# GaryGky/IDEAL-NeRF

Measured on AMD Instinct MI355X. Metric: ray-samples/sec (64+128 pts, 512x512), whole job, higher is better.
Workload: dtype f32

## Files before the change

ideal-nerf_amd/_lib.py:

```python
import ctypes as C
import os

HERE = os.path.dirname(os.path.abspath(__file__))
LIB_PATH = os.environ.get("IDN_LIB") or os.path.join(HERE, "libidealnerf.so")

IDN_PREC_F32, IDN_PREC_BF16X3, IDN_PREC_BF16, IDN_PREC_FP16X3, IDN_PREC_BF16X6 = 0, 1, 2, 3, 4
RAY_FLOATS = 11
MAX_MULTIRES, MAX_MULTIRES_VIEWS = 10, 4
SAMPLE_MAX_REGION = 4096
SCORE_TILE = 32
PROF_KINDS = ("mlp_fwd", "mlp_fwd_save", "delta_chain", "dw_gemm", "dw_gemm_x6", "mlp_fwd_save_x6", "delta_chain_x6")

fp = C.c_void_p


class FaceNerfParams(C.Structure):
    _fields_ = [("pts_w", fp * 8), ("pts_b", fp * 8), ("views_w", fp * 3), ("views_b", fp * 3),
                ("alpha_w", fp), ("alpha_b", fp), ("rgb_w", fp), ("rgb_b", fp),
                ("dim_aud", C.c_int), ("dim_expr", C.c_int), ("dim_latent", C.c_int),
                ("multires_plus1", C.c_int), ("multires_views_plus1", C.c_int)]


class FaceNerfGrads(C.Structure):
    _fields_ = [("pts_w", fp * 8), ("pts_b", fp * 8), ("views_w", fp * 3), ("views_b", fp * 3),
                ("alpha_w", fp), ("alpha_b", fp), ("rgb_w", fp), ("rgb_b", fp)]


class PassBwdExtra(C.Structure):
    _fields_ = [("d_expr", fp), ("d_rays", fp), ("d_views0_bias", fp)]


class CompositeOut(C.Structure):
    _fields_ = [(n, fp) for n in ("rgb_map", "disp_map", "acc_map", "depth_map", "weights", "rgb_fg", "last_weight")]


class RenderArgs(C.Structure):
    _fields_ = [("rays", fp), ("bc_rgb", fp), ("n_rays", C.c_int64), ("n_samples", C.c_int),
                ("n_importance", C.c_int), ("precision", C.c_int),
                ("packed_coarse", fp), ("folded_coarse", fp), ("packed_fine", fp), ("folded_fine", fp),
                ("t_vals", fp), ("t_rand", fp), ("u", fp), ("u_per_ray", C.c_int)] + \
               [(n, fp) for n in ("rgb_map", "disp_map", "acc_map", "depth_map", "last_weight", "rgb_fg",
                                  "rgb0", "disp0", "acc0", "z_std", "last_weight0", "rgb_fg0",
                                  "tap_z_coarse", "tap_raw_coarse", "tap_weights_coarse", "tap_cdf", "tap_inds",
                                  "tap_z_samples", "tap_z_fine", "tap_raw_fine", "tap_weights_fine")] + \
               [("workspace", fp), ("workspace_bytes", C.c_size_t), ("precision_fine_plus1", C.c_int),
                ("lindisp", C.c_int), ("white_bkgd", C.c_int), ("noise_coarse", fp), ("noise_fine", fp), ("fused_march", C.c_int),
                ("rng_mode", C.c_int), ("rng_seed", C.c_uint64), ("rng_ray0", C.c_int64)]


class AudioNetParams(C.Structure):
    _fields_ = [("conv_w", fp * 4), ("conv_b", fp * 4), ("fc_w", fp * 2), ("fc_b", fp * 2), ("dim_aud", C.c_int)]


class AudioNetGrads(C.Structure):
    _fields_ = [("conv_w", fp * 4), ("conv_b", fp * 4), ("fc_w", fp * 2), ("fc_b", fp * 2)]


class Frame(C.Structure):
    _fields_ = [("c2w", C.c_float * 12), ("H", C.c_int), ("W", C.c_int), ("focal", C.c_float), ("cx", C.c_float), ("cy", C.c_float),
                ("near_", C.c_float), ("far_", C.c_float), ("row0", C.c_int), ("nrows", C.c_int), ("rays_out", fp)]


class RenderOpts(C.Structure):
    _fields_ = [("colour_gate", C.c_int), ("gate_counters", fp)]


class CullGridStruct(C.Structure):
    _fields_ = [("bits", fp), ("G", C.c_int), ("lo", C.c_float * 3), ("cell", C.c_float)]


CULL_MAX_OUTPUTS = 12


class CullOutput(C.Structure):
    _fields_ = [("dense", fp), ("live", fp), ("channels", C.c_int), ("fill_background", C.c_int), ("value", C.c_float)]


DW_MAX_PRODUCTS, DW_MAX_TAKES, DW_MAX_COLSUM_TAKES = 16, 4, 2


class DwTake(C.Structure):
    _fields_ = [("row0", C.c_int), ("col0", C.c_int), ("rows", C.c_int), ("cols", C.c_int), ("out", fp), ("ldo", C.c_int)]


class DwColsumTake(C.Structure):
    _fields_ = [("col0", C.c_int), ("cols", C.c_int), ("out", fp)]


class DwProduct(C.Structure):
    _fields_ = [("delta", fp), ("ld_delta", C.c_int), ("N", C.c_int), ("acts", fp), ("ld_acts", C.c_int), ("K", C.c_int),
                ("acts2", fp), ("want_colsum", C.c_int), ("n_takes", C.c_int), ("takes", DwTake * DW_MAX_TAKES),
                ("n_colsum_takes", C.c_int), ("colsum_takes", DwColsumTake * DW_MAX_COLSUM_TAKES),
                ("splits", C.c_int), ("chunks_per_split", C.c_int)]


PATCH_MAX, PATCH_MIN_P, PATCH_MAX_P = 16, 11, 48


class PatchSet(C.Structure):
    _fields_ = [("n_patches", C.c_int), ("p", C.c_int), ("oy", C.c_int * PATCH_MAX), ("ox", C.c_int * PATCH_MAX)]


ABI_VERSION = 4

PROTOTYPES = {
    "idealnerf_version": (C.c_int, []),
    "idealnerf_last_error": (C.c_char_p, []),
    "idealnerf_packed_weight_floats": (C.c_size_t, [C.c_int]),
    "idealnerf_folded_bias_floats": (C.c_size_t, []),
    "idealnerf_pack_weights": (C.c_int, [C.POINTER(FaceNerfParams), C.c_int, fp, fp]),
    "idealnerf_fold_conditioning": (C.c_int, [C.POINTER(FaceNerfParams), fp, fp, fp, fp, fp]),
    "idealnerf_facenerf_fwd": (C.c_int, [fp, fp, C.c_int, fp, C.c_int64, fp, fp]),
    "idealnerf_facenerf_fwd_ch": (C.c_int, [fp, fp, C.c_int, fp, C.c_int, C.c_int, C.c_int64, fp, fp]),
    "idealnerf_params_pts_ch": (C.c_int, [C.POINTER(FaceNerfParams)]),
    "idealnerf_params_views_ch": (C.c_int, [C.POINTER(FaceNerfParams)]),
    "idealnerf_query_rays_fwd": (C.c_int, [fp, fp, C.c_int, fp, fp, C.c_int64, C.c_int, fp, fp]),
    "idealnerf_query_points_fwd": (C.c_int, [fp, fp, C.c_int, fp, fp, C.c_int64, C.c_int, fp, fp]),
    "idealnerf_frame_rays": (C.c_int, [C.POINTER(C.c_float), C.c_int, C.c_int, C.c_float, C.c_float, C.c_float,
                                       C.c_float, C.c_float, C.c_int, C.c_int, fp, fp]),
    "idealnerf_to8b": (C.c_int, [fp, C.c_int64, C.c_int, fp, fp, fp]),
    "idealnerf_compose_to8b": (C.c_int, [fp, fp, fp, C.c_int64, C.c_int, fp, fp, fp, fp]),
    "idealnerf_philox_uniform": (C.c_int, [C.c_uint64, C.c_int, C.c_int64, C.c_int64, C.c_int, fp, fp]),
    "idealnerf_sample_pixels_workspace_bytes": (C.c_size_t, []),
    "idealnerf_sample_pixels": (C.c_int, [fp, C.c_int, C.c_int, C.c_int, C.c_int, C.c_int, C.c_int, C.c_uint64, C.c_uint64,
                                          fp, C.c_size_t, fp, fp]),
    "idealnerf_gather_rays": (C.c_int, [fp, C.c_int64, C.POINTER(C.c_float), C.c_int, C.c_int, C.c_float, C.c_float, C.c_float,
                                        fp, fp, fp, fp, fp, fp, fp, fp]),
    "idealnerf_gather_ray_pairs": (C.c_int, [fp, C.c_int64, C.POINTER(C.c_float), C.POINTER(C.c_float), C.c_int, C.c_int, C.c_float,
                                             C.c_float, C.c_float, fp, fp, fp, fp, fp, fp, fp, fp, fp]),
    "idealnerf_frame_scores_workspace_bytes": (C.c_size_t, [C.c_int, C.c_int]),
    "idealnerf_frame_scores": (C.c_int, [fp, fp, fp, C.c_int, C.c_int, fp, fp, C.c_size_t, fp]),
    "idealnerf_patch_pixels": (C.c_int, [C.POINTER(PatchSet), C.c_int, fp, fp]),
    "idealnerf_ssim_patch_fwd": (C.c_int, [fp, fp, C.c_int, C.c_int, fp, fp]),
    "idealnerf_ssim_patch_bwd": (C.c_int, [fp, fp, C.c_int, C.c_int, C.c_float, fp, fp]),
    "idealnerf_coarse_depths": (C.c_int, [fp, fp, fp, C.c_int, C.c_int64, C.c_int, fp, fp]),
    "idealnerf_composite_fwd": (C.c_int, [fp, fp, fp, fp, fp, C.c_int, C.c_int64, C.c_int, C.POINTER(CompositeOut), fp]),
    "idealnerf_sample_pdf_fwd": (C.c_int, [fp, fp, fp, C.c_int, C.c_int64, C.c_int, C.c_int, fp, fp, fp, fp, fp, fp]),
    "idealnerf_march_fwd": (C.c_int, [fp, fp, fp, fp, fp, C.c_int, fp, C.c_int, C.c_int64, C.c_int, C.c_int,
                                      C.POINTER(CompositeOut), fp, fp, fp, fp, fp, fp]),
    "idealnerf_sample_pdf_bins_fwd": (C.c_int, [fp, fp, fp, C.c_int, C.c_int64, C.c_int, C.c_int, fp, fp, fp, fp]),
    "idealnerf_invert_cdf": (C.c_int, [fp, fp, fp, C.c_int, C.c_int64, C.c_int, C.c_int, fp, fp, fp]),
    "idealnerf_render_workspace_bytes": (C.c_size_t, [C.c_int64, C.c_int, C.c_int]),
    "idealnerf_render_rays_fwd": (C.c_int, [C.POINTER(RenderArgs), fp]),
    "idealnerf_render_frame_workspace_bytes": (C.c_size_t, [C.c_int64, C.c_int, C.c_int]),
    "idealnerf_render_frame_fwd": (C.c_int, [C.POINTER(RenderArgs), C.POINTER(Frame), fp]),
    "idealnerf_render_rays_fwd_opts": (C.c_int, [C.POINTER(RenderArgs), C.POINTER(RenderOpts), fp]),
    "idealnerf_render_frame_fwd_opts": (C.c_int, [C.POINTER(RenderArgs), C.POINTER(Frame), C.POINTER(RenderOpts), fp]),
    "idealnerf_colour_gate_max_dist": (C.c_float, []),
    "idealnerf_audio_net_saved_floats": (C.c_size_t, [C.c_int]),
    "idealnerf_audio_net_fwd": (C.c_int, [C.POINTER(AudioNetParams), fp, C.c_int, fp, fp, fp]),
    "idealnerf_audio_net_bwd": (C.c_int, [C.POINTER(AudioNetParams), C.POINTER(AudioNetGrads), fp, fp, fp, C.c_int, fp]),
    "idealnerf_train_acts_floats": (C.c_size_t, [C.c_int64]),
    "idealnerf_query_rays_train_fwd": (C.c_int, [fp, fp, C.c_int, fp, fp, C.c_int64, C.c_int, fp, fp, fp]),
    "idealnerf_query_rays_train_fwd_ch": (C.c_int, [fp, fp, C.c_int, fp, fp, C.c_int64, C.c_int, C.c_int, C.c_int, fp, fp, fp]),
    "idealnerf_pass_bwd_workspace_bytes": (C.c_size_t, [C.c_int64, C.c_int]),
    "idealnerf_pass_bwd": (C.c_int, [C.POINTER(FaceNerfParams), C.POINTER(FaceNerfGrads), fp, fp, fp, fp, fp, fp, fp,
                                     fp, C.c_int64, C.c_int, fp, fp, fp, fp, fp, fp, fp, C.c_size_t, fp]),
    "idealnerf_pass_bwd_rays": (C.c_int, [C.POINTER(FaceNerfParams), C.POINTER(FaceNerfGrads), fp, fp, fp, fp, fp, fp, fp,
                                          fp, C.c_int64, C.c_int, fp, fp, fp, fp, fp, fp, fp, fp, C.c_size_t, fp]),
    "idealnerf_pass_bwd_cond": (C.c_int, [C.POINTER(FaceNerfParams), fp, fp, fp, fp, fp, fp, fp, fp, C.c_int64, C.c_int, fp, fp, fp,
                                          fp, fp, fp, fp, C.c_size_t, fp]),
    "idealnerf_pass_bwd_ex": (C.c_int, [C.POINTER(FaceNerfParams), C.POINTER(FaceNerfGrads), fp, fp, fp, fp, fp, fp, fp,
                                        fp, C.c_int64, C.c_int, fp, fp, fp, fp, fp, fp, C.POINTER(PassBwdExtra), fp, C.c_size_t, fp]),
    "idealnerf_facenerf_train_fwd": (C.c_int, [fp, fp, C.c_int, fp, C.c_int64, fp, fp, fp]),
    "idealnerf_facenerf_train_fwd_ch": (C.c_int, [fp, fp, C.c_int, fp, C.c_int, C.c_int, C.c_int64, fp, fp, fp]),
    "idealnerf_facenerf_bwd_workspace_bytes": (C.c_size_t, [C.c_int64]),
    "idealnerf_facenerf_bwd": (C.c_int, [C.POINTER(FaceNerfParams), C.POINTER(FaceNerfGrads), fp, fp, fp, fp, C.c_int64, fp,
                                         fp, fp, fp, fp, fp, C.c_size_t, fp]),
    "idealnerf_dw_gemm_workspace_bytes": (C.c_size_t, []),
    "idealnerf_dw_gemm": (C.c_int, [fp, C.c_int, fp, C.c_int, C.c_int64, fp, fp, C.c_int, fp, C.c_size_t, fp]),
    "idealnerf_dw_products_workspace_bytes": (C.c_size_t, []),
    "idealnerf_dw_products": (C.c_int, [C.c_int64, C.c_int, C.c_int, C.POINTER(DwProduct), C.c_int, fp, C.c_size_t, fp]),
    "idealnerf_delta_chain_workspace_bytes": (C.c_size_t, []),
    "idealnerf_delta_chain": (C.c_int, [C.POINTER(FaceNerfParams), C.c_int, fp, C.c_int64, fp, fp, fp, fp, C.c_int,
                                        C.POINTER(C.c_int), fp, C.c_size_t, fp]),
    "idealnerf_composite_bwd": (C.c_int, [fp, fp, fp, fp, C.c_int64, C.c_int, fp, fp, fp, fp, fp, C.c_int, fp, C.c_int, fp, C.c_int, fp]),
    "idealnerf_input_grad": (C.c_int, [C.POINTER(FaceNerfParams), fp, fp, fp, C.c_int64, C.c_int64, fp, C.c_int, C.POINTER(C.c_int), fp]),
    "idealnerf_ray_grad": (C.c_int, [fp, C.c_int, C.c_int, fp, fp, C.c_int64, C.c_int, fp, fp]),
    "idealnerf_fold_bwd": (C.c_int, [C.POINTER(FaceNerfParams), fp, fp, fp, fp, fp, fp, fp, fp, fp, fp, fp, fp, fp]),
    "idealnerf_cond_colsums_workspace_bytes": (C.c_size_t, []),
    "idealnerf_cond_colsums": (C.c_int, [fp, fp, fp, C.c_int64, C.c_int64, fp, fp, fp, C.c_size_t, fp]),
    "idealnerf_cull_mark": (C.c_int, [fp, C.c_int64, C.c_float, fp, fp]),
    "idealnerf_cull_cells": (C.c_int, [fp, C.c_int, C.c_int, fp, fp]),
    "idealnerf_cull_classify_workspace_bytes": (C.c_size_t, [C.c_int64]),
    "idealnerf_cull_classify": (C.c_int, [C.POINTER(CullGridStruct), C.POINTER(Frame), C.c_float, C.c_int, fp, fp, fp, C.c_size_t, fp]),
    "idealnerf_cull_gather": (C.c_int, [fp, C.c_int64, C.POINTER(Frame), fp, fp, fp, fp]),
    "idealnerf_cull_scatter": (C.c_int, [fp, C.c_int64, C.c_int64, fp, C.POINTER(CullOutput), C.c_int, fp]),
    "idealnerf_cull_sample_classify": (C.c_int, [C.POINTER(CullGridStruct), fp, fp, C.c_int64, C.c_int, fp, fp, fp, C.c_size_t, fp]),
    "idealnerf_cull_sample_gather": (C.c_int, [fp, C.c_int64, fp, fp, C.c_int64, C.c_int, fp, fp, fp]),
    "idealnerf_cull_sample_scatter": (C.c_int, [fp, C.c_int64, fp, C.c_int64, fp, fp]),
    "idealnerf_profile_begin": (None, []),
    "idealnerf_profile_end": (C.c_int, [C.POINTER(C.c_double), C.POINTER(C.c_int64), C.POINTER(C.c_int64)]),
    "idealnerf_profile_end_kinds": (C.c_int, [C.POINTER(C.c_double), C.POINTER(C.c_int64), C.POINTER(C.c_int64)]),
}

_lib = None


class IdealNerfError(RuntimeError):
    pass


def load():
    global _lib
    if _lib is not None:
        return _lib
    if not os.path.exists(LIB_PATH):
        raise IdealNerfError(
            f"{LIB_PATH} is missing: build the HIP extension first "
            "(python ideal-nerf_amd/build.py, or __graft_entry__.build()). There is no fallback path.")
    lib = C.CDLL(LIB_PATH)
    for name, (res, args) in PROTOTYPES.items():
        fn = getattr(lib, name)
        fn.restype = res
        fn.argtypes = args
    if lib.idealnerf_version() != ABI_VERSION:
        raise IdealNerfError(f"{LIB_PATH} has ABI version {lib.idealnerf_version()}, this package binds version {ABI_VERSION}: rebuild it")
    _lib = lib
    return lib


def check(rc):
    if rc != 0:
        msg = load().idealnerf_last_error()
        raise IdealNerfError(f"libidealnerf error {rc}: {msg.decode() if msg else '?'}")
```

ideal-nerf_amd/csrc/dw_gemm.h:

```cpp
#pragma once
#include "mlp_common.h"

namespace idn {

__device__ __forceinline__ f32x16 mfma32(float a, float b, f32x16 c) { return __builtin_amdgcn_mfma_f32_32x32x2f32(a, b, c, 0, 0, 0); }
__device__ __forceinline__ int d_row(int r, int hh) { return (r & 3) + 8 * (r >> 2) + 4 * hh; }

struct TNArgs {
    const float* A; int lda;
    const float* B; int ldb;
    float* part;
    int N, K;
    long P;
    int chunks_per_split;
    float* cpart;
    int b_split, b_off0, b_off1;
};
constexpr int kMaxTnBatch = 12;
struct TNBatch {
    TNArgs it[kMaxTnBatch];
    int n, splits;
};
constexpr int kMaxReduceItems = 32;
struct ReduceItem {
    const float* part;
    float* out;
    int splits, N, K, ldo, rows, cols;
    int block_end;
};
struct ReduceBatch {
    ReduceItem it[kMaxReduceItems];
    int n;
};

inline size_t al256(size_t x) { return (x + 255) & ~(size_t)255; }
enum { kPipeX6 = IDN_DW_PIPE_BF16X6, kPipeF32 = IDN_DW_PIPE_F32 };

struct DwPassProduct { int N, K; bool colsum; int pipes; };
constexpr int kOnX6 = 1 << kPipeX6, kOnF32 = 1 << kPipeF32, kOnBoth = kOnX6 | kOnF32;
constexpr DwPassProduct kTrunk = {256, 256, true, kOnBoth};
constexpr DwPassProduct kPassProducts[] = {
    {64, 128, true, kOnBoth},
    {256, 256, true, kOnX6}, {128, 128, true, kOnF32}, {128, 128, true, kOnF32},
    kTrunk, {128, 64, false, kOnBoth},
    kTrunk, kTrunk, kTrunk, {256, 64, false, kOnBoth}, kTrunk, kTrunk, kTrunk, kTrunk,
    {256, 64, true, kOnBoth},
};
constexpr size_t pass_sum(int pipe, int what) {
    size_t n = 0;
    for (const DwPassProduct& t : kPassProducts)
        if (t.pipes >> pipe & 1) n += what == 0 ? (t.N == 256 && t.K == 256) : what == 1 ? (size_t)t.N * t.K : t.colsum ? t.N : 0;
    return n;
}
constexpr int kX6ItemsPerPass = (int)pass_sum(kPipeX6, 0);
static_assert(kX6ItemsPerPass == 9 && kX6ItemsPerPass <= kMaxTnBatch, "one x6 batch per pass");

constexpr int kMaxSplits = 256;
constexpr int kColsumBlocks = 256;
constexpr int kGemmsPerPass = 16;
constexpr size_t kPartFloatsPerSplit = 9 * 65536 + 6 * 16384 + 4 * 8192;
constexpr size_t kPartPoolFloats = (size_t)kMaxSplits * kPartFloatsPerSplit, kCpartPoolFloats = (size_t)kColsumBlocks * 256 * kGemmsPerPass;
static_assert(pass_sum(kPipeX6, 1) <= kPartFloatsPerSplit && pass_sum(kPipeF32, 1) <= kPartFloatsPerSplit, "a pass's partial blocks fit");
static_assert(kMaxSplits * pass_sum(kPipeX6, 2) <= kCpartPoolFloats && kMaxSplits * pass_sum(kPipeF32, 2) <= kCpartPoolFloats, "a pass's column sums fit");

struct DwProduct { const float *part, *cpart; int splits, N, K, chunks_per_split; };

struct DwPass {
    DwPass(float* part, size_t part_floats, float* cpart, size_t cpart_floats, int64_t P, int pipe, int x6_items, hipStream_t s)
        : part_next(part), part_left(part_floats), cpart_next(cpart), cpart_left(cpart_floats), P(P), pipe(pipe), x6_items(x6_items), s(s) {}
    int product(const float* A, int lda, int N, const float* B, int ldb, int K, bool want_colsum, DwProduct* h, const float* B2 = nullptr);
    int take(const DwProduct& h, int row0, int col0, int rows, int cols, float* out, int ldo);
    int take_colsum(const DwProduct& h, int col0, int cols, float* out);
    int finish();

private:
    float* part_next; size_t part_left;
    float* cpart_next; size_t cpart_left;
    int64_t P;
    int pipe, x6_items;
    hipStream_t s;
    TNBatch x6{{}, 0, 0};
    ReduceBatch red{{}, 0};
    int red_blocks = 0;
};

}
```

ideal-nerf_amd/csrc/dw_gemm.hip:

```cpp
#include "dw_gemm.h"
#include "mlp_x6.h"

namespace idn {

template <int N>
struct LdsVec;
template <>
struct LdsVec<4> {
    f32x4 v;
    template <int OFF>
    __device__ __forceinline__ void issue(uint32_t addr) { asm volatile("ds_read_b128 %0, %1 offset:%2" : "=v"(v) : "v"(addr), "n"(OFF) : "memory"); }
    __device__ __forceinline__ float get(int j) const { return v[j]; }
};
template <>
struct LdsVec<2> {
    typedef float f32x2 __attribute__((ext_vector_type(2)));
    f32x2 v;
    template <int OFF>
    __device__ __forceinline__ void issue(uint32_t addr) { asm volatile("ds_read_b64 %0, %1 offset:%2" : "=v"(v) : "v"(addr), "n"(OFF) : "memory"); }
    __device__ __forceinline__ float get(int j) const { return v[j]; }
};
template <>
struct LdsVec<1> {
    float v;
    template <int OFF>
    __device__ __forceinline__ void issue(uint32_t addr) { asm volatile("ds_read_b32 %0, %1 offset:%2" : "=v"(v) : "v"(addr), "n"(OFF) : "memory"); }
    __device__ __forceinline__ float get(int) const { return v; }
};
template <int OFF>
__device__ __forceinline__ void lds_read_f32(float& dst, uint32_t addr) {
    asm volatile("ds_read_b32 %0, %1 offset:%2" : "=v"(dst) : "v"(addr), "n"(OFF) : "memory");
}
__device__ __forceinline__ float landed(float& v) {
    asm volatile("" : "+v"(v));
    return v;
}
template <int NEWER, class VA, class VB>
__device__ __forceinline__ void lds_retire(VA& a, VB& b) {
    if constexpr (NEWER == 0) asm volatile("s_waitcnt lgkmcnt(0)" : "+v"(a.v), "+v"(b.v)::"memory");
    else asm volatile("s_waitcnt lgkmcnt(2)" : "+v"(a.v), "+v"(b.v)::"memory");
}

constexpr int kTnRows = 16, kTnBufs = 3;
constexpr int kTnNarrowBufs = 3;
constexpr int kTnRows4x1 = 32, kTnRowsThin = 64;
constexpr int kTnNarrowSplits = 256;

template <int NTW, int KTW, int NB = kTnBufs, int R = kTnRows>
__global__ __launch_bounds__(256) void gemm_tn_kernel(TNArgs g) {
    static_assert(R % 16 == 0, "chunks are multiples of 16 points");
    constexpr int NPA = NTW * R / 16, NPB = KTW * R / 16;
    static_assert(NB >= 3 && (NB - 2) * (NPA + NPB) <= 63, "vmcnt is a 6-bit field");
    constexpr int BN = 64 * NTW, BK = 64 * KTW;
    constexpr int kTileFloats = R * (BN + BK);
    constexpr int kSteps = R / 2;
    constexpr int NP = NPA + NPB;
    static_assert(NP <= kSteps, "at most one piece per step");
    extern __shared__ __attribute__((aligned(16))) float tn_smem[];
    const int tid = threadIdx.x, lane = tid & 63;
    const int w = __builtin_amdgcn_readfirstlane(tid >> 6);
    const int i = lane & 31, hh = lane >> 5;
    const int wr = w >> 1, wc = w & 1;
    const int n0 = blockIdx.x * BN, k0 = blockIdx.y * BK;
    const int split = blockIdx.z;
    f32x16 acc[NTW][KTW];
#pragma unroll
    for (int a = 0; a < NTW; ++a)
#pragma unroll
        for (int b = 0; b < KTW; ++b)
            for (int r = 0; r < 16; ++r) acc[a][b][r] = 0.f;

    const long c_begin = (long)split * g.chunks_per_split;
    long c_end = c_begin + g.chunks_per_split;
    const long c_total = g.P / R;
    if (c_end > c_total) c_end = c_total;
    const bool colsum_block = g.cpart != nullptr && blockIdx.y == 0;
    const bool do_colsum = colsum_block && tid < BN;
    const int ccol = tid < BN ? tid : 0;
    float csum = 0.0f;

    constexpr int kRowsPerPieceA = 256 / BN > 0 ? 256 / BN : 1, kRowsPerPieceB = 256 / BK > 0 ? 256 / BK : 1;
    const __amdgpu_buffer_rsrc_t rsrcA = __builtin_amdgcn_make_buffer_rsrc(const_cast<float*>(g.A + n0 + c_begin * R * (long)g.lda), 0, 0xfffffffc, 0x00020000);
    const __amdgpu_buffer_rsrc_t rsrcB = __builtin_amdgcn_make_buffer_rsrc(const_cast<float*>(g.B + k0 + c_begin * R * (long)g.ldb), 0, 0xfffffffc, 0x00020000);
    const uint32_t voffA = ((lane / (BN / 4)) * g.lda + (lane % (BN / 4)) * 4) * 4;
    const uint32_t voffB = ((lane / (BK / 4)) * g.ldb + (lane % (BK / 4)) * 4) * 4;
    const uint32_t rowA = g.lda * 4, rowB = g.ldb * 4;
    auto piece_a = [&](long c, int buf, int ja) {
        const int pc = NPA * w + ja;
        __builtin_amdgcn_raw_ptr_buffer_load_lds(rsrcA, (__attribute__((address_space(3))) void*)(tn_smem + buf * kTileFloats + pc * 256), 16, voffA,
                                                 (uint32_t)(((c - c_begin) * R + pc * kRowsPerPieceA) * rowA), 0, 0);
    };
    auto piece_b = [&](long c, int buf, int jb) {
        const int pc = NPB * w + jb;
        __builtin_amdgcn_raw_ptr_buffer_load_lds(rsrcB, (__attribute__((address_space(3))) void*)(tn_smem + buf * kTileFloats + R * BN + pc * 256), 16, voffB,
                                                 (uint32_t)(((c - c_begin) * R + pc * kRowsPerPieceB) * rowB), 0, 0);
    };
    auto piece = [&](long c, int buf, int j) {
        if (j < NPA) piece_a(c, buf, j);
        else if (j < NP) piece_b(c, buf, j - NPA);
    };
    const uint32_t smem0 = (uint32_t)(uintptr_t)(__attribute__((address_space(3))) float*)tn_smem;
    const uint32_t a_addr0 = smem0 + (hh * BN + NTW * (32 * wr + i)) * 4;
    const uint32_t b_addr0 = smem0 + (R * BN + hh * BK + KTW * (32 * wc + i)) * 4;
    for (int ahead = 0; ahead < NB - 1; ++ahead)
        for (int j = 0; j < NP; ++j) piece(c_begin + ahead < c_end ? c_begin + ahead : c_end - 1, ahead, j);
    int buf = 0;
    for (long c = c_begin; c < c_end; ++c) {
        asm volatile("s_waitcnt vmcnt(%0)" ::"n"((NB - 2) * NP) : "memory");
        __builtin_amdgcn_s_barrier();
        asm volatile("" ::: "memory");
        const int buf2 = buf >= 1 ? buf - 1 : NB - 1;
        const long cnext = c + NB - 1 < c_end ? c + NB - 1 : c_end - 1;
        float cs[16];
        auto cs_issue = [&](int batch) {
            const uint32_t caddr = smem0 + buf * (kTileFloats * 4) + ccol * 4 + batch * (16 * BN * 4);
            static_for<16>([&](auto Row) {
                lds_read_f32<decltype(Row)::value * BN * 4>(cs[decltype(Row)::value], caddr);
            });
        };
        static_assert(R / 16 <= kSteps / 4, "one batch of column reads per iteration of the first half loop");
        if (colsum_block) cs_issue(0);
        LdsVec<NTW> a0v, a1v;
        LdsVec<KTW> b0v, b1v;
        constexpr int kStepA = 2 * BN * 4, kStepB = 2 * BK * 4;
        uint32_t pa = a_addr0 + buf * (kTileFloats * 4), pb = b_addr0 + buf * (kTileFloats * 4);
        a0v.template issue<0>(pa);
        b0v.template issue<0>(pb);
        static_assert(NPA <= kSteps / 2 && NPB <= kSteps / 2, "pieces of one matrix fit one half of a chunk");
        constexpr int M = NTW * KTW;
        if constexpr (M >= 4) {
            auto step = [&](LdsVec<NTW>& ca, LdsVec<KTW>& cb, auto&& side0, auto&& side1, auto&& side2) {
                lds_retire<0>(ca, cb);
                static_for<M>([&](auto M_) {
                    constexpr int m = decltype(M_)::value, x = m / KTW, y = m % KTW;
                    acc[x][y] = mfma32(ca.get(x), cb.get(y), acc[x][y]);
                    if constexpr (m < 3) {
                        __builtin_amdgcn_sched_barrier(0);
                        if constexpr (m == 0) side0();
                        if constexpr (m == 1) side1();
                        if constexpr (m == 2) side2();
                        __builtin_amdgcn_sched_barrier(0);
                    }
                });
            };
#pragma unroll 1
            for (int it = 0; it < kSteps / 4; ++it) {
                step(a0v, b0v,
                     [&]() { a1v.template issue<kStepA>(pa); b1v.template issue<kStepB>(pb); },
                     [&]() { if (2 * it < NPA) piece_a(cnext, buf2, 2 * it); },
                     [&]() {
                         if (colsum_block && it < R / 16) {
                             static_for<16>([&](auto Row) { csum += landed(cs[decltype(Row)::value]); });
                         }
                         pa += 2 * kStepA;
                         pb += 2 * kStepB;
                     });
                step(a1v, b1v,
                     [&]() { a0v.template issue<0>(pa); b0v.template issue<0>(pb); },
                     [&]() { if (2 * it + 1 < NPA) piece_a(cnext, buf2, 2 * it + 1); },
                     [&]() { if (colsum_block && it + 1 < R / 16) cs_issue(it + 1); });
            }
#pragma unroll 1
            for (int it = 0; it < kSteps / 4; ++it) {
                const bool last = it == kSteps / 4 - 1;
                step(a0v, b0v,
                     [&]() { a1v.template issue<kStepA>(pa); b1v.template issue<kStepB>(pb); },
                     [&]() { if (2 * it < NPB) piece_b(cnext, buf2, 2 * it); },
                     [&]() {
                         pa = last ? pa : pa + 2 * kStepA;
                         pb = last ? pb : pb + 2 * kStepB;
                     });
                step(a1v, b1v,
                     [&]() { a0v.template issue<0>(pa); b0v.template issue<0>(pb); },
                     [&]() { if (2 * it + 1 < NPB) piece_b(cnext, buf2, 2 * it + 1); },
                     [&]() {});
            }
        } else {
            static_assert(M == 2 && kSteps % 8 == 0, "the two-pair schedule");
            LdsVec<NTW> a2v, a3v;
            LdsVec<KTW> b2v, b3v;
            a1v.template issue<kStepA>(pa);
            b1v.template issue<kStepB>(pb);
            auto quad = [&](LdsVec<NTW>& c0a, LdsVec<KTW>& c0b, LdsVec<NTW>& c1a, LdsVec<KTW>& c1b, LdsVec<NTW>& n0a, LdsVec<KTW>& n0b,
                            LdsVec<NTW>& n1a, LdsVec<KTW>& n1b, bool last, auto&& side_c, auto&& side_d) {
                lds_retire<0>(c0a, c0b);
                lds_retire<0>(c1a, c1b);
                const uint32_t na = last ? pa : pa + 2 * kStepA, nb = last ? pb : pb + 2 * kStepB;
                auto mf = [&](LdsVec<NTW>& ca, LdsVec<KTW>& cb, auto M_) {
                    constexpr int m = decltype(M_)::value, x = m / KTW, y = m % KTW;
                    acc[x][y] = mfma32(ca.get(x), cb.get(y), acc[x][y]);
                    __builtin_amdgcn_sched_barrier(0);
                };
                mf(c0a, c0b, ic<0>{});
                n0a.template issue<0>(na);
                n0b.template issue<0>(nb);
                __builtin_amdgcn_sched_barrier(0);
                mf(c0a, c0b, ic<1>{});
                n1a.template issue<kStepA>(na);
                n1b.template issue<kStepB>(nb);
                __builtin_amdgcn_sched_barrier(0);
                mf(c1a, c1b, ic<0>{});
                side_c();
                __builtin_amdgcn_sched_barrier(0);
                mf(c1a, c1b, ic<1>{});
                side_d();
                pa = na;
                pb = nb;
                __builtin_amdgcn_sched_barrier(0);
            };
#pragma unroll 1
            for (int it = 0; it < kSteps / 8; ++it) {
                quad(a0v, b0v, a1v, b1v, a2v, b2v, a3v, b3v, false,
                     [&]() { if (2 * it < NPA) piece_a(cnext, buf2, 2 * it); },
                     [&]() {
                         if (colsum_block && it < R / 16) {
                             static_for<16>([&](auto Row) { csum += landed(cs[decltype(Row)::value]); });
                         }
                     });
                quad(a2v, b2v, a3v, b3v, a0v, b0v, a1v, b1v, false,
                     [&]() { if (2 * it + 1 < NPA) piece_a(cnext, buf2, 2 * it + 1); },
                     [&]() { if (colsum_block && it + 1 < R / 16) cs_issue(it + 1); });
            }
#pragma unroll 1
            for (int it = 0; it < kSteps / 8; ++it) {
                quad(a0v, b0v, a1v, b1v, a2v, b2v, a3v, b3v, false,
                     [&]() { if (2 * it < NPB) piece_b(cnext, buf2, 2 * it); }, [&]() {});
                quad(a2v, b2v, a3v, b3v, a0v, b0v, a1v, b1v, it == kSteps / 8 - 1,
                     [&]() { if (2 * it + 1 < NPB) piece_b(cnext, buf2, 2 * it + 1); }, [&]() {});
            }
            lds_retire<0>(a1v, b1v);
        }
        lds_retire<0>(a0v, b0v);
        buf = buf + 1 == NB ? 0 : buf + 1;
    }
    asm volatile("s_waitcnt vmcnt(0)" ::: "memory");
    if (do_colsum) g.cpart[(long)split * g.N + n0 + tid] = csum;
    float* out = g.part + (long)split * g.N * g.K;
#pragma unroll
    for (int x = 0; x < NTW; ++x)
#pragma unroll
        for (int r = 0; r < 16; ++r) {
            const int n = n0 + NTW * (32 * wr + d_row(r, hh)) + x;
            float* dst = out + (long)n * g.K + k0 + KTW * (32 * wc + i);
            if constexpr (KTW == 4) {
                *reinterpret_cast<f32x4*>(dst) = f32x4{acc[x][0][r], acc[x][1][r], acc[x][2][r], acc[x][3][r]};
            } else {
#pragma unroll
                for (int y = 0; y < KTW; ++y) dst[y] = acc[x][y][r];
            }
        }
}

typedef unsigned tn_u32x4 __attribute__((ext_vector_type(4)));
typedef int tn_i32x4 __attribute__((ext_vector_type(4)));
__device__ __forceinline__ void split3(float x0, float x1, unsigned& p1, unsigned& p2, unsigned& p3) {
    float w1, w2, w3;
    x6::split3(x0, x1, w1, w2, w3);
    p1 = __float_as_uint(w1), p2 = __float_as_uint(w2), p3 = __float_as_uint(w3);
}
constexpr int kX6BufBytes = 2 * 8 * 3 * kFragBytes;
constexpr int kX6Lds = 2 * kX6BufBytes;

struct X6Frag {
    f32x4 v;
    template <int OFF>
    __device__ __forceinline__ void issue(uint32_t addr) { asm volatile("ds_read_b128 %0, %1 offset:%2" : "=v"(v) : "v"(addr), "n"(OFF) : "memory"); }
};
template <int N>
__device__ __forceinline__ void x6_retire(X6Frag (&f)[3]) {
    static_assert(N <= 15, "lgkmcnt is a 4-bit field");
    asm volatile("s_waitcnt lgkmcnt(%3)" : "+v"(f[0].v), "+v"(f[1].v), "+v"(f[2].v) : "n"(N) : "memory");
}

__device__ __forceinline__ void gemm_tn_x6_item(const TNArgs& g, const int split, char* x6_smem) {
    const int tid = threadIdx.x, lane = tid & 63;
    const int w = __builtin_amdgcn_readfirstlane(tid >> 6);
    const int i = lane & 31, hh = lane >> 5;
    const int wr = w >> 1, wc = w & 1;
    f32x16 acc[4][4];
#pragma unroll
    for (int a = 0; a < 4; ++a)
#pragma unroll
        for (int b = 0; b < 4; ++b)
            for (int r = 0; r < 16; ++r) acc[a][b][r] = 0.f;

    const long c_begin = (long)split * g.chunks_per_split;
    long c_end = c_begin + g.chunks_per_split;
    const long c_total = g.P / kTnRows;
    if (c_end > c_total) c_end = c_total;
    const int n_chunks = (int)(c_end - c_begin);
    auto make_rsrc = [](const float* ptr) {
        const uint64_t a64 = (uint64_t)(uintptr_t)ptr;
        return tn_i32x4{(int)(uint32_t)a64, (int)((uint32_t)(a64 >> 32) & 0xffffu), (int)0xfffffffcu, 0x00020000};
    };
    const tn_i32x4 rsrcA = make_rsrc(g.A + c_begin * kTnRows * (long)g.lda);
    const tn_i32x4 rsrcB = make_rsrc(g.B + c_begin * kTnRows * (long)g.ldb);
    const int voff = tid * 4;
    const int voffB = g.b_split ? (tid < 128 ? g.b_off0 : g.b_off1) + (tid & 127) * 4 : voff;
    const int rowA = g.lda * 4, rowB = g.ldb * 4;
    float ra[kTnRows], rb[kTnRows];
#pragma unroll
    for (int p = 0; p < kTnRows; ++p) ra[p] = rb[p] = 0.f;
    auto load_row_at = [&](float& dst, const tn_i32x4& rsrc, int soff, int vo) {
        asm volatile("buffer_load_dword %0, %1, %2, %3 offen" : "+v"(dst) : "v"(vo), "s"(rsrc), "s"(soff) : "memory");
    };
    auto load_row = [&](float& dst, const tn_i32x4& rsrc, int soff) { load_row_at(dst, rsrc, soff, voff); };
    auto load_chunk = [&](int rc) {
        const int base = (rc < n_chunks ? rc : n_chunks - 1) * kTnRows;
#pragma unroll
        for (int p = 0; p < kTnRows; ++p) load_row(ra[p], rsrcA, (base + p) * rowA);
#pragma unroll
        for (int p = 0; p < kTnRows; ++p) load_row_at(rb[p], rsrcB, (base + p) * rowB, voffB);
    };
    char* const my_slot = x6_smem + (tid >> 5) * (3 * kFragBytes) + (tid & 31) * 16;
    auto split_store = [&](int buf, int X, const float (&r)[kTnRows]) {
        unsigned pw[3][8];
#pragma unroll
        for (int j = 0; j < 8; ++j) split3(r[2 * j], r[2 * j + 1], pw[0][j], pw[1][j], pw[2][j]);
        char* dst = my_slot + buf * kX6BufBytes + X * (8 * 3 * kFragBytes);
#pragma unroll
        for (int q = 0; q < 3; ++q)
#pragma unroll
            for (int h2 = 0; h2 < 2; ++h2)
                *reinterpret_cast<tn_u32x4*>(dst + q * kFragBytes + h2 * 512) =
                    tn_u32x4{pw[q][4 * h2], pw[q][4 * h2 + 1], pw[q][4 * h2 + 2], pw[q][4 * h2 + 3]};
    };
    const bool do_colsum = g.cpart != nullptr;
    float csum = 0.0f, csum1 = 0.0f;
    auto colsum = [&]() {
        float s0 = (ra[0] + ra[1]) + (ra[2] + ra[3]), s1 = (ra[4] + ra[5]) + (ra[6] + ra[7]);
        float s2 = (ra[8] + ra[9]) + (ra[10] + ra[11]), s3 = (ra[12] + ra[13]) + (ra[14] + ra[15]);
        csum += (s0 + s1) + (s2 + s3);
    };
    const uint32_t smem0 = (uint32_t)(uintptr_t)(__attribute__((address_space(3))) char*)x6_smem;
    const uint32_t a_base = smem0 + (4 * wr) * (3 * kFragBytes) + lane * 16;
    const uint32_t b_base = smem0 + (8 + 4 * wc) * (3 * kFragBytes) + lane * 16;

    load_chunk(0);
#pragma unroll
    for (int p = 0; p < kTnRows; ++p) asm volatile("s_waitcnt vmcnt(0)" : "+v"(ra[p]), "+v"(rb[p])::"memory");
    colsum();
    split_store(0, 0, ra);
    split_store(0, 1, rb);
    load_chunk(1);
    asm volatile("s_waitcnt lgkmcnt(0)" ::: "memory");
    __builtin_amdgcn_s_barrier();
    asm volatile("" ::: "memory");

    X6Frag fa[4][3], fb[4][3];
    auto issue_first_row = [&](uint32_t pa, uint32_t pb) {
        static_for<3>([&](auto Q) { fa[0][decltype(Q)::value].template issue<decltype(Q)::value * kFragBytes>(pa); });
        static_for<2>([&](auto Y) {
            static_for<3>([&](auto Q) {
                fb[decltype(Y)::value][decltype(Q)::value].template issue<(decltype(Y)::value * 3 + decltype(Q)::value) * kFragBytes>(pb);
            });
        });
    };
    issue_first_row(a_base, b_base);
#pragma unroll 1
    for (int rc = 0; rc < n_chunks; ++rc) {
        const int buf = rc & 1;
        const uint32_t pa = a_base + buf * kX6BufBytes, pb = b_base + buf * kX6BufBytes;
        static_for<2>([&](auto Y) {
            static_for<3>([&](auto Q) {
                fb[decltype(Y)::value + 2][decltype(Q)::value].template issue<((decltype(Y)::value + 2) * 3 + decltype(Q)::value) * kFragBytes>(pb);
            });
        });
        static_for<3>([&](auto X) {
            static_for<3>([&](auto Q) {
                fa[decltype(X)::value + 1][decltype(Q)::value].template issue<((decltype(X)::value + 1) * 3 + decltype(Q)::value) * kFragBytes>(pa);
            });
        });
        auto mm2 = [&](int x, int y0, int y1) {
#define X6_TERM(QA, QB)                                                   \
    acc[x][y0] = x6::mfma_bf(fa[x][QA].v, fb[y0][QB].v, acc[x][y0]);        \
    acc[x][y1] = x6::mfma_bf(fa[x][QA].v, fb[y1][QB].v, acc[x][y1]);
            X6_TERM(0, 0) X6_TERM(0, 1) X6_TERM(1, 0) X6_TERM(1, 1) X6_TERM(0, 2) X6_TERM(2, 0)
#undef X6_TERM
        };
        x6_retire<15>(fa[0]);
        x6_retire<15>(fb[0]);
        x6_retire<15>(fb[1]);
        mm2(0, 0, 1);
        x6_retire<9>(fb[2]);
        x6_retire<9>(fb[3]);
        mm2(0, 2, 3);
        x6_retire<0>(fa[1]);
        x6_retire<0>(fa[2]);
        x6_retire<0>(fa[3]);
        const unsigned live_mask = rc + 1 < n_chunks ? 0xffffffffu : 0u;
        const int nbase = (rc + 2 < n_chunks ? rc + 2 : n_chunks - 1) * kTnRows;
        char* const dst = my_slot + (buf ^ 1) * kX6BufBytes;
        unsigned pw[2][3][8];
        float t0 = 0.f, t1 = 0.f;
        auto slice = [&](auto X_, auto S_) {
            constexpr int X = decltype(X_)::value, sl = decltype(S_)::value;
            float (&r)[kTnRows] = *(X ? &rb : &ra);
            auto store = [&](auto Q_, auto H_) {
                constexpr int q = decltype(Q_)::value, h2 = decltype(H_)::value;
                *reinterpret_cast<tn_u32x4*>(dst + X * (8 * 3 * kFragBytes) + q * kFragBytes + h2 * 512) =
                    tn_u32x4{pw[X][q][4 * h2], pw[X][q][4 * h2 + 1], pw[X][q][4 * h2 + 2], pw[X][q][4 * h2 + 3]};
            };
            if constexpr (sl < 24) {
                constexpr int j = sl / 3, ph = sl % 3;
                if constexpr (ph == 0) {
                    asm volatile("s_waitcnt vmcnt(30)" : "+v"(r[2 * j]), "+v"(r[2 * j + 1])::"memory");
                    const unsigned p1 = x6::cvt_pk_bf16(r[2 * j], r[2 * j + 1]);
                    pw[X][0][j] = p1;
                    t0 = r[2 * j] - __uint_as_float(p1 << 16);
                    t1 = r[2 * j + 1] - __uint_as_float(p1 & 0xffff0000u);
                    if constexpr (X == 0) {
                        csum += __uint_as_float(__float_as_uint(r[2 * j]) & live_mask);
                        csum1 += __uint_as_float(__float_as_uint(r[2 * j + 1]) & live_mask);
                        asm volatile("" : "+v"(csum), "+v"(csum1));
                    }
                } else if constexpr (ph == 1) {
                    const unsigned p2 = x6::cvt_pk_bf16(t0, t1);
                    pw[X][1][j] = p2;
                    t0 = t0 - __uint_as_float(p2 << 16);
                    t1 = t1 - __uint_as_float(p2 & 0xffff0000u);
                    pw[X][2][j] = x6::cvt_pk_bf16(t0, t1);
                } else {
                    load_row_at(r[2 * j], X ? rsrcB : rsrcA, (nbase + 2 * j) * (X ? rowB : rowA), X ? voffB : voff);
                    load_row_at(r[2 * j + 1], X ? rsrcB : rsrcA, (nbase + 2 * j + 1) * (X ? rowB : rowA), X ? voffB : voff);
                    if constexpr (j >= 3 && j < 6) store(ic<j - 3>{}, ic<0>{});
                    if constexpr (j == 7) store(ic<0>{}, ic<1>{});
                }
            } else if constexpr (sl == 24) {
                store(ic<1>{}, ic<1>{});
            } else if constexpr (sl == 25) {
                store(ic<2>{}, ic<1>{});
            }
        };
        __builtin_amdgcn_sched_barrier(0);
        static_for<72>([&](auto K_) {
            constexpr int k = decltype(K_)::value;
            constexpr int x = 1 + k / 24, kk = k % 24, y = 2 * (kk / 12) + (kk % 2), t = (kk % 12) / 2;
            constexpr int qa = t == 2 || t == 3 ? 1 : (t == 5 ? 2 : 0);
            constexpr int qb = t == 1 || t == 3 ? 1 : (t == 4 ? 2 : 0);
            acc[x][y] = x6::mfma_bf(fa[x][qa].v, fb[y][qb].v, acc[x][y]);
            constexpr int kX1 = 26;
            if constexpr (k < kX1) slice(ic<0>{}, ic<k>{});
            else slice(ic<1>{}, ic<k - kX1>{});
            if constexpr (k == 59) {
                asm volatile("s_waitcnt lgkmcnt(0)" ::: "memory");
                __builtin_amdgcn_s_barrier();
                asm volatile("" ::: "memory");
                issue_first_row(a_base + (buf ^ 1) * kX6BufBytes, b_base + (buf ^ 1) * kX6BufBytes);
            }
            __builtin_amdgcn_sched_barrier(0);
        });
    }
    x6_retire<0>(fa[0]);
    x6_retire<0>(fb[0]);
    x6_retire<0>(fb[1]);
#pragma unroll
    for (int p = 0; p < kTnRows; ++p) asm volatile("s_waitcnt vmcnt(0)" : "+v"(ra[p]), "+v"(rb[p])::"memory");
    if (do_colsum) g.cpart[(long)split * g.N + tid] = csum + csum1;
    float* out = g.part + (long)split * g.N * g.K;
#pragma unroll
    for (int x = 0; x < 4; ++x)
#pragma unroll
        for (int y = 0; y < 4; ++y)
#pragma unroll
            for (int r = 0; r < 16; ++r)
                out[(long)(32 * (4 * wr + x) + d_row(r, hh)) * g.K + 32 * (4 * wc + y) + i] = acc[x][y][r];
}
__global__ __launch_bounds__(256) void gemm_tn_x6_kernel(TNBatch b) {
    extern __shared__ __attribute__((aligned(16))) char x6_smem[];
    const int item = __builtin_amdgcn_readfirstlane((int)blockIdx.z / b.splits);
    const int split = __builtin_amdgcn_readfirstlane((int)blockIdx.z - item * b.splits);
    gemm_tn_x6_item(b.it[item], split, x6_smem);
}

__global__ __launch_bounds__(256) void reduce_batch_kernel(ReduceBatch b) {
    __shared__ double red[4][64];
    int i = 0;
    while (i + 1 < b.n && (int)blockIdx.x >= b.it[i].block_end) ++i;
    const ReduceItem& t = b.it[i];
    const int block0 = i ? b.it[i - 1].block_end : 0;
    const int o = threadIdx.x & 63, q = threadIdx.x >> 6;
    const int idx = ((int)blockIdx.x - block0) * 64 + o;
    const bool live = idx < t.rows * t.cols;
    const int n = live ? idx / t.cols : 0, k = live ? idx % t.cols : 0;
    double s = 0.0;
    if (live) {
        const float* src = t.part + (long)n * t.K + k;
        const long stride = (long)t.N * t.K;
#pragma unroll 8
        for (int sp = q; sp < t.splits; sp += 4) s += (double)src[sp * stride];
    }
    red[q][o] = s;
    __syncthreads();
    if (q == 0 && live) t.out[(long)n * t.ldo + k] = (float)(((red[0][o] + red[1][o]) + red[2][o]) + red[3][o]);
}

template <int NTW, int KTW, int NB, int R = kTnRows>
static int launch_tn(const TNArgs& g, int splits, hipStream_t s) {
    constexpr size_t lds = (size_t)NB * R * (size_t)(64 * NTW + 64 * KTW) * 4;
    static_assert(lds <= 160 * 1024, "the chunk ring must fit a CU's LDS");
    static LaunchSetup setup;
    int num_cu = 0;
    if (int e = setup.get([]() -> int {
            IDN_HIP_CHECK(hipFuncSetAttribute(reinterpret_cast<const void*>(&gemm_tn_kernel<NTW, KTW, NB, R>),
                                              hipFuncAttributeMaxDynamicSharedMemorySize, (int)lds));
            return IDN_OK;
        }, &num_cu))
        return e;
    hipLaunchKernelGGL((gemm_tn_kernel<NTW, KTW, NB, R>), dim3(g.N / (64 * NTW), g.K / (64 * KTW), splits), dim3(256), lds, s, g);
    IDN_HIP_CHECK(hipGetLastError());
    return IDN_OK;
}
struct DwShape { int N, K, rows_per_chunk, max_splits; int (*launch)(const TNArgs&, int, hipStream_t); };
constexpr DwShape kX6Shape = {256, 256, kTnRows, kMaxSplits, nullptr};
constexpr DwShape kF32Shapes[] = {
    {256, 256, kTnRows, kMaxSplits, &launch_tn<4, 4, kTnBufs>},
    {256, 64, kTnRows4x1, kTnNarrowSplits, &launch_tn<4, 1, kTnNarrowBufs, kTnRows4x1>},
    {128, 256, kTnRows, kMaxSplits, &launch_tn<2, 4, kTnBufs>},
    {128, 64, kTnRowsThin, kTnNarrowSplits, &launch_tn<2, 1, kTnNarrowBufs, kTnRowsThin>},
    {128, 128, kTnRows, kMaxSplits, &launch_tn<2, 2, kTnBufs>},
    {64, 128, kTnRowsThin, kTnNarrowSplits, &launch_tn<1, 2, kTnNarrowBufs, kTnRowsThin>},
};
static_assert(kTnNarrowSplits <= kMaxSplits, "the pools hold kMaxSplits splits of every product of a pass (dw_gemm.h)");

static int x6_setup(int* cus) {
    static LaunchSetup st;
    return st.get([]() -> int {
        IDN_HIP_CHECK(hipFuncSetAttribute(reinterpret_cast<const void*>(&gemm_tn_x6_kernel), hipFuncAttributeMaxDynamicSharedMemorySize, kX6Lds));
        return IDN_OK;
    }, cus);
}

int DwPass::product(const float* A, int lda, int N, const float* B, int ldb, int K, bool want_colsum, DwProduct* h, const float* B2) {
    const DwShape* sh = nullptr;
    if (N == 256 && K == 256 && pipe == kPipeX6) sh = &kX6Shape;
    else
        for (const DwShape& t : kF32Shapes)
            if (t.N == N && t.K == K) sh = &t;
    if (!sh) return fail(IDN_EUNSUPPORTED, "gemm_tn: no instantiation for %d x %d", N, K);
    const bool queued = sh->launch == nullptr;
    if (B2 && !queued) return fail(IDN_EINVAL, "gemm_tn: a split B needs the 256 x 256 bf16-piece kernel");
    if (P % sh->rows_per_chunk) return fail(IDN_EINVAL, "gemm_tn: %lld rows are not a multiple of the %d-row chunk", (long long)P, sh->rows_per_chunk);
    const long chunks = P / sh->rows_per_chunk;
    int splits = sh->max_splits;
    if (queued) {
        if (x6.n >= x6_items || x6.n >= kMaxTnBatch) return fail(IDN_EINVAL, "gemm_tn: more 256 x 256 products than the pass declared (%d)", x6_items);
        int cus = 0;
        if (int e = x6_setup(&cus)) return e;
        splits = 2 * cus / x6_items;
        if (splits > kMaxSplits) splits = kMaxSplits;
    }
    if (splits > chunks) splits = (int)chunks;
    if (splits < 1) splits = 1;
    const int cps = (int)((chunks + splits - 1) / splits);
    splits = (int)((chunks + cps - 1) / cps);
    const size_t part_floats = (size_t)splits * N * K, cpart_floats = want_colsum ? (size_t)splits * N : 0;
    if (part_floats > part_left || cpart_floats > cpart_left)
        return fail(IDN_EWORKSPACE, "gemm_tn: the partial blocks of %d x %d in %d splits do not fit the pool", N, K, splits);
    TNArgs g{A, lda, B, ldb, part_next, N, K, (long)P, cps, want_colsum ? cpart_next : nullptr, 0, 0, 0};
    if (B2) {
        const float* base = B < B2 ? B : B2;
        const int64_t o0 = (int64_t)(B - base) * 4, o1 = (int64_t)(B2 - base) * 4;
        if (o0 >= (int64_t)1 << 31 || o1 >= (int64_t)1 << 31) return fail(IDN_EUNSUPPORTED, "gemm_tn: split B matrices more than 2 GiB apart");
        g.B = base, g.b_split = 1;
        g.b_off0 = (int)o0, g.b_off1 = (int)o1;
    }
    if (queued) {
        x6.splits = splits;
        x6.it[x6.n++] = g;
    } else {
        ProfScope prof(s, P, IDN_PROF_DW_GEMM);
        if (int e = sh->launch(g, splits, s)) return e;
    }
    *h = DwProduct{g.part, g.cpart, splits, N, K, cps};
    part_next += part_floats, part_left -= part_floats;
    cpart_next += cpart_floats, cpart_left -= cpart_floats;
    return IDN_OK;
}

int DwPass::take(const DwProduct& h, int row0, int col0, int rows, int cols, float* out, int ldo) {
    if (red.n >= kMaxReduceItems) return fail(IDN_EUNSUPPORTED, "reduce queue full");
    red_blocks += (rows * cols + 63) / 64;
    red.it[red.n++] = ReduceItem{h.part + (size_t)row0 * h.K + col0, out, h.splits, h.N, h.K, ldo, rows, cols, red_blocks};
    return IDN_OK;
}
int DwPass::take_colsum(const DwProduct& h, int col0, int cols, float* out) {
    if (!h.cpart) return fail(IDN_EINVAL, "gemm_tn: the product kept no column sums");
    return take(DwProduct{h.cpart, nullptr, h.splits, 1, h.N, h.chunks_per_split}, 0, col0, 1, cols, out, cols);
}

int DwPass::finish() {
    if (x6.n) {
        ProfScope prof(s, P * x6.n, IDN_PROF_DW_GEMM_X6);
        hipLaunchKernelGGL(gemm_tn_x6_kernel, dim3(1, 1, x6.splits * x6.n), dim3(256), kX6Lds, s, x6);
    }
    IDN_HIP_CHECK(hipGetLastError());
    if (red.n) hipLaunchKernelGGL(reduce_batch_kernel, dim3(red_blocks), dim3(256), 0, s, red);
    IDN_HIP_CHECK(hipGetLastError());
    return IDN_OK;
}

size_t dw_gemm_workspace_bytes() { return al256((size_t)kMaxSplits * 65536 * 4) + al256((size_t)kColsumBlocks * 256 * 4); }
int launch_dw_gemm(const float* delta, int ld_delta, const float* acts, int ld_acts, int64_t rows, float* dW, float* db, int pipe,
                   void* ws, size_t ws_bytes, hipStream_t s) {
    if (rows <= 0 || rows % 128) return fail(IDN_EINVAL, "dw_gemm: rows %lld is not a positive multiple of 128", (long long)rows);
    if (ld_delta < 256 || ld_acts < 256) return fail(IDN_EINVAL, "dw_gemm: row pitch < 256");
    const int x6_items = pipe == IDN_DW_PIPE_BF16X6_PASS ? kX6ItemsPerPass : 1;
    if (pipe == IDN_DW_PIPE_BF16X6_PASS) pipe = IDN_DW_PIPE_BF16X6;
    if (pipe != IDN_DW_PIPE_BF16X6 && pipe != IDN_DW_PIPE_F32) return fail(IDN_EINVAL, "dw_gemm: pipe %d", pipe);
    if (!ws || ws_bytes < dw_gemm_workspace_bytes()) return fail(IDN_EWORKSPACE, "dw_gemm workspace %zu < %zu", ws_bytes, dw_gemm_workspace_bytes());
    float* part = reinterpret_cast<float*>(ws);
    float* cpart = reinterpret_cast<float*>(reinterpret_cast<char*>(ws) + al256((size_t)kMaxSplits * 65536 * 4));
    DwPass q(part, (size_t)kMaxSplits * 65536, cpart, (size_t)kColsumBlocks * 256, rows, pipe, x6_items, s);
    DwProduct h;
    if (int e = q.product(delta, ld_delta, 256, acts, ld_acts, 256, db != nullptr, &h)) return e;
    int e = db ? q.take_colsum(h, 0, 256, db) : IDN_OK;
    if (!e) e = q.take(h, 0, 0, 256, 256, dW, 256);
    return e ? e : q.finish();
}

size_t dw_products_workspace_bytes() { return al256(kPartPoolFloats * 4) + al256(kCpartPoolFloats * 4); }
int launch_dw_products(int64_t rows, int pipe, int x6_items, idn_dw_product* pr, int n, void* ws, size_t ws_bytes, hipStream_t s) {
    if (!pr) return fail(IDN_EINVAL, "dw_products: NULL pointer");
    if (n < 1 || n > IDN_DW_MAX_PRODUCTS) return fail(IDN_EINVAL, "dw_products: %d products outside [1, %d]", n, IDN_DW_MAX_PRODUCTS);
    if (pipe != kPipeX6 && pipe != kPipeF32) return fail(IDN_EINVAL, "dw_products: pipe %d", pipe);
    if (rows <= 0 || rows % 128) return fail(IDN_EINVAL, "dw_products: rows %lld is not a positive multiple of 128", (long long)rows);
    if (rows > (int64_t)1 << 24) return fail(IDN_EUNSUPPORTED, "dw_products: rows %lld exceed 2^24", (long long)rows);
    if (pipe == kPipeX6 && (x6_items < 1 || x6_items > kMaxTnBatch))
        return fail(IDN_EINVAL, "dw_products: x6_items %d outside [1, %d]", x6_items, kMaxTnBatch);
    int n_x6 = 0, n_red = 0;
    size_t part_per_split = 0, cpart_per_split = 0;
    for (int i = 0; i < n; ++i) {
        const idn_dw_product& t = pr[i];
        if (!t.delta || !t.acts) return fail(IDN_EINVAL, "dw_products: product %d: NULL pointer", i);
        const bool x6 = t.N == 256 && t.K == 256 && pipe == kPipeX6;
        bool known = x6;
        for (const DwShape& sh : kF32Shapes) known = known || (sh.N == t.N && sh.K == t.K);
        if (!known) return fail(IDN_EUNSUPPORTED, "dw_products: product %d: no instantiation for %d x %d", i, t.N, t.K);
        const int b_cols = t.acts2 ? 128 : t.K;
        if (t.ld_delta < t.N || t.ld_acts < b_cols) return fail(IDN_EINVAL, "dw_products: product %d: row pitch %d / %d < %d / %d", i, t.ld_delta, t.ld_acts, t.N, b_cols);
        if (t.ld_delta % 4 || t.ld_acts % 4 || ((uintptr_t)t.delta | (uintptr_t)t.acts | (uintptr_t)t.acts2) % 16)
            return fail(IDN_EINVAL, "dw_products: product %d: operands are not 16-byte aligned row by row", i);
        if (t.acts2 && !x6) return fail(IDN_EINVAL, "dw_products: product %d: a split B needs the 256 x 256 bf16-piece kernel", i);
        if (t.acts2) {
            const uintptr_t lo = (uintptr_t)(t.acts < t.acts2 ? t.acts : t.acts2), hi = (uintptr_t)(t.acts < t.acts2 ? t.acts2 : t.acts);
            if (hi - lo >= (uintptr_t)1 << 31) return fail(IDN_EUNSUPPORTED, "dw_products: product %d: split B matrices more than 2 GiB apart", i);
        }
        if (x6 && ++n_x6 > x6_items) return fail(IDN_EINVAL, "dw_products: more 256 x 256 products than x6_items (%d)", x6_items);
        if (t.n_takes < 0 || t.n_takes > IDN_DW_MAX_TAKES || t.n_colsum_takes < 0 || t.n_colsum_takes > IDN_DW_MAX_COLSUM_TAKES)
            return fail(IDN_EINVAL, "dw_products: product %d: %d takes / %d column-sum takes", i, t.n_takes, t.n_colsum_takes);
        if (t.n_colsum_takes && !t.want_colsum) return fail(IDN_EINVAL, "dw_products: product %d kept no column sums", i);
        if ((n_red += t.n_takes + t.n_colsum_takes) > kMaxReduceItems)
            return fail(IDN_EINVAL, "dw_products: more than %d takes in one pass", kMaxReduceItems);
        for (int j = 0; j < t.n_takes; ++j) {
            const idn_dw_take& k = t.takes[j];
            if (!k.out) return fail(IDN_EINVAL, "dw_products: product %d take %d: NULL pointer", i, j);
            if (k.row0 < 0 || k.col0 < 0 || k.rows < 1 || k.cols < 1 || k.row0 + k.rows > t.N || k.col0 + k.cols > t.K || k.ldo < k.cols)
                return fail(IDN_EINVAL, "dw_products: product %d take %d leaves the %d x %d block (or its pitch is short)", i, j, t.N, t.K);
        }
        for (int j = 0; j < t.n_colsum_takes; ++j) {
            const idn_dw_colsum_take& k = t.colsum_takes[j];
            if (!k.out) return fail(IDN_EINVAL, "dw_products: product %d column-sum take %d: NULL pointer", i, j);
            if (k.col0 < 0 || k.cols < 1 || k.col0 + k.cols > t.N)
                return fail(IDN_EINVAL, "dw_products: product %d column-sum take %d leaves the %d columns", i, j, t.N);
        }
        part_per_split += (size_t)t.N * t.K;
        cpart_per_split += t.want_colsum ? t.N : 0;
    }
    if (part_per_split > kPartFloatsPerSplit || cpart_per_split * kMaxSplits > kCpartPoolFloats)
        return fail(IDN_EWORKSPACE, "dw_products: the list's partial blocks do not fit the pools of a pass");
    if (!ws || ws_bytes < dw_products_workspace_bytes())
        return fail(IDN_EWORKSPACE, "dw_products workspace %zu < %zu", ws_bytes, dw_products_workspace_bytes());
    float* part = reinterpret_cast<float*>(ws);
    float* cpart = reinterpret_cast<float*>(reinterpret_cast<char*>(ws) + al256(kPartPoolFloats * 4));
    DwPass q(part, kPartPoolFloats, cpart, kCpartPoolFloats, rows, pipe, x6_items, s);
    for (int i = 0; i < n; ++i) {
        idn_dw_product& t = pr[i];
        DwProduct h;
        if (int e = q.product(t.delta, t.ld_delta, t.N, t.acts, t.ld_acts, t.K, t.want_colsum != 0, &h, t.acts2)) return e;
        for (int j = 0; j < t.n_colsum_takes; ++j)
            if (int e = q.take_colsum(h, t.colsum_takes[j].col0, t.colsum_takes[j].cols, t.colsum_takes[j].out)) return e;
        for (int j = 0; j < t.n_takes; ++j) {
            const idn_dw_take& k = t.takes[j];
            if (int e = q.take(h, k.row0, k.col0, k.rows, k.cols, k.out, k.ldo)) return e;
        }
        t.splits = h.splits, t.chunks_per_split = h.chunks_per_split;
    }
    return q.finish();
}

}
```

ideal-nerf_amd/csrc/train.hip:

```cpp
#include "dw_gemm.h"
#include "march.h"
#include <cstdlib>

namespace idn {

__device__ __forceinline__ double shfl_up_dd(double v, int delta) {
    int lo = __double2loint(v), hi = __double2hiint(v);
    lo = __shfl_up(lo, delta, 64);
    hi = __shfl_up(hi, delta, 64);
    return __hiloint2double(hi, lo);
}
__device__ __forceinline__ double shfl_down_dd(double v, int delta) {
    int lo = __double2loint(v), hi = __double2hiint(v);
    lo = __shfl_down(lo, delta, 64);
    hi = __shfl_down(hi, delta, 64);
    return __hiloint2double(hi, lo);
}
__device__ __forceinline__ double shfl_xor_dd(double v, int mask) {
    int lo = __double2loint(v), hi = __double2hiint(v);
    lo = __shfl_xor(lo, mask, 64);
    hi = __shfl_xor(hi, mask, 64);
    return __hiloint2double(hi, lo);
}

template <int SPL, bool kNorm = false>
__global__ __launch_bounds__(256) void composite_bwd_kernel(CompBwdArgs a) {
    const int lane = threadIdx.x & 63;
    const long ray = (long)blockIdx.x * 4 + (threadIdx.x >> 6);
    if (ray >= a.n_rays) return;
    const int S = a.S;
    const float* rr = a.rays + ray * IDN_RAY_FLOATS;
    const float dn = sqrtf((rr[3] * rr[3] + rr[4] * rr[4]) + rr[5] * rr[5]);
    const float4* rawr = a.raw + ray * S;
    const float* zr = a.z + ray * S;
    float gr = 0, gg = 0, gb = 0, fr = 0, fg = 0, fb = 0, glw = 0, gacc = 0;
    if (a.g_rgb) { gr = a.g_rgb[ray * 3]; gg = a.g_rgb[ray * 3 + 1]; gb = a.g_rgb[ray * 3 + 2]; }
    if (a.g_fg) { fr = a.g_fg[ray * 3]; fg = a.g_fg[ray * 3 + 1]; fb = a.g_fg[ray * 3 + 2]; }
    if (a.g_lw) glw = a.g_lw[ray];
    if (a.g_acc) gacc = a.g_acc[ray];

    float zs[SPL + 1];
    float4 rw[SPL];
#pragma unroll
    for (int i = 0; i < SPL; ++i) {
        const int s = lane * SPL + i;
        zs[i] = s < S ? zr[s] : 0.f;
        rw[i] = s < S ? rawr[s] : make_float4(0.f, 0.f, 0.f, 0.f);
    }
    zs[SPL] = __shfl_down(zs[0], 1, 64);
    float alpha[SPL], tf[SPL], ex[SPL], dist[SPL];
    double local = 1.0;
#pragma unroll
    for (int i = 0; i < SPL; ++i) {
        const int s = lane * SPL + i;
        float d = (s >= S - 1) ? 1e10f : (zs[i + 1] - zs[i]);
        d = d * dn;
        const float e = expf(-(fmaxf(rw[i].w, 0.0f) + 1e-6f) * d);
        dist[i] = d;
        ex[i] = e;
        alpha[i] = (s < S) ? 1.0f - e : 0.0f;
        tf[i] = (s < S) ? (1.0f - (1.0f - e)) + 1e-10f : 1.0f;
        local *= (double)tf[i];
    }
    double incl = local;
#pragma unroll
    for (int d = 1; d < 64; d <<= 1) {
        const double o = shfl_up_dd(incl, d);
        if (lane >= d) incl *= o;
    }
    double run = shfl_up_dd(incl, 1);
    if (lane == 0) run = 1.0;
    float T[SPL], w[SPL], dw[SPL], cr[SPL], cg[SPL], cb[SPL];
    double lsum = 0.0;
#pragma unroll
    for (int i = 0; i < SPL; ++i) {
        const int s = lane * SPL + i;
        T[i] = (float)run;
        w[i] = alpha[i] * T[i];
        run *= (double)tf[i];
        dw[i] = 0.f;
        cr[i] = cg[i] = cb[i] = 0.f;
        if (s < S) {
            if (s == S - 1) {
                cr[i] = a.bc[ray * 3]; cg[i] = a.bc[ray * 3 + 1]; cb[i] = a.bc[ray * 3 + 2];
                dw[i] = (gr * cr[i] + gg * cg[i] + gb * cb[i]) + glw + gacc;
            } else {
                cr[i] = 1.0f / (1.0f + expf(-rw[i].x));
                cg[i] = 1.0f / (1.0f + expf(-rw[i].y));
                cb[i] = 1.0f / (1.0f + expf(-rw[i].z));
                dw[i] = ((gr + fr) * cr[i] + (gg + fg) * cg[i] + (gb + fb) * cb[i]) + gacc;
            }
            lsum += (double)dw[i] * (double)w[i];
        }
    }
    double lsfx = lsum;
#pragma unroll
    for (int d = 1; d < 64; d <<= 1) {
        const double o = shfl_down_dd(lsfx, d);
        if (lane + d < 64) lsfx += o;
    }
    double after = shfl_down_dd(lsfx, 1);
    if (lane == 63) after = 0.0;
    double sfx[SPL];
#pragma unroll
    for (int i = SPL - 1; i >= 0; --i) {
        sfx[i] = after;
        after += (double)dw[i] * (double)w[i];
    }
    double nsum = 0.0;
#pragma unroll
    for (int i = 0; i < SPL; ++i) {
        const int s = lane * SPL + i;
        if (s < S) {
            const float dalpha = dw[i] * T[i] - (float)(sfx[i] / (double)tf[i]);
            const float dsig = (rw[i].w > 0.f) ? dalpha * ex[i] * dist[i] : 0.f;
            if constexpr (kNorm) {
                if (s < S - 1)
                    nsum += (double)dalpha * (double)ex[i] * (double)(fmaxf(rw[i].w, 0.0f) + 1e-6f) * (double)(zs[i + 1] - zs[i]);
            }
            const long p = ray * S + s;
            a.d_sig[p * a.ld_sig] = dsig;
            float d0 = 0.f, d1 = 0.f, d2 = 0.f;
            if (s < S - 1) {
                d0 = w[i] * (gr + fr) * cr[i] * (1.0f - cr[i]);
                d1 = w[i] * (gg + fg) * cg[i] * (1.0f - cg[i]);
                d2 = w[i] * (gb + fb) * cb[i] * (1.0f - cb[i]);
            }
            a.d_rgb[p * a.ld_rgb + 0] = d0;
            a.d_rgb[p * a.ld_rgb + 1] = d1;
            a.d_rgb[p * a.ld_rgb + 2] = d2;
        }
    }
    if constexpr (kNorm) {
#pragma unroll
        for (int m = 32; m >= 1; m >>= 1) nsum += shfl_xor_dd(nsum, m);
        if (lane == 0) a.d_norm[ray * a.ld_norm] = (float)nsum;
    }
}

__device__ __forceinline__ float cond_val(const FoldBwdArgs& d, int c) {
    if (c < d.p.dim_aud) return d.aud[c];
    c -= d.p.dim_aud;
    if (c < d.p.dim_expr) return d.expr[c] * 1.0f / 3.0f;
    c -= d.p.dim_expr;
    return d.latent[c];
}
template <bool kCondOnly>
__global__ void fold_bwd_kernel(FoldBwdArgs d) {
    const int C = d.p.dim_aud + d.p.dim_expr + d.p.dim_latent;
    const int PC = pts_ch_of(d.p), VC = views_ch_of(d.p);
    const int ld0 = PC + C, ld5 = PC + C + IDN_W, ldv = IDN_W + VC + d.p.dim_expr;
    const int idx = blockIdx.x * blockDim.x + threadIdx.x + (kCondOnly ? IDN_W * C + (IDN_W / 2) * d.p.dim_expr : 0);
    const int n_outer = IDN_W * C;
    if (!kCondOnly && idx < n_outer) {
        const int n = idx / C, c = idx % C;
        const float cv = cond_val(d, c);
        d.gW0[(long)n * ld0 + PC + c] = d.db0[n] * cv;
        d.gW5[(long)n * ld5 + PC + c] = d.db5[n] * cv;
    } else if (!kCondOnly && idx < n_outer + (IDN_W / 2) * d.p.dim_expr) {
        const int k = idx - n_outer, n = k / d.p.dim_expr, e = k % d.p.dim_expr;
        d.gWv0[(long)n * ldv + IDN_W + VC + e] = d.dbv[n] * (d.expr[e] * 1.0f / 3.0f);
    } else {
        const int rel = idx - n_outer - (IDN_W / 2) * d.p.dim_expr;
        const int c = rel >> 6, lane = rel & 63;
        if (c >= C) return;
        double s = 0.0;
        for (int n = lane; n < IDN_W; n += 64)
            s += (double)d.p.pts_w[0][(long)n * ld0 + PC + c] * (double)d.db0[n] +
                 (double)d.p.pts_w[5][(long)n * ld5 + PC + c] * (double)d.db5[n];
#pragma unroll
        for (int m = 32; m >= 1; m >>= 1) s += shfl_xor_dd(s, m);
        const int e = c - d.p.dim_aud;
        const bool want_expr = d.d_expr != nullptr && e >= 0 && e < d.p.dim_expr;
        double sv = 0.0;
        if (want_expr) {
            for (int n = lane; n < IDN_W / 2; n += 64)
                sv += (double)d.p.views_w[0][(long)n * ldv + IDN_W + VC + e] * (double)d.dbv[n];
#pragma unroll
            for (int m = 32; m >= 1; m >>= 1) sv += shfl_xor_dd(sv, m);
        }
        if (lane != 0) return;
        if (c < d.p.dim_aud) {
            if (d.d_aud) d.d_aud[c] += (float)s;
        } else if (c >= d.p.dim_aud + d.p.dim_expr) {
            if (d.d_latent) d.d_latent[c - d.p.dim_aud - d.p.dim_expr] += (float)s;
        } else if (want_expr) {
            d.d_expr[e] += (float)((s + sv) / 3.0);
        }
    }
}

__global__ __launch_bounds__(256) void colsum_rows_kernel(const float* m0, const float* m1, long rows, long rows_per_block, double* part) {
    const float* m = blockIdx.y ? m1 : m0;
    const long r0 = (long)blockIdx.x * rows_per_block;
    const long r1 = r0 + rows_per_block < rows ? r0 + rows_per_block : rows;
    const float* col = m + threadIdx.x;
    double acc = 0.0;
    long r = r0;
    for (; r + 8 <= r1; r += 8) {
        float v[8];
#pragma unroll
        for (int i = 0; i < 8; ++i) v[i] = col[(r + i) * 256];
#pragma unroll
        for (int i = 0; i < 8; ++i) acc += (double)v[i];
    }
    for (; r < r1; ++r) acc += (double)col[r * 256];
    part[((long)blockIdx.x * 2 + blockIdx.y) * 256 + threadIdx.x] = acc;
}
__global__ __launch_bounds__(256) void colsum_finish_kernel(const double* part, int blocks, float* out) {
    double acc = 0.0;
    for (int b = 0; b < blocks; ++b) acc += part[((long)b * 2 + blockIdx.x) * 256 + threadIdx.x];
    out[blockIdx.x * 256 + threadIdx.x] = (float)acc;
}
constexpr int kCondColsumBlocks = 512;
static_assert(512 + (size_t)kCondColsumBlocks * 512 * 2 <= kCpartPoolFloats, "the conditioning-only column sums fit the cpart pool");
size_t cond_colsums_workspace_bytes() { return (size_t)kCondColsumBlocks * 512 * sizeof(double); }

int launch_cond_colsums(const float* dA0, const float* dA5, const float* dV0, int64_t P, int64_t Pp, float* db, float* dbv,
                        double* part, hipStream_t s) {
    const int64_t chunks = Pp / 128;
    const int64_t rows_per_block = (chunks + kCondColsumBlocks - 1) / kCondColsumBlocks * 128;
    if (dA0) {
        const int blocks = (int)((Pp + rows_per_block - 1) / rows_per_block);
        hipLaunchKernelGGL(colsum_rows_kernel, dim3(blocks, 2), dim3(256), 0, s, dA0, dA5, (long)Pp, (long)rows_per_block, part);
        IDN_HIP_CHECK(hipGetLastError());
        hipLaunchKernelGGL(colsum_finish_kernel, dim3(2), dim3(256), 0, s, (const double*)part, blocks, db);
        IDN_HIP_CHECK(hipGetLastError());
    }
    if (dV0) {
        const int blocks = (int)((P + rows_per_block - 1) / rows_per_block);
        hipLaunchKernelGGL(colsum_rows_kernel, dim3(blocks, 1), dim3(128), 0, s, dV0, dV0, (long)P, (long)rows_per_block, part);
        IDN_HIP_CHECK(hipGetLastError());
        hipLaunchKernelGGL(colsum_finish_kernel, dim3(1), dim3(128), 0, s, (const double*)part, blocks, dbv);
        IDN_HIP_CHECK(hipGetLastError());
    }
    return IDN_OK;
}

int launch_fold_bwd(const FoldBwdArgs& f, bool cond_only, hipStream_t s) {
    const int C = f.p.dim_aud + f.p.dim_expr + f.p.dim_latent;
    if (cond_only) {
        if (C == 0) return IDN_OK;
        hipLaunchKernelGGL(fold_bwd_kernel<true>, dim3((C * 64 + 255) / 256), dim3(256), 0, s, f);
    } else {
        const int total = IDN_W * C + (IDN_W / 2) * f.p.dim_expr + C * 64;
        if (total == 0) return IDN_OK;
        hipLaunchKernelGGL(fold_bwd_kernel<false>, dim3((total + 255) / 256), dim3(256), 0, s, f);
    }
    IDN_HIP_CHECK(hipGetLastError());
    return IDN_OK;
}

struct BwdWs {
    float *dA[8], *dV[2], *dV0, *dRGB, *part, *cpart, *wbwd;
    size_t bytes;
};
static BwdWs carve_bwd(char* base, int64_t p_pad) {
    BwdWs w;
    size_t off = 0;
    auto take = [&](size_t floats) {
        float* p = reinterpret_cast<float*>(base + off);
        off += al256(floats * 4);
        return p;
    };
    for (int l = 0; l < 8; ++l) w.dA[l] = take((size_t)p_pad * 256);
    w.dV[0] = take((size_t)p_pad * 256);
    w.dV[1] = w.dV[0] + 128;
    w.dV0 = take((size_t)p_pad * 256);
    w.dRGB = take((size_t)p_pad * 64);
    w.part = take(kPartPoolFloats);
    w.cpart = take(kCpartPoolFloats);
    w.wbwd = take(bwd_stream_floats_x6());
    w.bytes = off;
    return w;
}

size_t bwd_workspace_bytes(int64_t n_points) {
    const int64_t p_pad = (n_points + 127) / 128 * 128;
    return carve_bwd(nullptr, p_pad).bytes;
}

static int backward_pipe() {
    static const int v = [] {
        const char* e = getenv("IDN_BACKWARD_PIPE");
        return (e && e[0] == 'f' && e[1] == '3' && e[2] == '2' && e[3] == 0) ? kPipeF32 : kPipeX6;
    }();
    return v;
}

static int bwd_tail(const idn_facenerf_params& p, const idn_facenerf_grads* grads, const BwdCond& cond, const float* acts, int64_t P,
                    int64_t Pp, const BwdWs& w, hipStream_t s) {
    const int C = p.dim_aud + p.dim_expr + p.dim_latent;
    const int PC = pts_ch_of(p), VC = views_ch_of(p);
    const int ld0 = PC + C, ld5 = PC + C + IDN_W, ldv = IDN_W + VC + p.dim_expr;
    auto act = [&](int i) { return acts + (size_t)act_off(i) * Pp; };
    auto a_l = [&](int l) { return act(kActA1 + l - 1); };
    auto v_l = [&](int l) { return act(kActV1 + l - 1); };
#define TRY(x) do { if (int e_ = (x)) return e_; } while (0)
    const int pipe = backward_pipe();
    if (pipe == kPipeX6) {
        TRY(launch_pack_bf16x6_bwd(p, w.wbwd, s));
        TRY(launch_delta_chain_x6(w.wbwd, acts, Pp, w.dRGB, w.dV0, w.dV[0], w.dV[1], w.dA, s));
    } else {
        TRY(launch_pack_f32_bwd(p, w.wbwd, s));
        TRY(launch_delta_chain(w.wbwd, acts, Pp, w.dRGB, w.dV0, w.dV[0], w.dV[1], w.dA, s));
    }
    if (!grads) {
        const bool want_dbv = cond.d_expr != nullptr || cond.d_vb != nullptr;
        if (C == 0 && !want_dbv) return IDN_OK;
        float* db = w.cpart;
        double* part = reinterpret_cast<double*>(w.cpart + 512);
        float* dbv = cond.d_vb ? cond.d_vb : w.part;
        TRY(launch_cond_colsums(C > 0 ? w.dA[0] : nullptr, w.dA[5], want_dbv ? w.dV0 : nullptr, P, Pp, db, dbv, part, s));
        const FoldBwdArgs f{p, cond.aud, cond.expr, cond.latent, db, db + 256, dbv, nullptr, nullptr, nullptr, cond.d_aud, cond.d_latent, cond.d_expr};
        return launch_fold_bwd(f, true, s);
    }
    const idn_facenerf_grads& gr = *grads;
    DwPass q(w.part, kPartPoolFloats, w.cpart, kCpartPoolFloats, Pp, pipe, kX6ItemsPerPass, s);
    DwProduct h;
    TRY(q.product(w.dRGB, 64, 64, v_l(3), 128, 128, true, &h));
    TRY(q.take_colsum(h, 0, 3, gr.rgb_b));
    TRY(q.take(h, 0, 0, 3, 128, gr.rgb_w, 128));
    if (pipe == kPipeX6) {
        TRY(q.product(w.dV[0], 256, 256, v_l(2), 128, 256, true, &h, v_l(1)));
        TRY(q.take_colsum(h, 0, 128, gr.views_b[2]));
        TRY(q.take_colsum(h, 128, 128, gr.views_b[1]));
        TRY(q.take(h, 0, 0, 128, 128, gr.views_w[2], 128));
        TRY(q.take(h, 128, 128, 128, 128, gr.views_w[1], 128));
    } else {
        for (int l = 2; l >= 1; --l) {
            TRY(q.product(w.dV[2 - l], 256, 128, v_l(l), 128, 128, true, &h));
            TRY(q.take_colsum(h, 0, 128, gr.views_b[l]));
            TRY(q.take(h, 0, 0, 128, 128, gr.views_w[l], 128));
        }
    }
    TRY(q.product(w.dV0, 256, 256, a_l(8), 256, 256, true, &h));
    TRY(q.take_colsum(h, 0, 128, gr.views_b[0]));
    TRY(q.take_colsum(h, kSigmaChannel, 1, gr.alpha_b));
    TRY(q.take(h, 0, 0, 128, 256, gr.views_w[0], ldv));
    TRY(q.take(h, kSigmaChannel, 0, 1, 256, gr.alpha_w, 256));
    TRY(q.product(w.dV0, 256, 128, act(kActDir), 64, 64, false, &h));
    TRY(q.take(h, 0, 0, 128, VC, gr.views_w[0] + IDN_W, ldv));
    for (int l = 7; l >= 1; --l) {
        TRY(q.product(w.dA[l], 256, 256, a_l(l), 256, 256, true, &h));
        TRY(q.take_colsum(h, 0, 256, gr.pts_b[l]));
        TRY(q.take(h, 0, 0, 256, 256, l == 5 ? gr.pts_w[5] + PC + C : gr.pts_w[l], l == 5 ? ld5 : 256));
        if (l == 5) {
            TRY(q.product(w.dA[5], 256, 256, act(kActX0), 64, 64, false, &h));
            TRY(q.take(h, 0, 0, 256, PC, gr.pts_w[5], ld5));
        }
    }
    TRY(q.product(w.dA[0], 256, 256, act(kActX0), 64, 64, true, &h));
    TRY(q.take_colsum(h, 0, 256, gr.pts_b[0]));
    TRY(q.take(h, 0, 0, 256, PC, gr.pts_w[0], ld0));
    TRY(q.finish());
    const FoldBwdArgs f{p, cond.aud, cond.expr, cond.latent, gr.pts_b[0], gr.pts_b[5], gr.views_b[0], gr.pts_w[0], gr.pts_w[5],
                        gr.views_w[0], cond.d_aud, cond.d_latent, cond.d_expr};
    TRY(launch_fold_bwd(f, false, s));
#undef TRY
    return IDN_OK;
}


template <bool kNorm>
static void launch_composite_bwd_spl(const CompBwdArgs& a, hipStream_t s) {
    const dim3 grid((unsigned)((a.n_rays + 3) / 4)), block(256);
    switch ((a.S + 63) / 64) {
        case 1: hipLaunchKernelGGL((composite_bwd_kernel<1, kNorm>), grid, block, 0, s, a); break;
        case 2: hipLaunchKernelGGL((composite_bwd_kernel<2, kNorm>), grid, block, 0, s, a); break;
        case 3: hipLaunchKernelGGL((composite_bwd_kernel<3, kNorm>), grid, block, 0, s, a); break;
        case 4: hipLaunchKernelGGL((composite_bwd_kernel<4, kNorm>), grid, block, 0, s, a); break;
        case 5: hipLaunchKernelGGL((composite_bwd_kernel<5, kNorm>), grid, block, 0, s, a); break;
        case 6: hipLaunchKernelGGL((composite_bwd_kernel<6, kNorm>), grid, block, 0, s, a); break;
        case 7: hipLaunchKernelGGL((composite_bwd_kernel<7, kNorm>), grid, block, 0, s, a); break;
        default: hipLaunchKernelGGL((composite_bwd_kernel<8, kNorm>), grid, block, 0, s, a); break;
    }
}

int launch_composite_bwd(const CompBwdArgs& a, hipStream_t s) {
    if (a.S < 2 || a.S > 64 * kMaxSpl) return fail(IDN_EUNSUPPORTED, "composite_bwd: n_samples %d outside [2, %d]", a.S, 64 * kMaxSpl);
    if (a.d_norm) launch_composite_bwd_spl<true>(a, s);
    else launch_composite_bwd_spl<false>(a, s);
    IDN_HIP_CHECK(hipGetLastError());
    return IDN_OK;
}

int launch_pass_bwd(const PassBwd& b, hipStream_t s) {
    const idn_facenerf_params& p = *b.p;
    const int64_t n_rays = b.n_rays; const int S = b.S;
    float* const d_rays = b.d_rays;
    const int64_t P = n_rays * S;
    const int64_t Pp = (P + 127) / 128 * 128;
    if (S < 2 || S > 64 * kMaxSpl) return fail(IDN_EUNSUPPORTED, "pass_bwd: n_samples %d outside [2, %d]", S, 64 * kMaxSpl);
    const BwdWs w = carve_bwd(reinterpret_cast<char*>(b.ws), Pp);
    if (!b.ws || b.ws_bytes < w.bytes) return fail(IDN_EWORKSPACE, "backward workspace %zu < %zu", b.ws_bytes, w.bytes);

    IDN_HIP_CHECK(hipMemsetAsync(w.dRGB, 0, (size_t)Pp * 64 * 4, s));
    if (Pp > P) IDN_HIP_CHECK(hipMemsetAsync(w.dV0 + (size_t)P * 256, 0, (size_t)(Pp - P) * 256 * 4, s));
    {
        CompBwdArgs a{reinterpret_cast<const float4*>(b.raw), b.z, b.rays, b.bc, b.g_rgb, b.g_fg, b.g_lw, b.g_acc,
                      w.dRGB, 64, w.dV0 + kSigmaChannel, 256, (long)n_rays, S, d_rays ? d_rays + 6 : nullptr, IDN_RAY_FLOATS};
        if (int e = launch_composite_bwd(a, s)) return e;
    }
    if (int e = bwd_tail(p, b.grads, b.cond, b.acts, P, Pp, w, s)) return e;
    if (d_rays) {
        float* d_x = w.dA[1];
        static_assert(IDN_PTS_CH + IDN_VIEWS_CH <= 256, "the input-row gradient fits a delta matrix");
        if (int e = launch_dx(p, w.dA[0], w.dA[5], w.dV0, P, Pp, d_x, 0, nullptr, s)) return e;
        return launch_ray_grad(d_x, pts_ch_of(p), views_ch_of(p), b.rays, b.z, n_rays, S, d_rays, s);
    }
    return IDN_OK;
}

__global__ __launch_bounds__(256) void head_seed_kernel(const float* g_out, long n, long p_pad, float* d_rgb, float* dv0) {
    const long idx = (long)blockIdx.x * 256 + threadIdx.x;
    const long p = idx >> 4;
    const int q = (int)(idx & 15);
    if (p >= p_pad) return;
    f32x4 v = {0.f, 0.f, 0.f, 0.f};
    if (q == 0 && p < n) v = f32x4{g_out[p * 4 + 0], g_out[p * 4 + 1], g_out[p * 4 + 2], 0.f};
    *reinterpret_cast<f32x4*>(d_rgb + p * 64 + 4 * q) = v;
    if (q == 0) dv0[p * 256 + kSigmaChannel] = p < n ? g_out[p * 4 + 3] : 0.f;
}

constexpr int kDxFrags = 2 * 64 + 16;
constexpr int kDxLds = kDxFrags * kFragBytes;
constexpr int kDxWaves = 16;
static_assert(kDxLds <= 160 * 1024, "the fragments must fit a CU's LDS");
struct DxArgs {
    const float* w0; int ld0;
    const float* w5; int ld5;
    const float* wv; int ldv;
    const float* dA0; const float* dA5; const float* dV0;
    long n, p_pad;
    float* d_x;
    int pts_ch, views_ch;
};
__global__ __launch_bounds__(64 * kDxWaves, 1) void dx_kernel(DxArgs a) {
    extern __shared__ __attribute__((aligned(16))) f32x4 dx_frag[];
    const int tid = threadIdx.x, lane = tid & 63;
    const int wave = __builtin_amdgcn_readfirstlane(tid >> 6);
    const int j = lane & 31, hh = lane >> 5;
    for (int e = tid; e < kDxFrags * 64; e += 64 * kDxWaves) {
        const int f = e >> 6, i = e & 31, h = (e >> 5) & 1;
        float v[4];
        for (int t = 0; t < 4; ++t) {
            if (f < 128) {
                const int g = f >> 1, col = 32 * (f & 1) + i, k = 8 * g + 4 * h + t;
                const float* row = k < IDN_W ? a.w0 + (long)k * a.ld0 : a.w5 + (long)(k - IDN_W) * a.ld5;
                v[t] = col < a.pts_ch ? row[col] : 0.f;
            } else {
                const int k = 8 * (f - 128) + 4 * h + t;
                v[t] = i < a.views_ch ? a.wv[(long)k * a.ldv + IDN_W + i] : 0.f;
            }
        }
        dx_frag[e] = f32x4{v[0], v[1], v[2], v[3]};
    }
    __syncthreads();
    const long ntiles = a.p_pad / 32;
    for (long tile = (long)blockIdx.x * kDxWaves + wave; tile < ntiles; tile += (long)gridDim.x * kDxWaves) {
        const long p = tile * 32 + j;
        f32x16 acc0, acc1, accv;
        for (int r = 0; r < 16; ++r) acc0[r] = acc1[r] = accv[r] = 0.f;
        const float* r0 = a.dA0 + p * 256 + 4 * hh;
        const float* r5 = a.dA5 + p * 256 + 4 * hh;
        const float* rv = a.dV0 + p * 256 + 4 * hh;
#pragma unroll 4
        for (int g = 0; g < 32; ++g) {
            const f32x4 d = *reinterpret_cast<const f32x4*>(r0 + 8 * g);
            const f32x4 w0 = dx_frag[(2 * g) * 64 + lane], w1 = dx_frag[(2 * g + 1) * 64 + lane];
#pragma unroll
            for (int t = 0; t < 4; ++t) {
                acc0 = mfma32(w0[t], d[t], acc0);
                acc1 = mfma32(w1[t], d[t], acc1);
            }
        }
#pragma unroll 4
        for (int g = 0; g < 32; ++g) {
            const f32x4 d = *reinterpret_cast<const f32x4*>(r5 + 8 * g);
            const f32x4 w0 = dx_frag[(64 + 2 * g) * 64 + lane], w1 = dx_frag[(64 + 2 * g + 1) * 64 + lane];
#pragma unroll
            for (int t = 0; t < 4; ++t) {
                acc0 = mfma32(w0[t], d[t], acc0);
                acc1 = mfma32(w1[t], d[t], acc1);
            }
        }
#pragma unroll 4
        for (int g = 0; g < 16; ++g) {
            const f32x4 d = *reinterpret_cast<const f32x4*>(rv + 8 * g);
            const f32x4 w = dx_frag[(128 + g) * 64 + lane];
#pragma unroll
            for (int t = 0; t < 4; ++t) accv = mfma32(w[t], d[t], accv);
        }
        if (p < a.n) {
            float* o = a.d_x + p * (a.pts_ch + a.views_ch);
#pragma unroll
            for (int r = 0; r < 16; ++r) {
                const int col = d_row(r, hh);
                if (col < a.pts_ch) o[col] = acc0[r];
                if (col < a.pts_ch - 32) o[32 + col] = acc1[r];
                if (col < a.views_ch) o[a.pts_ch + col] = accv[r];
            }
        }
    }
}

int launch_dx(const idn_facenerf_params& p, const float* dA0, const float* dA5, const float* dV0, int64_t n, int64_t Pp, float* d_x,
              int max_blocks, int* blocks_out, hipStream_t s) {
    static LaunchSetup setup;
    int num_cu = 0;
    if (int e = setup.get([]() -> int {
            IDN_HIP_CHECK(hipFuncSetAttribute(reinterpret_cast<const void*>(&dx_kernel), hipFuncAttributeMaxDynamicSharedMemorySize, kDxLds));
            return IDN_OK;
        }, &num_cu))
        return e;
    const int C = p.dim_aud + p.dim_expr + p.dim_latent;
    const int PC = pts_ch_of(p), VC = views_ch_of(p);
    const DxArgs da{p.pts_w[0], PC + C, p.pts_w[5], PC + C + IDN_W, p.views_w[0], IDN_W + VC + p.dim_expr,
                    dA0, dA5, dV0, (long)n, (long)Pp, d_x, PC, VC};
    const int64_t groups = (Pp / 32 + kDxWaves - 1) / kDxWaves;
    int grid = (int)(groups < num_cu ? groups : num_cu);
    if (max_blocks > 0 && grid > max_blocks) grid = max_blocks;
    hipLaunchKernelGGL(dx_kernel, dim3(grid), dim3(64 * kDxWaves), kDxLds, s, da);
    IDN_HIP_CHECK(hipGetLastError());
    if (blocks_out) *blocks_out = grid;
    return IDN_OK;
}

int launch_facenerf_bwd(const idn_facenerf_params& p, const idn_facenerf_grads& gr, const BwdCond& cond, const float* acts,
                        int64_t n, const float* g_out, float* d_x, void* ws_, size_t ws_bytes, hipStream_t s) {
    const int64_t Pp = (n + 127) / 128 * 128;
    const BwdWs w = carve_bwd(reinterpret_cast<char*>(ws_), Pp);
    if (!ws_ || ws_bytes < w.bytes) return fail(IDN_EWORKSPACE, "backward workspace %zu < %zu", ws_bytes, w.bytes);
    {
        const long threads = (long)Pp * 16;
        hipLaunchKernelGGL(head_seed_kernel, dim3((unsigned)((threads + 255) / 256)), dim3(256), 0, s, g_out, (long)n, (long)Pp,
                           w.dRGB, w.dV0);
        IDN_HIP_CHECK(hipGetLastError());
    }
    if (int e = bwd_tail(p, &gr, cond, acts, n, Pp, w, s)) return e;
    if (d_x) return launch_dx(p, w.dA[0], w.dA[5], w.dV0, n, Pp, d_x, 0, nullptr, s);
    return IDN_OK;
}

}
```

ideal-nerf_amd/ops.py:

```python
import contextlib
import ctypes as C
import os
from typing import Dict, Optional

import torch

from . import _lib
from ._lib import IDN_PREC_F32, RAY_FLOATS, IdealNerfError, check

PTS_CH, VIEWS_CH, W_HID = 63, 27, 256


def embed_channels(multires: int, views: bool = False) -> int:
    limit = _lib.MAX_MULTIRES_VIEWS if views else _lib.MAX_MULTIRES
    name = "multires_views" if views else "multires"
    if not 0 <= int(multires) <= limit:
        raise NotImplementedError(f"{name}={multires}: libidealnerf is compiled for {name} in 0..{limit} "
                                  f"({3 + 6 * limit} input channels at the most)")
    return 3 + 6 * int(multires)


def check_input_channels(input_ch: int, input_ch_views: int):
    for ch, name, flag, limit in ((input_ch, "input_ch", "multires", _lib.MAX_MULTIRES),
                                  (input_ch_views, "input_ch_views", "multires_views", _lib.MAX_MULTIRES_VIEWS)):
# ... 164 lines not shown


def facenerf_bwd(p, grads, aud, expr, latent, acts, g_out, d_x=None, d_aud=None, d_expr=None, d_latent=None):
    lib = _lib.load()
    _shape(g_out, "g_out", None, 4)
    n = g_out.shape[0]
    _shape(acts, "acts", lib.idealnerf_train_acts_floats(n))
    _shape(d_x, "d_x", n, sum(widths(p)))
    for t, name, dim in ((aud, "aud", p.dim_aud), (expr, "expr", p.dim_expr), (latent, "latent", p.dim_latent),
                         (d_aud, "d_aud", p.dim_aud), (d_expr, "d_expr", p.dim_expr), (d_latent, "d_latent", p.dim_latent)):
        _shape(t, name, dim)
    for k, t in grads.items():
        _ptr(t, f"grad {k}")
    with _Launch(aud, expr, latent, acts, g_out, d_x, d_aud, d_expr, d_latent, *grads.values()) as L:
        ptrs = [_ptr(t, name) for t, name in ((aud, "aud"), (expr, "expr"), (latent, "latent"), (acts, "acts"))]
        ptrs += [n, _ptr(g_out, "g_out")]
        ptrs += [_ptr(t, name) for t, name in ((d_x, "d_x"), (d_aud, "d_aud"), (d_expr, "d_expr"), (d_latent, "d_latent"))]
        ws = _workspace(lib.idealnerf_facenerf_bwd_workspace_bytes(n), g_out.device, L.stream)
        check(lib.idealnerf_facenerf_bwd(C.byref(p), C.byref(grads_struct(grads)), *ptrs, ws.data_ptr(), ws.numel(), L.stream))
    return grads


def query_rays_train_fwd(packed, folded, rays, z, precision=_lib.IDN_PREC_BF16X6, pts_ch=PTS_CH, views_ch=VIEWS_CH):
    lib = _lib.load()
    check_input_channels(pts_ch, views_ch)
    _shape(z, "z", None, None)
    n, S = z.shape
    _shape(rays, "rays", n, RAY_FLOATS)
    with _Launch(packed, folded, rays, z) as L:
        raw = torch.empty((n, S, 4), dtype=torch.float32, device=z.device)
        acts = torch.empty(lib.idealnerf_train_acts_floats(n * S), dtype=torch.float32, device=z.device)
        check(lib.idealnerf_query_rays_train_fwd_ch(_ptr(packed, "packed"), _ptr(folded, "folded"), precision, _ptr(rays, "rays"),
                                                    _ptr(z, "z"), n, S, pts_ch, views_ch, raw.data_ptr(), acts.data_ptr(), L.stream))
    return raw, acts


def _pass_bwd(p, grads, aud, expr, latent, acts, raw, z, rays, bc, g_rgb, g_fg, g_lw, g_acc, d_aud, d_latent, d_views0_bias=None,
              d_rays=None, with_rays=False, d_expr=None, ex=False):
    lib = _lib.load()
    if grads is None:
        grads = {}
    n, S = z.shape
    for t, name, shape in ((raw, "raw", (n, S, 4)), (rays, "rays", (n, RAY_FLOATS)), (bc, "bc_rgb", (n, 3)),
                           (g_rgb, "g_rgb_map", (n, 3)), (g_fg, "g_rgb_fg", (n, 3)), (g_lw, "g_last_weight", (n,)),
                           (g_acc, "g_acc", (n,)), (d_rays, "d_rays", (n, RAY_FLOATS)), (d_expr, "d_expr", (p.dim_expr,))):
        _shape(t, name, *shape)
    tensors = (aud, expr, latent, acts, raw, z, rays, bc, g_rgb, g_fg, g_lw, g_acc, d_aud, d_latent)
    with _Launch(*tensors, d_rays, d_expr, d_views0_bias if ex else None, *grads.values()) as L:
        ws = _workspace(lib.idealnerf_pass_bwd_workspace_bytes(n, S), z.device, L.stream)
        ptrs = [_ptr(t) for t in tensors]
        if ex:
            _shape(d_views0_bias, "d_views0_bias", W_HID // 2)
            extra = _lib.PassBwdExtra(_ptr(d_expr, "d_expr"), _ptr(d_rays, "d_rays"), _ptr(d_views0_bias, "d_views0_bias"))
            check(lib.idealnerf_pass_bwd_ex(C.byref(p), C.byref(grads_struct(grads)) if grads else None, *ptrs[:8], n, S, *ptrs[8:],
                                            C.byref(extra), ws.data_ptr(), ws.numel(), L.stream))
        elif with_rays:
            check(lib.idealnerf_pass_bwd_rays(C.byref(p), C.byref(grads_struct(grads)), *ptrs[:8], n, S, *ptrs[8:], _ptr(d_rays, "d_rays"),
                                              ws.data_ptr(), ws.numel(), L.stream))
        elif grads:
            check(lib.idealnerf_pass_bwd(C.byref(p), C.byref(grads_struct(grads)), *ptrs[:8], n, S, *ptrs[8:], ws.data_ptr(), ws.numel(), L.stream))
        else:
            check(lib.idealnerf_pass_bwd_cond(C.byref(p), *ptrs[:8], n, S, *ptrs[8:], ws.data_ptr(), ws.numel(), L.stream))
    return grads


def pass_bwd(p, grads, aud, expr, latent, acts, raw, z, rays, bc, g_rgb, g_fg, g_lw, g_acc, d_aud, d_latent):
    return _pass_bwd(p, grads, aud, expr, latent, acts, raw, z, rays, bc, g_rgb, g_fg, g_lw, g_acc, d_aud, d_latent)


def pass_bwd_rays(p, grads, aud, expr, latent, acts, raw, z, rays, bc, g_rgb, g_fg, g_lw, g_acc, d_aud, d_latent, d_rays):
    return _pass_bwd(p, grads, aud, expr, latent, acts, raw, z, rays, bc, g_rgb, g_fg, g_lw, g_acc, d_aud, d_latent,
                     d_rays=d_rays, with_rays=True)


def pass_bwd_cond(p, aud, expr, latent, acts, raw, z, rays, bc, g_rgb, g_fg, g_lw, g_acc, d_aud, d_latent, d_views0_bias=None):
    if d_views0_bias is not None and d_aud is None and d_latent is None:
        raise IdealNerfError("pass_bwd_cond: d_views0_bias needs d_aud or d_latent (with neither the pass is not run)")
    _pass_bwd(p, None, aud, expr, latent, acts, raw, z, rays, bc, g_rgb, g_fg, g_lw, g_acc, d_aud, d_latent, d_views0_bias,
              ex=d_views0_bias is not None)


def pass_bwd_ex(p, grads, aud, expr, latent, acts, raw, z, rays, bc, g_rgb, g_fg, g_lw, g_acc, d_aud, d_latent, d_expr=None,
                d_rays=None, d_views0_bias=None):
    return _pass_bwd(p, grads, aud, expr, latent, acts, raw, z, rays, bc, g_rgb, g_fg, g_lw, g_acc, d_aud, d_latent,
                     d_views0_bias=d_views0_bias, d_rays=d_rays, d_expr=d_expr, ex=True)


def query_rays_fwd(packed, folded, rays, z, precision=IDN_PREC_F32) -> torch.Tensor:
    lib = _lib.load()
    _shape(z, "z", None, None)
    n, S = z.shape
    _shape(rays, "rays", n, RAY_FLOATS)
    _net_buffers(lib, packed, folded, precision)
    with _Launch(packed, folded, rays, z) as L:
        raw = torch.empty((n, S, 4), dtype=torch.float32, device=z.device)
        check(lib.idealnerf_query_rays_fwd(_ptr(packed, "packed"), _ptr(folded, "folded"), precision, _ptr(rays, "rays"),
                                           _ptr(z, "z"), n, S, raw.data_ptr(), L.stream))
    return raw


def query_points_fwd(packed, folded, pts, viewdirs, precision=IDN_PREC_F32) -> torch.Tensor:
    lib = _lib.load()
    _shape(pts, "pts", None, None, 3)
    n, S, _ = pts.shape
    _shape(viewdirs, "viewdirs", n, 3)
    _net_buffers(lib, packed, folded, precision)
    with _Launch(packed, folded, pts, viewdirs) as L:
        raw = torch.empty((n, S, 4), dtype=torch.float32, device=pts.device)
        check(lib.idealnerf_query_points_fwd(_ptr(packed, "packed"), _ptr(folded, "folded"), precision, _ptr(pts, "pts"),
                                             _ptr(viewdirs, "viewdirs"), n, S, raw.data_ptr(), L.stream))
    return raw


def frame_rays(c2w, H, W, focal, near, far, row0=0, nrows=None, cx=None, cy=None, device="cuda") -> torch.Tensor:
    lib = _lib.load()
    nrows = H - row0 if nrows is None else nrows
    if not (0 <= row0 and 0 <= nrows and row0 + nrows <= H and W > 0):
        raise IdealNerfError(f"rows [{row0}, {row0 + nrows}) are outside a {H}x{W} frame")
    if tuple(c2w.shape[-2:]) not in ((3, 4), (4, 4)) or c2w.dim() != 2:
        raise IdealNerfError(f"c2w must be [3, 4] or [4, 4], got {list(c2w.shape)}")
    m = (C.c_float * 12)(*[float(v) for v in c2w[:3, :4].reshape(-1).tolist()])
    with _Launch(device=device) as L:
        out = torch.empty((nrows * W, RAY_FLOATS), dtype=torch.float32, device=L.device)
        check(lib.idealnerf_frame_rays(m, H, W, float(focal), -1.0 if cx is None else float(cx),
                                       -1.0 if cy is None else float(cy), float(near), float(far), row0, nrows,
                                       out.data_ptr(), L.stream))
    return out


def to8b(rgb, swap_rb=False, nonfinite_flag=None) -> torch.Tensor:
    lib = _lib.load()
    if rgb.shape[-1] != 3:
        raise IdealNerfError(f"to8b expects [..., 3], got {tuple(rgb.shape)}")
    if nonfinite_flag is not None and (nonfinite_flag.dtype != torch.int32 or not nonfinite_flag.is_cuda
                                       or nonfinite_flag.numel() < 1):
        raise IdealNerfError("nonfinite_flag must be an int32 device tensor")
    with _Launch(rgb, nonfinite_flag) as L:
        out = torch.empty(rgb.shape, dtype=torch.uint8, device=rgb.device)
        check(lib.idealnerf_to8b(_ptr(rgb, "rgb"), rgb.numel() // 3, int(bool(swap_rb)), out.data_ptr(),
                                 nonfinite_flag.data_ptr() if nonfinite_flag is not None else None, L.stream))
    return out


def compose_to8b(rgb_head, last_weight, rgb_fg, swap_rb=False, nonfinite_flag=None, want_fg=False):
    lib = _lib.load()
    if rgb_head.shape[-1] != 3:
        raise IdealNerfError(f"compose_to8b expects rgb_head [..., 3], got {tuple(rgb_head.shape)}")
    _shape(rgb_fg, "rgb_fg", *rgb_head.shape)
    _shape(last_weight, "last_weight", *rgb_head.shape[:-1])
    if nonfinite_flag is not None and (nonfinite_flag.dtype != torch.int32 or not nonfinite_flag.is_cuda
                                       or nonfinite_flag.numel() < 1):
        raise IdealNerfError("nonfinite_flag must be an int32 device tensor")
    with _Launch(rgb_head, last_weight, rgb_fg, nonfinite_flag) as L:
        ptrs = (_ptr(rgb_head, "rgb_head"), _ptr(last_weight, "last_weight"), _ptr(rgb_fg, "rgb_fg"))
        out = torch.empty(rgb_head.shape, dtype=torch.uint8, device=rgb_head.device)
        fg_out = torch.empty_like(out) if want_fg else None
        check(lib.idealnerf_compose_to8b(*ptrs, rgb_head.numel() // 3, int(bool(swap_rb)), out.data_ptr(),
                                         fg_out.data_ptr() if want_fg else None,
                                         nonfinite_flag.data_ptr() if nonfinite_flag is not None else None, L.stream))
    return (out, fg_out) if want_fg else out


def coarse_depths(rays, t_vals, t_rand=None, lindisp=False) -> torch.Tensor:
    lib = _lib.load()
    _shape(rays, "rays", None, RAY_FLOATS)
    _shape(t_vals, "t_vals", None)
    n, S = rays.shape[0], t_vals.shape[0]
    _shape(t_rand, "t_rand", n, S)
    with _Launch(rays, t_vals, t_rand) as L:
        z = torch.empty((n, S), dtype=torch.float32, device=rays.device)
        check(lib.idealnerf_coarse_depths(_ptr(rays, "rays"), _ptr(t_vals, "t_vals"), _ptr(t_rand, "t_rand"),
                                          int(bool(lindisp)), n, S, z.data_ptr(), L.stream))
    return z


def composite_fwd(raw, z, rays, bc_rgb, with_fg=False, with_weights=True, sigma_noise=None,
                  white_bkgd=False) -> Dict[str, torch.Tensor]:
    lib = _lib.load()
    _shape(z, "z", None, None)
    n, S = z.shape
    _shape(raw, "raw", n, S, 4)
    _shape(rays, "rays", n, RAY_FLOATS)
    _shape(bc_rgb, "bc_rgb", n, 3)
    _shape(sigma_noise, "sigma_noise", n, S)
    dev = z.device
    with _Launch(raw, z, rays, bc_rgb, sigma_noise) as L:
        new = lambda *s: torch.empty(s, dtype=torch.float32, device=dev)
        o = dict(rgb_map=new(n, 3), disp_map=new(n), acc_map=new(n), depth_map=new(n), last_weight=new(n))
        if with_weights:
            o["weights"] = new(n, S)
        if with_fg:
            o["rgb_fg"] = new(n, 3)
        co = _lib.CompositeOut(**{k: v.data_ptr() for k, v in o.items()})
        check(lib.idealnerf_composite_fwd(_ptr(raw, "raw"), _ptr(z, "z"), _ptr(rays, "rays"), _ptr(bc_rgb, "bc_rgb"),
                                          _ptr(sigma_noise, "sigma_noise"), int(bool(white_bkgd)), n, S, C.byref(co), L.stream))
    return o


def _u_shape(u, n, n_importance=None):
    if u.dim() == 2:
        _shape(u, "u", n, n_importance)
        return 1
    _shape(u, "u", n_importance)
    return 0


def sample_pdf_fwd(z, weights, u, n_importance) -> Dict[str, torch.Tensor]:
    lib = _lib.load()
    _shape(z, "z", None, None)
    n, S = z.shape
    _shape(weights, "weights", n, S)
    per_ray = _u_shape(u, n, n_importance)
    dev = z.device
    with _Launch(z, weights, u) as L:
        o = dict(z_samples=torch.empty((n, n_importance), dtype=torch.float32, device=dev),
                 inds=torch.empty((n, n_importance), dtype=torch.int64, device=dev),
                 cdf=torch.empty((n, S - 1), dtype=torch.float32, device=dev),
                 z_fine=torch.empty((n, S + n_importance), dtype=torch.float32, device=dev),
                 z_std=torch.empty((n,), dtype=torch.float32, device=dev))
        check(lib.idealnerf_sample_pdf_fwd(_ptr(z, "z"), _ptr(weights, "weights"), _ptr(u, "u"), per_ray, n, S,
                                           n_importance, o["z_samples"].data_ptr(), o["inds"].data_ptr(),
                                           o["cdf"].data_ptr(), o["z_fine"].data_ptr(), o["z_std"].data_ptr(), L.stream))
    return o


def march_fwd(raw, z, rays, bc_rgb, u, n_importance, with_fg=False, with_weights=False, sigma_noise=None,
              white_bkgd=False) -> Dict[str, torch.Tensor]:
    lib = _lib.load()
    _shape(z, "z", None, None)
    n, S = z.shape
    _shape(raw, "raw", n, S, 4)
    _shape(rays, "rays", n, RAY_FLOATS)
    _shape(bc_rgb, "bc_rgb", n, 3)
    _shape(sigma_noise, "sigma_noise", n, S)
    per_ray = _u_shape(u, n, n_importance)
    dev = z.device
    with _Launch(raw, z, rays, bc_rgb, u, sigma_noise) as L:
        new = lambda *s: torch.empty(s, dtype=torch.float32, device=dev)
        o = dict(rgb_map=new(n, 3), disp_map=new(n), acc_map=new(n), depth_map=new(n), last_weight=new(n))
        if with_weights:
            o["weights"] = new(n, S)
        if with_fg:
            o["rgb_fg"] = new(n, 3)
        co = _lib.CompositeOut(**{k: v.data_ptr() for k, v in o.items()})
        o.update(z_samples=new(n, n_importance), inds=torch.empty((n, n_importance), dtype=torch.int64, device=dev),
                 cdf=new(n, S - 1), z_fine=new(n, S + n_importance), z_std=new(n))
        check(lib.idealnerf_march_fwd(_ptr(raw, "raw"), _ptr(z, "z"), _ptr(rays, "rays"), _ptr(bc_rgb, "bc_rgb"),
                                      _ptr(sigma_noise, "sigma_noise"), int(bool(white_bkgd)), _ptr(u, "u"), per_ray, n, S,
                                      n_importance, C.byref(co), o["z_samples"].data_ptr(), o["inds"].data_ptr(),
                                      o["cdf"].data_ptr(), o["z_fine"].data_ptr(), o["z_std"].data_ptr(), L.stream))
    return o


def sample_pdf_bins_fwd(bins, weights, u) -> Dict[str, torch.Tensor]:
    lib = _lib.load()
    _shape(bins, "bins", None, None)
    n, nb = bins.shape
    _shape(weights, "weights", n, nb - 1)
    per_ray = _u_shape(u, n)
    ni = u.shape[-1]
    dev = bins.device
    with _Launch(bins, weights, u) as L:
        o = dict(z_samples=torch.empty((n, ni), dtype=torch.float32, device=dev),
                 inds=torch.empty((n, ni), dtype=torch.int64, device=dev),
                 cdf=torch.empty((n, nb), dtype=torch.float32, device=dev))
        check(lib.idealnerf_sample_pdf_bins_fwd(_ptr(bins, "bins"), _ptr(weights, "weights"), _ptr(u, "u"), per_ray, n,
                                                nb, ni, o["z_samples"].data_ptr(), o["inds"].data_ptr(),
                                                o["cdf"].data_ptr(), L.stream))
    return o


def invert_cdf(cdf, bins, u):
    lib = _lib.load()
    _shape(cdf, "cdf", None, None)
    n, nb = cdf.shape
    _shape(bins, "bins", n, nb)
    per_ray = _u_shape(u, n)
    ni = u.shape[-1]
    with _Launch(cdf, bins, u) as L:
        zs = torch.empty((n, ni), dtype=torch.float32, device=cdf.device)
        inds = torch.empty((n, ni), dtype=torch.int64, device=cdf.device)
        check(lib.idealnerf_invert_cdf(_ptr(cdf, "cdf"), _ptr(bins, "bins"), _ptr(u, "u"), per_ray, n, nb, ni,
                                       zs.data_ptr(), inds.data_ptr(), L.stream))
    return zs, inds


def dw_gemm(delta, acts, pipe=0, with_bias=True):
    lib = _lib.load()
    _shape(delta, "delta", None, None)
    rows = delta.shape[0]
    _shape(acts, "acts", rows, None)
    with _Launch(delta, acts) as L:
        dW = torch.empty((256, 256), dtype=torch.float32, device=delta.device)
        db = torch.empty(256, dtype=torch.float32, device=delta.device) if with_bias else None
        nbytes = lib.idealnerf_dw_gemm_workspace_bytes()
        ws = _workspace(nbytes, delta.device, L.stream)
        check(lib.idealnerf_dw_gemm(_ptr(delta, "delta"), delta.shape[1], _ptr(acts, "acts"), acts.shape[1], rows, dW.data_ptr(),
                                    None if db is None else db.data_ptr(), int(pipe), ws.data_ptr(), ws.numel(), L.stream))
    return dW, db


DW_SHAPES = ((256, 256), (256, 64), (128, 256), (128, 64), (128, 128), (64, 128))
DW_MAX_X6_ITEMS, DW_MAX_REDUCE_ITEMS = 12, 32


_dw_products_ws = {}


def dw_products(rows, products, pipe=0, x6_items=1):
    lib = _lib.load()
    E = IdealNerfError
    if not 1 <= len(products) <= _lib.DW_MAX_PRODUCTS:
        raise E(f"dw_products: {len(products)} products outside [1, {_lib.DW_MAX_PRODUCTS}]")
    if pipe not in (0, 1):
        raise E(f"dw_products: pipe {pipe}")
    if rows <= 0 or rows % 128:
        raise E(f"dw_products: rows {rows} is not a positive multiple of 128")
    if pipe == 0 and not 1 <= x6_items <= DW_MAX_X6_ITEMS:
        raise E(f"dw_products: x6_items {x6_items} outside [1, {DW_MAX_X6_ITEMS}]")
    n_x6 = n_red = 0
    tensors = []
    for i, t in enumerate(products):
        N, K = int(t["N"]), int(t["K"])
        if (N, K) not in DW_SHAPES:
            raise E(f"dw_products: product {i}: no instantiation for {N} x {K}")
        _shape(t["delta"], f"product {i}: delta", rows, None)
        _shape(t["acts"], f"product {i}: acts", rows, None)
        b_cols = K if t.get("acts2") is None else 128
        if t["delta"].shape[1] < N or t["acts"].shape[1] < b_cols:
            raise E(f"dw_products: product {i}: row pitch {t['delta'].shape[1]} / {t['acts'].shape[1]} < {N} / {b_cols}")
        d0 = int(t.get("delta_col0", 0))
        if d0 < 0 or d0 % 4 or d0 + N > t["delta"].shape[1]:
            raise E(f"dw_products: product {i}: delta columns {d0} .. {d0 + N} of {t['delta'].shape[1]}")
        x6 = pipe == 0 and (N, K) == (256, 256)
        if t.get("acts2") is not None:
            if not x6:
                raise E(f"dw_products: product {i}: a split B needs the 256 x 256 bf16-piece kernel")
            _shape(t["acts2"], f"product {i}: acts2", rows, t["acts"].shape[1])
        n_x6 += x6
        if n_x6 > x6_items:
            raise E(f"dw_products: more 256 x 256 products than x6_items ({x6_items})")
        takes, ctakes = t.get("takes", ()), t.get("colsum_takes", ())
        if len(takes) > _lib.DW_MAX_TAKES or len(ctakes) > _lib.DW_MAX_COLSUM_TAKES:
            raise E(f"dw_products: product {i}: {len(takes)} takes / {len(ctakes)} column-sum takes")
        if ctakes and not t.get("colsum"):
            raise E(f"dw_products: product {i} kept no column sums")
        n_red += len(takes) + len(ctakes)
        if n_red > DW_MAX_REDUCE_ITEMS:
            raise E(f"dw_products: more than {DW_MAX_REDUCE_ITEMS} takes in one pass")
        for j, (row0, col0, nr, nc, out, o_r, o_c) in enumerate(takes):
            if min(row0, col0) < 0 or min(nr, nc) < 1 or row0 + nr > N or col0 + nc > K:
                raise E(f"dw_products: product {i} take {j} leaves the {N} x {K} block")
            _shape(out, f"product {i} take {j}: out", None, None)
            if min(o_r, o_c) < 0 or o_r + nr > out.shape[0] or o_c + nc > out.shape[1]:
                raise E(f"dw_products: product {i} take {j} does not fit out {list(out.shape)}")
            tensors.append(out)
        for j, (col0, nc, out, o0) in enumerate(ctakes):
            if col0 < 0 or nc < 1 or col0 + nc > N:
                raise E(f"dw_products: product {i} column-sum take {j} leaves the {N} columns")
            _shape(out, f"product {i} column-sum take {j}: out", None)
            if o0 < 0 or o0 + nc > out.shape[0]:
                raise E(f"dw_products: product {i} column-sum take {j} does not fit out {list(out.shape)}")
            tensors.append(out)
        tensors += [t["delta"], t["acts"], t.get("acts2")]
    with _Launch(*tensors) as L:
        recs = (_lib.DwProduct * len(products))()
        for r, t in zip(recs, products):
            r.delta, r.ld_delta, r.N = _ptr(t["delta"], "delta") + 4 * int(t.get("delta_col0", 0)), t["delta"].shape[1], int(t["N"])
            r.acts, r.ld_acts, r.K = _ptr(t["acts"], "acts"), t["acts"].shape[1], int(t["K"])
            r.acts2, r.want_colsum = _ptr(t.get("acts2"), "acts2"), int(bool(t.get("colsum")))
            takes, ctakes = t.get("takes", ()), t.get("colsum_takes", ())
            r.n_takes, r.n_colsum_takes = len(takes), len(ctakes)
            for k, (row0, col0, nr, nc, out, o_r, o_c) in zip(r.takes, takes):
                k.row0, k.col0, k.rows, k.cols, k.ldo = row0, col0, nr, nc, out.shape[1]
                k.out = _ptr(out, "out") + 4 * (o_r * out.shape[1] + o_c)
            for k, (col0, nc, out, o0) in zip(r.colsum_takes, ctakes):
                k.col0, k.cols, k.out = col0, nc, _ptr(out, "out") + 4 * o0
        nbytes = lib.idealnerf_dw_products_workspace_bytes()
        key = (str(L.device), int(L.stream))
        ws = _dw_products_ws.get(key)
        if ws is None:
            ws = _dw_products_ws[key] = torch.zeros(nbytes, dtype=torch.uint8, device=L.device)
        check(lib.idealnerf_dw_products(rows, int(pipe), int(x6_items), recs, len(products), ws.data_ptr(), ws.numel(), L.stream))
        return [(r.splits, r.chunks_per_split) for r in recs]


_delta_chain_ws = {}


def delta_chain(p, pipe, acts, d_rgb, dv0, max_blocks=0, dv21=None, da=None):
    lib = _lib.load()
    E = IdealNerfError
    if not isinstance(p, _lib.FaceNerfParams):
        raise E("delta_chain: p must be a params_struct")
    if pipe not in (0, 1):
        raise E(f"delta_chain: pipe {pipe}")
    if isinstance(max_blocks, bool) or not isinstance(max_blocks, int) or max_blocks < 0:
        raise E(f"delta_chain: max_blocks {max_blocks} < 0")
    _shape(dv0, "dv0", None, 256)
    p_pad = dv0.shape[0]
    if p_pad <= 0 or p_pad % 128 or p_pad > 1 << 24:
        raise E(f"delta_chain: p_pad {p_pad} is not a positive multiple of 128 up to 2^24")
    _shape(acts, "acts", lib.idealnerf_train_acts_floats(p_pad))
    _shape(d_rgb, "d_rgb", p_pad, 64)
    _shape(dv21, "dv21", p_pad, 256)
    _shape(da, "da", 8, p_pad, 256)
    for t, name in ((acts, "acts"), (d_rgb, "d_rgb"), (dv0, "dv0"), (dv21, "dv21"), (da, "da")):
        if t is not None and t.dtype != torch.float32:
            raise E(f"{name} must be {torch.float32} (got {t.dtype})")
    with _Launch(acts, d_rgb, dv0, dv21, da) as L:
        ptrs = [_ptr(t, name) for t, name in ((acts, "acts"), (d_rgb, "d_rgb"), (dv0, "dv0"))]
        if dv21 is None:
            dv21 = torch.empty((p_pad, 256), dtype=torch.float32, device=L.device)
        if da is None:
            da = torch.empty((8, p_pad, 256), dtype=torch.float32, device=L.device)
        ptrs += [_ptr(dv21, "dv21"), _ptr(da, "da")]
        if any(q % 16 for q in ptrs):
            raise E("delta_chain: operands are not 16-byte aligned")
        key = str(L.device)
        ws = _delta_chain_ws.get(key)
        if ws is None:
            ws = _delta_chain_ws[key] = torch.zeros(lib.idealnerf_delta_chain_workspace_bytes(), dtype=torch.uint8, device=L.device)
        blocks = C.c_int(0)
        check(lib.idealnerf_delta_chain(C.byref(p), int(pipe), ptrs[0], p_pad, ptrs[1], ptrs[2], ptrs[3], ptrs[4], int(max_blocks),
                                        C.byref(blocks), ws.data_ptr(), ws.numel(), L.stream))
    return dv21, da, blocks.value


def composite_bwd(raw, z, rays, bc, g_rgb=None, g_fg=None, g_lw=None, g_acc=None, d_rgb=None, d_sig=None, sig_col=0, d_norm=None,
                  norm_col=0):
    lib = _lib.load()
    E = IdealNerfError
    if z is None:
        raise E("composite_bwd: z is None")
    _shape(z, "z", None, None)
    n, S = z.shape
    for t, name, shape in ((raw, "raw", (n, S, 4)), (rays, "rays", (n, RAY_FLOATS)), (bc, "bc_rgb", (n, 3)), (g_rgb, "g_rgb_map", (n, 3)),
                           (g_fg, "g_rgb_fg", (n, 3)), (g_lw, "g_last_weight", (n,)), (g_acc, "g_acc", (n,)), (d_rgb, "d_rgb", (None, None)),
                           (d_sig, "d_sig", (None, None)), (d_norm, "d_norm", (n, None))):
        if t is None and name in ("raw", "rays", "bc_rgb"):
            raise E(f"composite_bwd: {name} is None")
        _shape(t, name, *shape)
    if not 2 <= S <= 512:
        raise E(f"composite_bwd: n_samples {S} outside [2, 512]")
    if (d_rgb is None) != (d_sig is None):
        raise E("composite_bwd: d_rgb and d_sig come together")
    for t, name, col in ((d_sig, "sig_col", sig_col), (d_norm, "norm_col", norm_col)):
        if isinstance(col, bool) or not isinstance(col, int) or col < 0 or (t is None and col != 0) or (t is not None and col >= t.shape[1]):
            raise E(f"composite_bwd: {name} {col} is not a column of its matrix")
    if d_rgb is not None and (d_rgb.shape[0] < n * S or d_sig.shape[0] < n * S or d_rgb.shape[1] < 3):
        raise E(f"composite_bwd: d_rgb {list(d_rgb.shape)} / d_sig {list(d_sig.shape)} hold fewer than {n * S} rows or d_rgb fewer than 3 columns")
    with _Launch(raw, z, rays, bc, g_rgb, g_fg, g_lw, g_acc, d_rgb, d_sig, d_norm) as L:
        ptrs = [_ptr(t, name) for t, name in ((raw, "raw"), (z, "z"), (rays, "rays"), (bc, "bc_rgb"))]
        grad_ptrs = [_ptr(t, name) for t, name in ((g_rgb, "g_rgb_map"), (g_fg, "g_rgb_fg"), (g_lw, "g_last_weight"), (g_acc, "g_acc"))]
        if d_rgb is None:
            d_rgb = d_sig = torch.empty((n, S, 4), dtype=torch.float32, device=L.device)
            out = (d_rgb.data_ptr(), 4, d_rgb.data_ptr() + 12, 4)
        else:
            out = (_ptr(d_rgb, "d_rgb"), d_rgb.shape[1], _ptr(d_sig, "d_sig") + 4 * sig_col, d_sig.shape[1])
        norm = (None, 0) if d_norm is None else (_ptr(d_norm, "d_norm") + 4 * norm_col, d_norm.shape[1])
        check(lib.idealnerf_composite_bwd(*ptrs, n, S, *grad_ptrs, *out, *norm, L.stream))
    return d_rgb, d_sig, d_norm


def _all_f32(*named):
    for t, name in named:
        if t is not None and t.dtype != torch.float32:
            raise IdealNerfError(f"{name} must be {torch.float32} (got {t.dtype})")


def input_grad(p, dA0, dA5, dV0, n, d_x=None, max_blocks=0):
    lib = _lib.load()
    E = IdealNerfError
    if not isinstance(p, _lib.FaceNerfParams):
        raise E("input_grad: p must be a params_struct")
    if isinstance(max_blocks, bool) or not isinstance(max_blocks, int) or max_blocks < 0:
        raise E(f"input_grad: max_blocks {max_blocks} < 0")
    _shape(dA0, "dA0", None, 256)
    p_pad = dA0.shape[0]
    if p_pad <= 0 or p_pad % 128 or p_pad > 1 << 24:
        raise E(f"input_grad: p_pad {p_pad} is not a positive multiple of 128 up to 2^24")
    if isinstance(n, bool) or not isinstance(n, int) or not 1 <= n <= p_pad:
        raise E(f"input_grad: n {n} outside [1, p_pad = {p_pad}]")
    _shape(dA5, "dA5", p_pad, 256)
    _shape(dV0, "dV0", p_pad, 256)
    _shape(d_x, "d_x", n, sum(widths(p)))
    _all_f32((dA0, "dA0"), (dA5, "dA5"), (dV0, "dV0"), (d_x, "d_x"))
    with _Launch(dA0, dA5, dV0, d_x) as L:
        ptrs = [_ptr(t, name) for t, name in ((dA0, "dA0"), (dA5, "dA5"), (dV0, "dV0"))]
        if any(q % 16 for q in ptrs):
            raise E("input_grad: the delta matrices are not 16-byte aligned")
        if d_x is None:
            d_x = torch.empty((n, sum(widths(p))), dtype=torch.float32, device=L.device)
        blocks = C.c_int(0)
        check(lib.idealnerf_input_grad(C.byref(p), *ptrs, n, p_pad, _ptr(d_x, "d_x"), int(max_blocks), C.byref(blocks), L.stream))
    return d_x, blocks.value


def ray_grad(d_x, pts_ch, views_ch, rays, z, d_rays):
    lib = _lib.load()
    E = IdealNerfError
    for ch, name, limit in ((pts_ch, "pts_ch", PTS_CH), (views_ch, "views_ch", VIEWS_CH)):
        if isinstance(ch, bool) or not isinstance(ch, int) or ch < 3 or ch > limit or ch % 6 != 3:
            raise E(f"ray_grad: {name} {ch} is not 3 + 6 L up to {limit}")
    if z is None or d_rays is None:
        raise E("ray_grad: z / d_rays is None")
    _shape(z, "z", None, None)
    n, S = z.shape
    if not 2 <= S <= 512:
        raise E(f"ray_grad: n_samples {S} outside [2, 512]")
    for t, name, shape in ((d_x, "d_x", (n * S, pts_ch + views_ch)), (rays, "rays", (n, RAY_FLOATS)), (d_rays, "d_rays", (n, RAY_FLOATS))):
        if t is None:
            raise E(f"ray_grad: {name} is None")
        _shape(t, name, *shape)
    _all_f32((d_x, "d_x"), (rays, "rays"), (z, "z"), (d_rays, "d_rays"))
    with _Launch(d_x, rays, z, d_rays) as L:
        ptrs = [_ptr(t, name) for t, name in ((d_x, "d_x"), (rays, "rays"), (z, "z"), (d_rays, "d_rays"))]
        check(lib.idealnerf_ray_grad(ptrs[0], pts_ch, views_ch, ptrs[1], ptrs[2], n, S, ptrs[3], L.stream))
    return d_rays


def fold_bwd(p, aud, expr, latent, db0, db5, dbv, gW0=None, gW5=None, gWv0=None, d_aud=None, d_expr=None, d_latent=None):
    lib = _lib.load()
    E = IdealNerfError
    if not isinstance(p, _lib.FaceNerfParams):
        raise E("fold_bwd: p must be a params_struct")
    given = sum(t is not None for t in (gW0, gW5, gWv0))
    if given not in (0, 3):
        raise E(f"fold_bwd: {given} of the three gradient tensors (all three, or none)")
    pc, vc = widths(p)
    Cc = p.dim_aud + p.dim_expr + p.dim_latent
    for t, name, dim in ((aud, "aud", p.dim_aud), (expr, "expr", p.dim_expr), (latent, "latent", p.dim_latent)):
        if (t is None) != (dim == 0):
            raise E(f"fold_bwd: {name} is {'None' if t is None else 'given'} but the network's width is {dim}")
        _shape(t, name, dim)
    for t, name, dim in ((d_aud, "d_aud", p.dim_aud), (d_expr, "d_expr", p.dim_expr), (d_latent, "d_latent", p.dim_latent)):
        if t is not None and dim == 0:
            raise E(f"fold_bwd: {name} for a width of 0")
        _shape(t, name, dim)
    if db0 is None or db5 is None or (dbv is None and p.dim_expr > 0 and (given or d_expr is not None)):
        raise E("fold_bwd: db0 / db5 / dbv is None")
    for t, name, shape in ((db0, "db0", (W_HID,)), (db5, "db5", (W_HID,)), (dbv, "dbv", (W_HID // 2,)), (gW0, "gW0", (W_HID, pc + Cc)),
                           (gW5, "gW5", (W_HID, pc + Cc + W_HID)), (gWv0, "gWv0", (W_HID // 2, W_HID + vc + p.dim_expr))):
        _shape(t, name, *shape)
    named = ((aud, "aud"), (expr, "expr"), (latent, "latent"), (db0, "db0"), (db5, "db5"), (dbv, "dbv"), (gW0, "gW0"), (gW5, "gW5"),
             (gWv0, "gWv0"), (d_aud, "d_aud"), (d_expr, "d_expr"), (d_latent, "d_latent"))
    _all_f32(*named)
    with _Launch(*(t for t, _ in named)) as L:
        check(lib.idealnerf_fold_bwd(C.byref(p), *(_ptr(t, name) for t, name in named), L.stream))


_cond_colsums_ws = {}


def cond_colsums(dA0, dA5, dV0, P, db=None, dbv=None):
    lib = _lib.load()
    E = IdealNerfError
    if (dA0 is None) != (dA5 is None):
        raise E("cond_colsums: dA0 and dA5 come together")
    first = dA0 if dA0 is not None else dV0
    if first is None:
        raise E("cond_colsums: no matrix")
    _shape(first, "dA0" if dA0 is not None else "dV0", None, 256)
    p_pad = first.shape[0]
    if p_pad <= 0 or p_pad % 128 or p_pad > 1 << 24:
        raise E(f"cond_colsums: p_pad {p_pad} is not a positive multiple of 128 up to 2^24")
    if isinstance(P, bool) or not isinstance(P, int) or not 1 <= P <= p_pad:
        raise E(f"cond_colsums: P {P} outside [1, p_pad = {p_pad}]")
    if (db is not None and dA0 is None) or (dbv is not None and dV0 is None):
        raise E("cond_colsums: an output without its matrices")
    for t, name, shape in ((dA5, "dA5", (p_pad, 256)), (dV0, "dV0", (p_pad, 256)), (db, "db", (2, 256)), (dbv, "dbv", (128,))):
        _shape(t, name, *shape)
    named = ((dA0, "dA0"), (dA5, "dA5"), (dV0, "dV0"), (db, "db"), (dbv, "dbv"))
    _all_f32(*named)
    with _Launch(*(t for t, _ in named)) as L:
        ptrs = [_ptr(t, name) for t, name in named[:3]]
        if db is None and dA0 is not None:
            db = torch.empty((2, 256), dtype=torch.float32, device=L.device)
        if dbv is None and dV0 is not None:
            dbv = torch.empty((128,), dtype=torch.float32, device=L.device)
        key = (str(L.device), int(L.stream))
        ws = _cond_colsums_ws.get(key)
        if ws is None:
            ws = _cond_colsums_ws[key] = torch.zeros(lib.idealnerf_cond_colsums_workspace_bytes(), dtype=torch.uint8, device=L.device)
        check(lib.idealnerf_cond_colsums(*ptrs, P, p_pad, _ptr(db, "db"), _ptr(dbv, "dbv"), ws.data_ptr(), ws.numel(), L.stream))
    return db, dbv


AUDIO_NET_MAX_BWD_WINDOWS = 8


def _audio_params_struct(params, dim_aud):
    shapes = [(32, 29, 3), (32,), (32, 32, 3), (32,), (64, 32, 3), (64,), (64, 64, 3), (64,), (64, 64), (64,), (dim_aud, 64), (dim_aud,)]
    if len(params) != 12:
        raise IdealNerfError(f"AudioNet has 12 parameter tensors, got {len(params)}")
    for i, (t, shp) in enumerate(zip(params, shapes)):
        _shape(t, f"AudioNet parameter {i}", *shp)
    p = _lib.AudioNetParams()
    for i in range(4):
        p.conv_w[i], p.conv_b[i] = _ptr(params[2 * i], "conv weight"), _ptr(params[2 * i + 1], "conv bias")
    for i in range(2):
        p.fc_w[i], p.fc_b[i] = _ptr(params[8 + 2 * i], "fc weight"), _ptr(params[9 + 2 * i], "fc bias")
    p.dim_aud = int(dim_aud)
    return p


def audio_net_fwd(params, windows, dim_aud, save=False):
    lib = _lib.load()
    _shape(windows, "windows", None, 16, 29)
    n = windows.shape[0]
    with _Launch(windows, *params) as L:
        p = _audio_params_struct(params, dim_aud)
        out = torch.empty((n, dim_aud), dtype=torch.float32, device=windows.device)
        saved = torch.empty(lib.idealnerf_audio_net_saved_floats(n), dtype=torch.float32, device=windows.device) if save else None
        check(lib.idealnerf_audio_net_fwd(C.byref(p), _ptr(windows, "windows"), n, out.data_ptr(),
                                          None if saved is None else saved.data_ptr(), L.stream))
    return out, saved


def audio_net_bwd(params, windows, saved, d_out, dim_aud):
    lib = _lib.load()
    n = windows.shape[0]
    _shape(windows, "windows", None, 16, 29)
    _shape(d_out, "d_out", n, dim_aud)
    _shape(saved, "saved", lib.idealnerf_audio_net_saved_floats(n))
    with _Launch(windows, saved, d_out, *params) as L:
        p = _audio_params_struct(params, dim_aud)
        grads = [torch.empty_like(t) for t in params]
        g = _lib.AudioNetGrads()
        for i in range(4):
            g.conv_w[i], g.conv_b[i] = grads[2 * i].data_ptr(), grads[2 * i + 1].data_ptr()
        for i in range(2):
            g.fc_w[i], g.fc_b[i] = grads[8 + 2 * i].data_ptr(), grads[9 + 2 * i].data_ptr()
        check(lib.idealnerf_audio_net_bwd(C.byref(p), C.byref(g), _ptr(windows, "windows"), _ptr(saved, "saved"), _ptr(d_out, "d_out"),
                                          n, L.stream))
    return grads


SCORE_GROUPS = ("frame", "rect", "outside", "mouth", "torso")
SCORE_COLUMNS = ("n_pixels", "sse", "n_windows", "ssim_sum")
SCORE_TILE = _lib.SCORE_TILE


def frame_scores_workspace_doubles(H, W) -> int:
    return _lib.load().idealnerf_frame_scores_workspace_bytes(int(H), int(W)) // 8


def frame_scores(pred, truth_u8, regions=None, out=None, workspace=None) -> torch.Tensor:
    lib = _lib.load()
    if pred.dim() != 3 or pred.shape[-1] != 3:
        raise IdealNerfError(f"pred must be [H, W, 3], got {list(pred.shape)}")
    H, W = int(pred.shape[0]), int(pred.shape[1])
    _shape(truth_u8, "truth_u8", H, W, 3)
    _shape(regions, "regions", H, W)
    _shape(out, "out", 5, 4)
    with _Launch(pred, truth_u8, regions, out, workspace) as L:
        ptrs = (_ptr(pred, "pred"), _ptr(truth_u8, "truth_u8", torch.uint8), _ptr(regions, "regions", torch.uint8))
        need = lib.idealnerf_frame_scores_workspace_bytes(H, W)
        if out is None:
            out = torch.empty((5, 4), dtype=torch.float64, device=pred.device)
        if workspace is None:
            workspace = torch.empty(need // 8, dtype=torch.float64, device=pred.device)
        if workspace.numel() * 8 < need:
            raise IdealNerfError(f"workspace must hold {need // 8} float64 for a {H} x {W} frame, got {workspace.numel()}")
        check(lib.idealnerf_frame_scores(*ptrs, H, W, _ptr(out, "out", torch.float64), _ptr(workspace, "workspace", torch.float64),
                                         workspace.numel() * 8, L.stream))
    return out


def summarise_scores(table):
    import numpy as np
    t = np.asarray(table.detach().cpu() if isinstance(table, torch.Tensor) else table, dtype=np.float64)
    if t.ndim < 2 or t.shape[-2:] != (5, 4):
# ... 528 lines not shown
```

include/idealnerf.h:

```cpp
#ifndef IDEALNERF_H
#define IDEALNERF_H

#include <stddef.h>
#include <stdint.h>

#ifdef __cplusplus
extern "C" {
#endif

#define IDN_OK 0
#define IDN_EINVAL (-1)
#define IDN_EUNSUPPORTED (-2)
#define IDN_EHIP (-3)
#define IDN_EWORKSPACE (-4)

#define IDN_W 256
#define IDN_D 8
#define IDN_PTS_CH 63
#define IDN_VIEWS_CH 27
#define IDN_MAX_MULTIRES 10
#define IDN_MAX_MULTIRES_VIEWS 4
#define IDN_RAY_FLOATS 11

#define IDN_PREC_F32 0
#define IDN_PREC_BF16X3 1
#define IDN_PREC_BF16 2
#define IDN_PREC_FP16X3 3
#define IDN_PREC_BF16X6 4

int idealnerf_version(void);
const char* idealnerf_last_error(void);

size_t idealnerf_packed_weight_floats(int precision);
size_t idealnerf_folded_bias_floats(void);

typedef struct idn_facenerf_params {
    const float* pts_w[8];
    const float* pts_b[8];
    const float* views_w[3];
    const float* views_b[3];
    const float* alpha_w;
    const float* alpha_b;
    const float* rgb_w;
    const float* rgb_b;
    int dim_aud, dim_expr, dim_latent;
    int multires_plus1, multires_views_plus1;
} idn_facenerf_params;

int idealnerf_params_pts_ch(const idn_facenerf_params* p);
int idealnerf_params_views_ch(const idn_facenerf_params* p);

int idealnerf_pack_weights(const idn_facenerf_params* p, int precision, float* packed, void* stream);

int idealnerf_fold_conditioning(const idn_facenerf_params* p, const float* aud, const float* expr,
                                const float* latent, float* folded, void* stream);

int idealnerf_facenerf_fwd(const float* packed, const float* folded, int precision, const float* x,
                           int64_t n, float* out, void* stream);
int idealnerf_facenerf_fwd_ch(const float* packed, const float* folded, int precision, const float* x, int pts_ch,
                              int views_ch, int64_t n, float* out, void* stream);

int idealnerf_query_rays_fwd(const float* packed, const float* folded, int precision, const float* rays,
                             const float* z, int64_t n_rays, int n_samples, float* raw, void* stream);

int idealnerf_query_points_fwd(const float* packed, const float* folded, int precision, const float* pts,
                               const float* viewdirs, int64_t n_rays, int n_samples, float* raw, void* stream);

int idealnerf_frame_rays(const float* c2w, int H, int W, float focal, float cx, float cy, float near_, float far_,
                         int row0, int nrows, float* rays_out, void* stream);

int idealnerf_coarse_depths(const float* rays, const float* t_vals, const float* t_rand, int lindisp, int64_t n_rays,
                            int n_samples, float* z, void* stream);

typedef struct idn_composite_out {
    float* rgb_map;
    float* disp_map;
    float* acc_map;
    float* depth_map;
    float* weights;
    float* rgb_fg;
    float* last_weight;
} idn_composite_out;

int idealnerf_composite_fwd(const float* raw, const float* z, const float* rays, const float* bc_rgb,
                            const float* sigma_noise, int white_bkgd, int64_t n_rays, int n_samples,
                            const idn_composite_out* out, void* stream);

int idealnerf_sample_pdf_fwd(const float* z, const float* weights, const float* u, int u_per_ray,
                             int64_t n_rays, int n_samples, int n_importance, float* z_samples, int64_t* inds,
                             float* cdf, float* z_fine, float* z_std, void* stream);

int idealnerf_march_fwd(const float* raw, const float* z, const float* rays, const float* bc_rgb, const float* sigma_noise,
                        int white_bkgd, const float* u, int u_per_ray, int64_t n_rays, int n_samples, int n_importance,
                        const idn_composite_out* out, float* z_samples, int64_t* inds, float* cdf, float* z_fine,
                        float* z_std, void* stream);

int idealnerf_sample_pdf_bins_fwd(const float* bins, const float* weights, const float* u, int u_per_ray,
                                  int64_t n_rays, int n_bins, int n_importance, float* z_samples, int64_t* inds,
                                  float* cdf, void* stream);

int idealnerf_invert_cdf(const float* cdf, const float* bins, const float* u, int u_per_ray, int64_t n_rays,
                         int n_bins, int n_importance, float* z_samples, int64_t* inds, void* stream);

typedef struct idn_render_args {
    const float* rays;
    const float* bc_rgb;
    int64_t n_rays;
    int n_samples;
    int n_importance;
    int precision;
    const float* packed_coarse;
    const float* folded_coarse;
    const float* packed_fine;
    const float* folded_fine;
    const float* t_vals;
    const float* t_rand;
    const float* u;
    int u_per_ray;
    float* rgb_map;  float* disp_map;  float* acc_map;  float* depth_map;  float* last_weight;  float* rgb_fg;
    float* rgb0;     float* disp0;     float* acc0;     float* z_std;      float* last_weight0; float* rgb_fg0;
    float* tap_z_coarse;
    float* tap_raw_coarse;
    float* tap_weights_coarse;
    float* tap_cdf;
    int64_t* tap_inds;
    float* tap_z_samples;
    float* tap_z_fine;
    float* tap_raw_fine;
    float* tap_weights_fine;
    void* workspace;
    size_t workspace_bytes;
    int precision_fine_plus1;
    int lindisp;
    int white_bkgd;
    const float* noise_coarse;
    const float* noise_fine;
    int fused_march;
    int rng_mode;
    uint64_t rng_seed;
    int64_t rng_ray0;
} idn_render_args;

int idealnerf_philox_uniform(uint64_t seed, int which, int64_t row0, int64_t n_rows, int n_cols, float* out, void* stream);

#define IDN_SAMPLE_MAX_REGION 4096
size_t idealnerf_sample_pixels_workspace_bytes(void);
int idealnerf_sample_pixels(const uint8_t* region_map, int H, int W, int n_rect, int n_outside, int n_mouth, int n_torso,
                            uint64_t seed, uint64_t draw, void* workspace, size_t workspace_bytes, int64_t* sel, void* stream);

int idealnerf_gather_rays(const int64_t* sel, int64_t n, const float* c2w, int H, int W, float focal, float cx, float cy,
                          const uint8_t* image, const uint8_t* background, const float* target_table, const float* background_table,
                          float* batch_rays, float* target_s, float* bc_rgb, void* stream);

int idealnerf_gather_ray_pairs(const int64_t* sel, int64_t n, const float* c2w, const float* c2w_torso, int H, int W, float focal,
                               float cx, float cy, const uint8_t* image, const uint8_t* background, const float* target_table,
                               const float* background_table, float* batch_rays, float* batch_rays_torso, float* target_s,
                               float* bc_rgb, void* stream);

#define IDN_SCORE_TILE 32
size_t idealnerf_frame_scores_workspace_bytes(int H, int W);
int idealnerf_frame_scores(const float* pred, const uint8_t* truth, const uint8_t* regions, int H, int W, double* out,
                           void* workspace, size_t workspace_bytes, void* stream);

#define IDN_PATCH_MAX 16
#define IDN_PATCH_MIN_P 11
#define IDN_PATCH_MAX_P 48
typedef struct idn_patch_set {
    int n_patches;
    int p;
    int oy[IDN_PATCH_MAX];
    int ox[IDN_PATCH_MAX];
} idn_patch_set;
int idealnerf_patch_pixels(const idn_patch_set* set, int W, int64_t* sel_out, void* stream);
int idealnerf_ssim_patch_fwd(const float* pred, const float* truth, int n_patches, int p, double* out, void* stream);
int idealnerf_ssim_patch_bwd(const float* pred, const float* truth, int n_patches, int p, float g, float* d_pred, void* stream);

size_t idealnerf_render_workspace_bytes(int64_t n_rays, int n_samples, int n_importance);
int idealnerf_render_rays_fwd(const idn_render_args* a, void* stream);

typedef struct idn_frame {
    float c2w[12];
    int H, W;
    float focal, cx, cy;
    float near_, far_;
    int row0, nrows;
    float* rays_out;
} idn_frame;
size_t idealnerf_render_frame_workspace_bytes(int64_t n_rays, int n_samples, int n_importance);
int idealnerf_render_frame_fwd(const idn_render_args* a, const idn_frame* frame, void* stream);

typedef struct idn_render_opts {
    int colour_gate;
    int64_t* gate_counters;
} idn_render_opts;
int idealnerf_render_rays_fwd_opts(const idn_render_args* a, const idn_render_opts* opts, void* stream);
int idealnerf_render_frame_fwd_opts(const idn_render_args* a, const idn_frame* frame, const idn_render_opts* opts, void* stream);
float idealnerf_colour_gate_max_dist(void);


size_t idealnerf_train_acts_floats(int64_t n_points);

int idealnerf_query_rays_train_fwd(const float* packed, const float* folded, int precision, const float* rays,
                                   const float* z, int64_t n_rays, int n_samples, float* raw, float* acts,
                                   void* stream);
int idealnerf_query_rays_train_fwd_ch(const float* packed, const float* folded, int precision, const float* rays,
                                      const float* z, int64_t n_rays, int n_samples, int pts_ch, int views_ch, float* raw,
                                      float* acts, void* stream);

typedef struct idn_facenerf_grads {
    float* pts_w[8];
    float* pts_b[8];
    float* views_w[3];
    float* views_b[3];
    float* alpha_w;
    float* alpha_b;
    float* rgb_w;
    float* rgb_b;
} idn_facenerf_grads;

size_t idealnerf_pass_bwd_workspace_bytes(int64_t n_rays, int n_samples);

int idealnerf_pass_bwd(const idn_facenerf_params* p, const idn_facenerf_grads* grads, const float* aud,
                       const float* expr, const float* latent, const float* acts, const float* raw, const float* z,
                       const float* rays, const float* bc_rgb, int64_t n_rays, int n_samples, const float* g_rgb_map,
                       const float* g_rgb_fg, const float* g_last_weight, const float* g_acc, float* d_aud,
                       float* d_latent, void* workspace, size_t workspace_bytes, void* stream);

int idealnerf_pass_bwd_rays(const idn_facenerf_params* p, const idn_facenerf_grads* grads, const float* aud,
                            const float* expr, const float* latent, const float* acts, const float* raw, const float* z,
                            const float* rays, const float* bc_rgb, int64_t n_rays, int n_samples, const float* g_rgb_map,
                            const float* g_rgb_fg, const float* g_last_weight, const float* g_acc, float* d_aud,
                            float* d_latent, float* d_rays, void* workspace, size_t workspace_bytes, void* stream);

int idealnerf_pass_bwd_cond(const idn_facenerf_params* p, const float* aud, const float* expr, const float* latent,
                            const float* acts, const float* raw, const float* z, const float* rays, const float* bc_rgb,
                            int64_t n_rays, int n_samples, const float* g_rgb_map, const float* g_rgb_fg,
                            const float* g_last_weight, const float* g_acc, float* d_aud, float* d_latent, void* workspace,
                            size_t workspace_bytes, void* stream);

typedef struct idn_pass_bwd_extra {
    float* d_expr;
    float* d_rays;
    float* d_views0_bias;
} idn_pass_bwd_extra;

int idealnerf_pass_bwd_ex(const idn_facenerf_params* p, const idn_facenerf_grads* grads, const float* aud,
                          const float* expr, const float* latent, const float* acts, const float* raw, const float* z,
                          const float* rays, const float* bc_rgb, int64_t n_rays, int n_samples, const float* g_rgb_map,
                          const float* g_rgb_fg, const float* g_last_weight, const float* g_acc, float* d_aud,
                          float* d_latent, const idn_pass_bwd_extra* extra, void* workspace, size_t workspace_bytes,
                          void* stream);

int idealnerf_facenerf_train_fwd(const float* packed, const float* folded, int precision, const float* x, int64_t n,
                                 float* out, float* acts, void* stream);
int idealnerf_facenerf_train_fwd_ch(const float* packed, const float* folded, int precision, const float* x, int pts_ch,
                                    int views_ch, int64_t n, float* out, float* acts, void* stream);

size_t idealnerf_facenerf_bwd_workspace_bytes(int64_t n);

int idealnerf_facenerf_bwd(const idn_facenerf_params* p, const idn_facenerf_grads* grads, const float* aud, const float* expr,
                           const float* latent, const float* acts, int64_t n, const float* g_out, float* d_x, float* d_aud,
                           float* d_expr, float* d_latent, void* workspace, size_t workspace_bytes, void* stream);

#define IDN_DW_PIPE_BF16X6 0
#define IDN_DW_PIPE_F32 1
#define IDN_DW_PIPE_BF16X6_PASS 2
size_t idealnerf_dw_gemm_workspace_bytes(void);
int idealnerf_dw_gemm(const float* delta, int ld_delta, const float* acts, int ld_acts, int64_t rows, float* dW, float* db,
                      int pipe, void* workspace, size_t workspace_bytes, void* stream);

#define IDN_DW_MAX_PRODUCTS 16
#define IDN_DW_MAX_TAKES 4
#define IDN_DW_MAX_COLSUM_TAKES 2
typedef struct idn_dw_take {
    int row0, col0, rows, cols;
    float* out;
    int ldo;
} idn_dw_take;
typedef struct idn_dw_colsum_take {
    int col0, cols;
    float* out;
} idn_dw_colsum_take;
typedef struct idn_dw_product {
    const float* delta;
    int ld_delta, N;
    const float* acts;
    int ld_acts, K;
    const float* acts2;
    int want_colsum;
    int n_takes;
    idn_dw_take takes[IDN_DW_MAX_TAKES];
    int n_colsum_takes;
    idn_dw_colsum_take colsum_takes[IDN_DW_MAX_COLSUM_TAKES];
    int splits, chunks_per_split;
} idn_dw_product;
size_t idealnerf_dw_products_workspace_bytes(void);
int idealnerf_dw_products(int64_t rows, int pipe, int x6_items, idn_dw_product* products, int n, void* workspace,
                          size_t workspace_bytes, void* stream);

size_t idealnerf_delta_chain_workspace_bytes(void);
int idealnerf_delta_chain(const idn_facenerf_params* p, int pipe, const float* acts, int64_t p_pad, const float* d_rgb,
                          float* dv0, float* dv21, float* da, int max_blocks, int* blocks_out, void* workspace,
                          size_t workspace_bytes, void* stream);

int idealnerf_composite_bwd(const float* raw, const float* z, const float* rays, const float* bc_rgb, int64_t n_rays,
                            int n_samples, const float* g_rgb_map, const float* g_rgb_fg, const float* g_last_weight,
                            const float* g_acc, float* d_rgb, int ld_rgb, float* d_sig, int ld_sig, float* d_norm, int ld_norm,
                            void* stream);

int idealnerf_input_grad(const idn_facenerf_params* p, const float* dA0, const float* dA5, const float* dV0, int64_t n,
                         int64_t p_pad, float* d_x, int max_blocks, int* blocks_out, void* stream);
int idealnerf_ray_grad(const float* d_x, int pts_ch, int views_ch, const float* rays, const float* z, int64_t n_rays, int n_samples,
                       float* d_rays, void* stream);
int idealnerf_fold_bwd(const idn_facenerf_params* p, const float* aud, const float* expr, const float* latent, const float* db0,
                       const float* db5, const float* dbv, float* gW0, float* gW5, float* gWv0, float* d_aud, float* d_expr,
                       float* d_latent, void* stream);
size_t idealnerf_cond_colsums_workspace_bytes(void);
int idealnerf_cond_colsums(const float* dA0, const float* dA5, const float* dV0, int64_t P, int64_t p_pad, float* db, float* dbv,
                           void* workspace, size_t workspace_bytes, void* stream);

typedef struct idn_audio_net_params {
    const float* conv_w[4];
    const float* conv_b[4];
    const float* fc_w[2];
    const float* fc_b[2];
    int dim_aud;
} idn_audio_net_params;
typedef struct idn_audio_net_grads {
    float* conv_w[4];
    float* conv_b[4];
    float* fc_w[2];
    float* fc_b[2];
} idn_audio_net_grads;
size_t idealnerf_audio_net_saved_floats(int n_windows);
int idealnerf_audio_net_fwd(const idn_audio_net_params* p, const float* windows, int n_windows, float* out, float* saved,
                            void* stream);
int idealnerf_audio_net_bwd(const idn_audio_net_params* p, const idn_audio_net_grads* grads, const float* windows,
                            const float* saved, const float* d_out, int n_windows, void* stream);

int idealnerf_to8b(const float* rgb, int64_t n_pixels, int swap_rb, uint8_t* out, int* nonfinite_flag, void* stream);

int idealnerf_compose_to8b(const float* rgb_head, const float* last_weight, const float* rgb_fg, int64_t n_pixels,
                           int swap_rb, uint8_t* out, uint8_t* fg_out, int* nonfinite_flag, void* stream);

int idealnerf_cull_mark(const float* raw, int64_t n, float sigma_min, uint8_t* corners, void* stream);
int idealnerf_cull_cells(const uint8_t* corners, int G, int dilate, uint32_t* bits, void* stream);

typedef struct idn_cull_grid {
    const uint32_t* bits;
    int G;
    float lo[3];
    float cell;
} idn_cull_grid;
size_t idealnerf_cull_classify_workspace_bytes(int64_t n_pixels);
int idealnerf_cull_classify(const idn_cull_grid* grid, const idn_frame* frame, float dz, int K, int64_t* sel, int32_t* n_live,
                            void* workspace, size_t workspace_bytes, void* stream);
int idealnerf_cull_gather(const int64_t* sel, int64_t n, const idn_frame* frame, const float* bc, float* rays, float* bc_live,
                          void* stream);
#define IDN_CULL_MAX_OUTPUTS 12
typedef struct idn_cull_output {
    float* dense;
    const float* live;
    int channels;
    int fill_background;
    float value;
} idn_cull_output;
int idealnerf_cull_scatter(const int64_t* sel, int64_t n_live, int64_t n_pixels, const float* bc, const idn_cull_output* outputs,
                           int n_outputs, void* stream);

int idealnerf_cull_sample_classify(const idn_cull_grid* grid, const float* rays, const float* z, int64_t n, int S, int64_t* sel,
                                   int32_t* n_live, void* workspace, size_t workspace_bytes, void* stream);
int idealnerf_cull_sample_gather(const int64_t* sel, int64_t m, const float* rays, const float* z, int64_t n, int S, float* pts,
                                 float* dirs, void* stream);
int idealnerf_cull_sample_scatter(const int64_t* sel, int64_t m, const float* raw_live, int64_t n_points, float* raw, void* stream);

void idealnerf_profile_begin(void);
int idealnerf_profile_end(double* total_ms, int64_t* launches, int64_t* points);

#define IDN_PROF_MLP_FWD 0
#define IDN_PROF_MLP_FWD_SAVE 1
#define IDN_PROF_DELTA_CHAIN 2
#define IDN_PROF_DW_GEMM 3
#define IDN_PROF_DW_GEMM_X6 4
#define IDN_PROF_MLP_FWD_SAVE_X6 5
#define IDN_PROF_DELTA_CHAIN_X6 6
#define IDN_PROF_KINDS 7
int idealnerf_profile_end_kinds(double* total_ms, int64_t* launches, int64_t* points);

#ifdef __cplusplus
}
#endif
#endif
```

Baseline: 133.1 million.

## Fold narrow 64-column dW products into the bf16x6 GEMM batch as extra blocks

In the bf16x6 weight-gradient pass, the 256x64 products for the view-direction and x0 inputs are now computed as a fifth column block inside the matching 256x256 GEMM item, which shares the delta fragments. The first layer's product becomes a column-only x6 item, and the batch schedules by per-item block counts instead of uniform items. The aim is to drop separate f32 launches and re-reads of the delta matrix, and to balance the work across the batch. The cost is heavier kernel templating, more LDS per buffer, and an extended ABI struct.

```diff
diff --git a/ideal-nerf_amd/_lib.py b/ideal-nerf_amd/_lib.py
--- a/ideal-nerf_amd/_lib.py
+++ b/ideal-nerf_amd/_lib.py
@@ -91,7 +91,7 @@
     _fields_ = [("delta", fp), ("ld_delta", C.c_int), ("N", C.c_int), ("acts", fp), ("ld_acts", C.c_int), ("K", C.c_int),
                 ("acts2", fp), ("want_colsum", C.c_int), ("n_takes", C.c_int), ("takes", DwTake * DW_MAX_TAKES),
                 ("n_colsum_takes", C.c_int), ("colsum_takes", DwColsumTake * DW_MAX_COLSUM_TAKES),
-                ("splits", C.c_int), ("chunks_per_split", C.c_int)]
+                ("splits", C.c_int), ("chunks_per_split", C.c_int), ("acts_x", fp), ("ld_acts_x", C.c_int), ("x6_col", C.c_int)]
 
 
 PATCH_MAX, PATCH_MIN_P, PATCH_MAX_P = 16, 11, 48
diff --git a/ideal-nerf_amd/csrc/dw_gemm.h b/ideal-nerf_amd/csrc/dw_gemm.h
--- a/ideal-nerf_amd/csrc/dw_gemm.h
+++ b/ideal-nerf_amd/csrc/dw_gemm.h
@@ -15,11 +15,16 @@
     int chunks_per_split;
     float* cpart;
     int b_split, b_off0, b_off1;
+    const float* E; int lde;
+    int shape;
 };
+enum { kX6Full = 0, kX6Wide = 1, kX6Col = 2 };
+constexpr int x6_blocks_of(int shape) { return shape == kX6Full ? 4 : shape == kX6Wide ? 5 : 1; }
 constexpr int kMaxTnBatch = 12;
 struct TNBatch {
     TNArgs it[kMaxTnBatch];
-    int n, splits;
+    int end[kMaxTnBatch];
+    int n;
 };
 constexpr int kMaxReduceItems = 32;
 struct ReduceItem {
@@ -37,23 +42,28 @@
 enum { kPipeX6 = IDN_DW_PIPE_BF16X6, kPipeF32 = IDN_DW_PIPE_F32 };
 
 struct DwPassProduct { int N, K; bool colsum; int pipes; };
-constexpr int kOnX6 = 1 << kPipeX6, kOnF32 = 1 << kPipeF32, kOnBoth = kOnX6 | kOnF32;
-constexpr DwPassProduct kTrunk = {256, 256, true, kOnBoth};
+constexpr int kOnX6 = 1 << kPipeX6, kOnF32 = 1 << kPipeF32, kOnBoth = kOnX6 | kOnF32, kX6Item = 1 << 2 | kOnX6;
+constexpr DwPassProduct kTrunkX6 = {256, 256, true, kX6Item}, kTrunkF32 = {256, 256, true, kOnF32};
 constexpr DwPassProduct kPassProducts[] = {
     {64, 128, true, kOnBoth},
-    {256, 256, true, kOnX6}, {128, 128, true, kOnF32}, {128, 128, true, kOnF32},
-    kTrunk, {128, 64, false, kOnBoth},
-    kTrunk, kTrunk, kTrunk, {256, 64, false, kOnBoth}, kTrunk, kTrunk, kTrunk, kTrunk,
-    {256, 64, true, kOnBoth},
+    {256, 256, true, kX6Item}, {128, 128, true, kOnF32}, {128, 128, true, kOnF32},
+    {256, 320, true, kX6Item}, kTrunkF32, {128, 64, false, kOnF32},
+    kTrunkX6, kTrunkX6, kTrunkF32, kTrunkF32,
+    {256, 320, true, kX6Item}, kTrunkF32, {256, 64, false, kOnF32},
+    kTrunkX6, kTrunkX6, kTrunkX6, kTrunkX6, kTrunkF32, kTrunkF32, kTrunkF32, kTrunkF32,
+    {256, 64, true, kX6Item}, {256, 64, true, kOnF32},
 };
 constexpr size_t pass_sum(int pipe, int what) {
     size_t n = 0;
     for (const DwPassProduct& t : kPassProducts)
-        if (t.pipes >> pipe & 1) n += what == 0 ? (t.N == 256 && t.K == 256) : what == 1 ? (size_t)t.N * t.K : t.colsum ? t.N : 0;
+        if (t.pipes >> pipe & 1) {
+            const bool item = pipe == kPipeX6 && (t.pipes & kX6Item) == kX6Item;
+            n += what == 0 ? (item ? t.K / 64 : 0) : what == 1 ? (size_t)t.N * t.K : what == 2 ? (t.colsum ? t.N : 0) : item;
+        }
     return n;
 }
-constexpr int kX6ItemsPerPass = (int)pass_sum(kPipeX6, 0);
-static_assert(kX6ItemsPerPass == 9 && kX6ItemsPerPass <= kMaxTnBatch, "one x6 batch per pass");
+constexpr int kX6ItemsPerPass = (int)pass_sum(kPipeX6, 3), kX6BlocksPerPass = (int)pass_sum(kPipeX6, 0);
+static_assert(kX6ItemsPerPass == 10 && kX6ItemsPerPass <= kMaxTnBatch && kX6BlocksPerPass == 7 * 4 + 2 * 5 + 1, "one x6 batch per pass");
 
 constexpr int kMaxSplits = 256;
 constexpr int kColsumBlocks = 256;
@@ -66,9 +76,10 @@
 struct DwProduct { const float *part, *cpart; int splits, N, K, chunks_per_split; };
 
 struct DwPass {
-    DwPass(float* part, size_t part_floats, float* cpart, size_t cpart_floats, int64_t P, int pipe, int x6_items, hipStream_t s)
-        : part_next(part), part_left(part_floats), cpart_next(cpart), cpart_left(cpart_floats), P(P), pipe(pipe), x6_items(x6_items), s(s) {}
-    int product(const float* A, int lda, int N, const float* B, int ldb, int K, bool want_colsum, DwProduct* h, const float* B2 = nullptr);
+    DwPass(float* part, size_t part_floats, float* cpart, size_t cpart_floats, int64_t P, int pipe, int x6_blocks, hipStream_t s)
+        : part_next(part), part_left(part_floats), cpart_next(cpart), cpart_left(cpart_floats), P(P), pipe(pipe), x6_blocks(x6_blocks), s(s) {}
+    int product(const float* A, int lda, int N, const float* B, int ldb, int K, bool want_colsum, DwProduct* h, const float* B2 = nullptr,
+                const float* Bx = nullptr, int ldbx = 0, bool x6_col = false);
     int take(const DwProduct& h, int row0, int col0, int rows, int cols, float* out, int ldo);
     int take_colsum(const DwProduct& h, int col0, int cols, float* out);
     int finish();
@@ -77,9 +88,10 @@
     float* part_next; size_t part_left;
     float* cpart_next; size_t cpart_left;
     int64_t P;
-    int pipe, x6_items;
+    int pipe, x6_blocks;
     hipStream_t s;
-    TNBatch x6{{}, 0, 0};
+    TNBatch x6{{}, {}, 0};
+    int x6_named = 0;
     ReduceBatch red{{}, 0};
     int red_blocks = 0;
 };
diff --git a/ideal-nerf_amd/csrc/dw_gemm.hip b/ideal-nerf_amd/csrc/dw_gemm.hip
--- a/ideal-nerf_amd/csrc/dw_gemm.hip
+++ b/ideal-nerf_amd/csrc/dw_gemm.hip
@@ -258,8 +258,15 @@
     x6::split3(x0, x1, w1, w2, w3);
     p1 = __float_as_uint(w1), p2 = __float_as_uint(w2), p3 = __float_as_uint(w3);
 }
-constexpr int kX6BufBytes = 2 * 8 * 3 * kFragBytes;
-constexpr int kX6Lds = 2 * kX6BufBytes;
+typedef unsigned tn_u32x2 __attribute__((ext_vector_type(2)));
+constexpr int kX6TileBytes = 3 * kFragBytes;
+template <bool MAIN, bool EXTRA>
+struct X6Lay {
+    static constexpr int kOffE = (MAIN ? 16 : 8) * kX6TileBytes;
+    static constexpr int kBufBytes = kOffE + (EXTRA ? 2 : 0) * kX6TileBytes;
+};
+constexpr int kX6Lds = 2 * X6Lay<true, true>::kBufBytes;
+static_assert(kX6Lds <= 160 * 1024, "two buffers of the widest item fit a CU's LDS");
 
 struct X6Frag {
     f32x4 v;
@@ -272,17 +279,25 @@
     asm volatile("s_waitcnt lgkmcnt(%3)" : "+v"(f[0].v), "+v"(f[1].v), "+v"(f[2].v) : "n"(N) : "memory");
 }
 
+__device__ __forceinline__ void mfma_bf_vgpr(f32x16& c, const f32x4& a, const f32x4& b) {
+    asm volatile("v_mfma_f32_32x32x16_bf16 %0, %1, %2, %0" : "+v"(c) : "v"(a), "v"(b));
+}
+template <bool MAIN, bool EXTRA>
 __device__ __forceinline__ void gemm_tn_x6_item(const TNArgs& g, const int split, char* x6_smem) {
+    static_assert(MAIN || EXTRA, "an item computes something");
+    constexpr int kX6BufBytes = X6Lay<MAIN, EXTRA>::kBufBytes, kOffE = X6Lay<MAIN, EXTRA>::kOffE;
     const int tid = threadIdx.x, lane = tid & 63;
     const int w = __builtin_amdgcn_readfirstlane(tid >> 6);
     const int i = lane & 31, hh = lane >> 5;
     const int wr = w >> 1, wc = w & 1;
-    f32x16 acc[4][4];
-#pragma unroll
-    for (int a = 0; a < 4; ++a)
+    f32x16 acc[4][4], acce[4];
+#pragma unroll
+    for (int a = 0; a < 4; ++a) {
 #pragma unroll
         for (int b = 0; b < 4; ++b)
             for (int r = 0; r < 16; ++r) acc[a][b][r] = 0.f;
+        for (int r = 0; r < 16; ++r) acce[a][r] = 0.f;
+    }
 
     const long c_begin = (long)split * g.chunks_per_split;
     long c_end = c_begin + g.chunks_per_split;
@@ -293,14 +308,19 @@
         const uint64_t a64 = (uint64_t)(uintptr_t)ptr;
         return tn_i32x4{(int)(uint32_t)a64, (int)((uint32_t)(a64 >> 32) & 0xffffu), (int)0xfffffffcu, 0x00020000};
     };
+    constexpr int kVm = kTnRows + (MAIN ? kTnRows : 0) + (EXTRA ? 4 : 0) - 2;
     const tn_i32x4 rsrcA = make_rsrc(g.A + c_begin * kTnRows * (long)g.lda);
-    const tn_i32x4 rsrcB = make_rsrc(g.B + c_begin * kTnRows * (long)g.ldb);
+    const tn_i32x4 rsrcB = make_rsrc((MAIN ? g.B : g.A) + c_begin * kTnRows * (long)g.ldb);
+    const tn_i32x4 rsrcE = make_rsrc((EXTRA ? g.E : g.A) + c_begin * kTnRows * (long)g.lde);
     const int voff = tid * 4;
     const int voffB = g.b_split ? (tid < 128 ? g.b_off0 : g.b_off1) + (tid & 127) * 4 : voff;
-    const int rowA = g.lda * 4, rowB = g.ldb * 4;
-    float ra[kTnRows], rb[kTnRows];
+    const int voffE = (tid & 63) * 4;
+    const int rowA = g.lda * 4, rowB = g.ldb * 4, rowE = g.lde * 4;
+    float ra[kTnRows], rb[kTnRows], re[4];
 #pragma unroll
     for (int p = 0; p < kTnRows; ++p) ra[p] = rb[p] = 0.f;
+#pragma unroll
+    for (int p = 0; p < 4; ++p) re[p] = 0.f;
     auto load_row_at = [&](float& dst, const tn_i32x4& rsrc, int soff, int vo) {
         asm volatile("buffer_load_dword %0, %1, %2, %3 offen" : "+v"(dst) : "v"(vo), "s"(rsrc), "s"(soff) : "memory");
     };
@@ -309,10 +329,22 @@
         const int base = (rc < n_chunks ? rc : n_chunks - 1) * kTnRows;
 #pragma unroll
         for (int p = 0; p < kTnRows; ++p) load_row(ra[p], rsrcA, (base + p) * rowA);
-#pragma unroll
-        for (int p = 0; p < kTnRows; ++p) load_row_at(rb[p], rsrcB, (base + p) * rowB, voffB);
+        if constexpr (MAIN) {
+#pragma unroll
+            for (int p = 0; p < kTnRows; ++p) load_row_at(rb[p], rsrcB, (base + p) * rowB, voffB);
+        }
+        if constexpr (EXTRA) {
+#pragma unroll
+            for (int p = 0; p < 4; ++p) load_row_at(re[p], rsrcE, (base + 4 * w + p) * rowE, voffE);
+        }
     };
     char* const my_slot = x6_smem + (tid >> 5) * (3 * kFragBytes) + (tid & 31) * 16;
+    char* const e_slot = x6_smem + kOffE + ((tid & 63) >> 5) * kX6TileBytes + (w >> 1) * 512 + (tid & 31) * 16 + (w & 1) * 8;
+    unsigned pe[3][2];
+    auto e_store = [&](int buf, auto Q_) {
+        constexpr int q = decltype(Q_)::value;
+        *reinterpret_cast<tn_u32x2*>(e_slot + buf * kX6BufBytes + q * kFragBytes) = tn_u32x2{pe[q][0], pe[q][1]};
+    };
     auto split_store = [&](int buf, int X, const float (&r)[kTnRows]) {
         unsigned pw[3][8];
 #pragma unroll
@@ -335,42 +367,59 @@
     const uint32_t smem0 = (uint32_t)(uintptr_t)(__attribute__((address_space(3))) char*)x6_smem;
     const uint32_t a_base = smem0 + (4 * wr) * (3 * kFragBytes) + lane * 16;
     const uint32_t b_base = smem0 + (8 + 4 * wc) * (3 * kFragBytes) + lane * 16;
+    const uint32_t e_base = smem0 + kOffE + wc * kX6TileBytes + lane * 16;
 
     load_chunk(0);
 #pragma unroll
     for (int p = 0; p < kTnRows; ++p) asm volatile("s_waitcnt vmcnt(0)" : "+v"(ra[p]), "+v"(rb[p])::"memory");
+    if constexpr (EXTRA) asm volatile("s_waitcnt vmcnt(0)" : "+v"(re[0]), "+v"(re[1]), "+v"(re[2]), "+v"(re[3])::"memory");
     colsum();
     split_store(0, 0, ra);
-    split_store(0, 1, rb);
+    if constexpr (MAIN) split_store(0, 1, rb);
+    if constexpr (EXTRA) {
+        split3(re[0], re[1], pe[0][0], pe[1][0], pe[2][0]);
+        split3(re[2], re[3], pe[0][1], pe[1][1], pe[2][1]);
+        static_for<3>([&](auto Q) { e_store(0, Q); });
+    }
     load_chunk(1);
     asm volatile("s_waitcnt lgkmcnt(0)" ::: "memory");
     __builtin_amdgcn_s_barrier();
     asm volatile("" ::: "memory");
 
-    X6Frag fa[4][3], fb[4][3];
+    constexpr bool ROT = MAIN && EXTRA;
+    X6Frag fa[4][3], fb[4][3], fe[3];
+    auto issue_fa = [&](auto Row_, auto Set_, uint32_t pa) {
+        static_for<3>([&](auto Q) {
+            fa[decltype(Set_)::value][decltype(Q)::value].template issue<(decltype(Row_)::value * 3 + decltype(Q)::value) * kFragBytes>(pa);
+        });
+    };
+    auto issue_fe = [&](uint32_t pe_) {
+        static_for<3>([&](auto Q) { fe[decltype(Q)::value].template issue<decltype(Q)::value * kFragBytes>(pe_); });
+    };
     auto issue_first_row = [&](uint32_t pa, uint32_t pb) {
         static_for<3>([&](auto Q) { fa[0][decltype(Q)::value].template issue<decltype(Q)::value * kFragBytes>(pa); });
-        static_for<2>([&](auto Y) {
-            static_for<3>([&](auto Q) {
-                fb[decltype(Y)::value][decltype(Q)::value].template issue<(decltype(Y)::value * 3 + decltype(Q)::value) * kFragBytes>(pb);
+        if constexpr (MAIN) {
+            static_for<2>([&](auto Y) {
+                static_for<3>([&](auto Q) {
+                    fb[decltype(Y)::value][decltype(Q)::value].template issue<(decltype(Y)::value * 3 + decltype(Q)::value) * kFragBytes>(pb);
+                });
             });
-        });
+        }
     };
     issue_first_row(a_base, b_base);
 #pragma unroll 1
     for (int rc = 0; rc < n_chunks; ++rc) {
         const int buf = rc & 1;
-        const uint32_t pa = a_base + buf * kX6BufBytes, pb = b_base + buf * kX6BufBytes;
-        static_for<2>([&](auto Y) {
-            static_for<3>([&](auto Q) {
-                fb[decltype(Y)::value + 2][decltype(Q)::value].template issue<((decltype(Y)::value + 2) * 3 + decltype(Q)::value) * kFragBytes>(pb);
+        const uint32_t pa = a_base + buf * kX6BufBytes, pb = b_base + buf * kX6BufBytes, pe_ = e_base + buf * kX6BufBytes;
+        if constexpr (!MAIN) issue_fe(pe_);
+        if constexpr (MAIN) {
+            static_for<2>([&](auto Y) {
+                static_for<3>([&](auto Q) {
+                    fb[decltype(Y)::value + 2][decltype(Q)::value].template issue<((decltype(Y)::value + 2) * 3 + decltype(Q)::value) * kFragBytes>(pb);
+                });
             });
-        });
-        static_for<3>([&](auto X) {
-            static_for<3>([&](auto Q) {
-                fa[decltype(X)::value + 1][decltype(Q)::value].template issue<((decltype(X)::value + 1) * 3 + decltype(Q)::value) * kFragBytes>(pa);
-            });
-        });
+        }
+        static_for<ROT ? 1 : 3>([&](auto X) { issue_fa(ic<decltype(X)::value + 1>{}, ic<decltype(X)::value + 1>{}, pa); });
         auto mm2 = [&](int x, int y0, int y1) {
 #define X6_TERM(QA, QB)                                                   \
     acc[x][y0] = x6::mfma_bf(fa[x][QA].v, fb[y0][QB].v, acc[x][y0]);        \
@@ -378,16 +427,47 @@
             X6_TERM(0, 0) X6_TERM(0, 1) X6_TERM(1, 0) X6_TERM(1, 1) X6_TERM(0, 2) X6_TERM(2, 0)
 #undef X6_TERM
         };
-        x6_retire<15>(fa[0]);
-        x6_retire<15>(fb[0]);
-        x6_retire<15>(fb[1]);
-        mm2(0, 0, 1);
-        x6_retire<9>(fb[2]);
-        x6_retire<9>(fb[3]);
-        mm2(0, 2, 3);
-        x6_retire<0>(fa[1]);
-        x6_retire<0>(fa[2]);
-        x6_retire<0>(fa[3]);
+        auto mme0 = [&]() {
+#define X6_TERM(QA, QB) acce[0] = x6::mfma_bf(fa[0][QA].v, fe[QB].v, acce[0]);
+            X6_TERM(0, 0) X6_TERM(0, 1) X6_TERM(1, 0) X6_TERM(1, 1) X6_TERM(0, 2) X6_TERM(2, 0)
+#undef X6_TERM
+        };
+        auto mm2e = [&]() {
+#define X6_TERM(QA, QB)                                                \
+    acc[0][2] = x6::mfma_bf(fa[0][QA].v, fb[2][QB].v, acc[0][2]);        \
+    acc[0][3] = x6::mfma_bf(fa[0][QA].v, fb[3][QB].v, acc[0][3]);        \
+    mfma_bf_vgpr(acce[0], fa[0][QA].v, fe[QB].v);
+            X6_TERM(0, 0) X6_TERM(0, 1) X6_TERM(1, 0) X6_TERM(1, 1) X6_TERM(0, 2) X6_TERM(2, 0)
+#undef X6_TERM
+        };
+        if constexpr (MAIN) {
+            x6_retire<ROT ? 9 : 15>(fa[0]);
+            x6_retire<ROT ? 9 : 15>(fb[0]);
+            x6_retire<ROT ? 9 : 15>(fb[1]);
+            if constexpr (EXTRA) issue_fe(pe_);
+            mm2(0, 0, 1);
+            if constexpr (!ROT) {
+                x6_retire<9>(fb[2]);
+                x6_retire<9>(fb[3]);
+                mm2(0, 2, 3);
+                x6_retire<0>(fa[1]);
+                x6_retire<0>(fa[2]);
+                x6_retire<0>(fa[3]);
+            } else {
+                x6_retire<0>(fb[2]);
+                x6_retire<0>(fb[3]);
+                x6_retire<0>(fa[1]);
+                x6_retire<0>(fe);
+                mm2e();
+            }
+        } else {
+            x6_retire<9>(fa[0]);
+            x6_retire<9>(fe);
+            mme0();
+            x6_retire<0>(fa[1]);
+            x6_retire<0>(fa[2]);
+            x6_retire<0>(fa[3]);
+        }
         const unsigned live_mask = rc + 1 < n_chunks ? 0xffffffffu : 0u;
         const int nbase = (rc + 2 < n_chunks ? rc + 2 : n_chunks - 1) * kTnRows;
         char* const dst = my_slot + (buf ^ 1) * kX6BufBytes;
@@ -404,7 +484,7 @@
             if constexpr (sl < 24) {
                 constexpr int j = sl / 3, ph = sl % 3;
                 if constexpr (ph == 0) {
-                    asm volatile("s_waitcnt vmcnt(30)" : "+v"(r[2 * j]), "+v"(r[2 * j + 1])::"memory");
+                    asm volatile("s_waitcnt vmcnt(%2)" : "+v"(r[2 * j]), "+v"(r[2 * j + 1]) : "n"(kVm) : "memory");
                     const unsigned p1 = x6::cvt_pk_bf16(r[2 * j], r[2 * j + 1]);
                     pw[X][0][j] = p1;
                     t0 = r[2 * j] - __uint_as_float(p1 << 16);
@@ -432,17 +512,57 @@
                 store(ic<2>{}, ic<1>{});
             }
         };
+        auto eslice = [&](auto S_) {
+            constexpr int sl = decltype(S_)::value;
+            if constexpr (sl < 6) {
+                constexpr int j = sl / 3, ph = sl % 3;
+                if constexpr (ph == 0) {
+                    asm volatile("s_waitcnt vmcnt(%2)" : "+v"(re[2 * j]), "+v"(re[2 * j + 1]) : "n"(kVm) : "memory");
+                    const unsigned p1 = x6::cvt_pk_bf16(re[2 * j], re[2 * j + 1]);
+                    pe[0][j] = p1;
+                    t0 = re[2 * j] - __uint_as_float(p1 << 16);
+                    t1 = re[2 * j + 1] - __uint_as_float(p1 & 0xffff0000u);
+                } else if constexpr (ph == 1) {
+                    const unsigned p2 = x6::cvt_pk_bf16(t0, t1);
+                    pe[1][j] = p2;
+                    t0 = t0 - __uint_as_float(p2 << 16);
+                    t1 = t1 - __uint_as_float(p2 & 0xffff0000u);
+                    pe[2][j] = x6::cvt_pk_bf16(t0, t1);
+                } else {
+                    load_row_at(re[2 * j], rsrcE, (nbase + 4 * w + 2 * j) * rowE, voffE);
+                    load_row_at(re[2 * j + 1], rsrcE, (nbase + 4 * w + 2 * j + 1) * rowE, voffE);
+                    if constexpr (j == 1) e_store(buf ^ 1, ic<0>{});
+                }
+            } else if constexpr (sl < 8) {
+                e_store(buf ^ 1, ic<sl - 5>{});
+            }
+        };
+        constexpr int kMainPerRow = MAIN ? 24 : 0, kPerRow = kMainPerRow + (EXTRA ? 6 : 0), kMfmas = 3 * kPerRow;
+        constexpr int kSlA = 26, kSlB = MAIN ? 26 : 0, kSlices = kSlA + kSlB + (EXTRA ? 8 : 0);
+        constexpr int kBar = MAIN ? kMfmas - 13 : kMfmas - 4, SPM = (kSlices + kBar - 1) / kBar;
+        static_assert(SPM * kBar >= kSlices && (MAIN && !EXTRA ? kBar == 59 && SPM == 1 : true), "every slice ahead of the chunk barrier");
         __builtin_amdgcn_sched_barrier(0);
-        static_for<72>([&](auto K_) {
+        static_for<kMfmas>([&](auto K_) {
             constexpr int k = decltype(K_)::value;
-            constexpr int x = 1 + k / 24, kk = k % 24, y = 2 * (kk / 12) + (kk % 2), t = (kk % 12) / 2;
+            constexpr int x = 1 + k / kPerRow, kk = k % kPerRow;
+            constexpr bool main = MAIN && !(EXTRA && kk % 5 == 4);
+            constexpr int m = EXTRA ? kk - kk / 5 : kk;
+            constexpr int y = 2 * (m / 12) + (m % 2), t = main ? (m % 12) / 2 : MAIN ? kk / 5 : kk;
             constexpr int qa = t == 2 || t == 3 ? 1 : (t == 5 ? 2 : 0);
             constexpr int qb = t == 1 || t == 3 ? 1 : (t == 4 ? 2 : 0);
-            acc[x][y] = x6::mfma_bf(fa[x][qa].v, fb[y][qb].v, acc[x][y]);
-            constexpr int kX1 = 26;
-            if constexpr (k < kX1) slice(ic<0>{}, ic<k>{});
-            else slice(ic<1>{}, ic<k - kX1>{});
-            if constexpr (k == 59) {
+            constexpr int fx = ROT ? (x & 1) : x;
+            if constexpr (ROT && kk == 0 && x >= 2) x6_retire<0>(fa[fx]);
+            if constexpr (main) acc[x][y] = x6::mfma_bf(fa[fx][qa].v, fb[y][qb].v, acc[x][y]);
+            else if constexpr (MAIN) mfma_bf_vgpr(acce[x], fa[fx][qa].v, fe[qb].v);
+            else acce[x] = x6::mfma_bf(fa[fx][qa].v, fe[qb].v, acce[x]);
+            if constexpr (ROT && kk == 0 && x < 3) issue_fa(ic<x + 1>{}, ic<(x + 1) & 1>{}, pa);
+            static_for<SPM>([&](auto J_) {
+                constexpr int sl = k * SPM + decltype(J_)::value;
+                if constexpr (sl < kSlA) slice(ic<0>{}, ic<sl>{});
+                else if constexpr (sl < kSlA + kSlB) slice(ic<1>{}, ic<sl - kSlA>{});
+                else if constexpr (sl < kSlices) eslice(ic<sl - kSlA - kSlB>{});
+            });
+            if constexpr (k == kBar) {
                 asm volatile("s_waitcnt lgkmcnt(0)" ::: "memory");
                 __builtin_amdgcn_s_barrier();
                 asm volatile("" ::: "memory");
@@ -452,25 +572,41 @@
         });
     }
     x6_retire<0>(fa[0]);
-    x6_retire<0>(fb[0]);
-    x6_retire<0>(fb[1]);
+    if constexpr (MAIN) {
+        x6_retire<0>(fb[0]);
+        x6_retire<0>(fb[1]);
+    }
 #pragma unroll
     for (int p = 0; p < kTnRows; ++p) asm volatile("s_waitcnt vmcnt(0)" : "+v"(ra[p]), "+v"(rb[p])::"memory");
+    if constexpr (EXTRA) asm volatile("s_waitcnt vmcnt(0)" : "+v"(re[0]), "+v"(re[1]), "+v"(re[2]), "+v"(re[3])::"memory");
     if (do_colsum) g.cpart[(long)split * g.N + tid] = csum + csum1;
     float* out = g.part + (long)split * g.N * g.K;
 #pragma unroll
-    for (int x = 0; x < 4; ++x)
-#pragma unroll
-        for (int y = 0; y < 4; ++y)
+    for (int x = 0; x < 4; ++x) {
+        if constexpr (MAIN) {
+#pragma unroll
+            for (int y = 0; y < 4; ++y)
+#pragma unroll
+                for (int r = 0; r < 16; ++r)
+                    out[(long)(32 * (4 * wr + x) + d_row(r, hh)) * g.K + 32 * (4 * wc + y) + i] = acc[x][y][r];
+        }
+        if constexpr (EXTRA) {
 #pragma unroll
             for (int r = 0; r < 16; ++r)
-                out[(long)(32 * (4 * wr + x) + d_row(r, hh)) * g.K + 32 * (4 * wc + y) + i] = acc[x][y][r];
+                out[(long)(32 * (4 * wr + x) + d_row(r, hh)) * g.K + (MAIN ? 256 : 0) + 32 * wc + i] = acce[x][r];
+        }
+    }
 }
 __global__ __launch_bounds__(256) void gemm_tn_x6_kernel(TNBatch b) {
     extern __shared__ __attribute__((aligned(16))) char x6_smem[];
-    const int item = __builtin_amdgcn_readfirstlane((int)blockIdx.z / b.splits);
-    const int split = __builtin_amdgcn_readfirstlane((int)blockIdx.z - item * b.splits);
-    gemm_tn_x6_item(b.it[item], split, x6_smem);
+    const int z = __builtin_amdgcn_readfirstlane((int)blockIdx.z);
+    int item = 0;
+    while (item + 1 < b.n && z >= b.end[item]) ++item;
+    const int split = z - (item ? b.end[item - 1] : 0);
+    const TNArgs& g = b.it[item];
+    if (g.shape == kX6Full) gemm_tn_x6_item<true, false>(g, split, x6_smem);
+    else if (g.shape == kX6Wide) gemm_tn_x6_item<true, true>(g, split, x6_smem);
+    else gemm_tn_x6_item<false, true>(g, split, x6_smem);
 }
 
 __global__ __launch_bounds__(256) void reduce_batch_kernel(ReduceBatch b) {
@@ -531,33 +667,42 @@
     }, cus);
 }
 
-int DwPass::product(const float* A, int lda, int N, const float* B, int ldb, int K, bool want_colsum, DwProduct* h, const float* B2) {
+int DwPass::product(const float* A, int lda, int N, const float* B, int ldb, int K, bool want_colsum, DwProduct* h, const float* B2,
+                    const float* Bx, int ldbx, bool x6_col) {
     const DwShape* sh = nullptr;
-    if (N == 256 && K == 256 && pipe == kPipeX6) sh = &kX6Shape;
+    int shape = -1;
+    if (pipe == kPipeX6 && N == 256 && K == 256) shape = Bx ? kX6Wide : kX6Full;
+    else if (pipe == kPipeX6 && N == 256 && K == 64 && x6_col) shape = kX6Col;
+    if (shape >= 0) sh = &kX6Shape;
     else
         for (const DwShape& t : kF32Shapes)
             if (t.N == N && t.K == K) sh = &t;
     if (!sh) return fail(IDN_EUNSUPPORTED, "gemm_tn: no instantiation for %d x %d", N, K);
     const bool queued = sh->launch == nullptr;
     if (B2 && !queued) return fail(IDN_EINVAL, "gemm_tn: a split B needs the 256 x 256 bf16-piece kernel");
+    if (Bx && shape != kX6Wide) return fail(IDN_EINVAL, "gemm_tn: an extra column block needs the 256 x 256 bf16-piece kernel");
     if (P % sh->rows_per_chunk) return fail(IDN_EINVAL, "gemm_tn: %lld rows are not a multiple of the %d-row chunk", (long long)P, sh->rows_per_chunk);
     const long chunks = P / sh->rows_per_chunk;
     int splits = sh->max_splits;
     if (queued) {
-        if (x6.n >= x6_items || x6.n >= kMaxTnBatch) return fail(IDN_EINVAL, "gemm_tn: more 256 x 256 products than the pass declared (%d)", x6_items);
+        const int blocks = x6_blocks_of(shape);
+        if (x6_named + blocks > x6_blocks || x6.n >= kMaxTnBatch)
+            return fail(IDN_EINVAL, "gemm_tn: more bf16-piece products than the pass declared (%d blocks of 64 columns)", x6_blocks);
+        x6_named += blocks;
         int cus = 0;
         if (int e = x6_setup(&cus)) return e;
-        splits = 2 * cus / x6_items;
+        splits = (int)((long)2 * cus * blocks / x6_blocks);
         if (splits > kMaxSplits) splits = kMaxSplits;
     }
     if (splits > chunks) splits = (int)chunks;
     if (splits < 1) splits = 1;
     const int cps = (int)((chunks + splits - 1) / splits);
     splits = (int)((chunks + cps - 1) / cps);
-    const size_t part_floats = (size_t)splits * N * K, cpart_floats = want_colsum ? (size_t)splits * N : 0;
+    const int Kp = shape == kX6Wide ? K + 64 : K;
+    const size_t part_floats = (size_t)splits * N * Kp, cpart_floats = want_colsum ? (size_t)splits * N : 0;
     if (part_floats > part_left || cpart_floats > cpart_left)
-        return fail(IDN_EWORKSPACE, "gemm_tn: the partial blocks of %d x %d in %d splits do not fit the pool", N, K, splits);
-    TNArgs g{A, lda, B, ldb, part_next, N, K, (long)P, cps, want_colsum ? cpart_next : nullptr, 0, 0, 0};
+        return fail(IDN_EWORKSPACE, "gemm_tn: the partial blocks of %d x %d in %d splits do not fit the pool", N, Kp, splits);
+    TNArgs g{A, lda, B, ldb, part_next, N, Kp, (long)P, cps, want_colsum ? cpart_next : nullptr, 0, 0, 0, nullptr, 0, shape};
     if (B2) {
         const float* base = B < B2 ? B : B2;
         const int64_t o0 = (int64_t)(B - base) * 4, o1 = (int64_t)(B2 - base) * 4;
@@ -565,14 +710,16 @@
         g.B = base, g.b_split = 1;
         g.b_off0 = (int)o0, g.b_off1 = (int)o1;
     }
+    if (shape == kX6Wide) g.E = Bx, g.lde = ldbx;
+    if (shape == kX6Col) g.E = B, g.lde = ldb, g.B = nullptr, g.ldb = 0;
     if (queued) {
-        x6.splits = splits;
+        x6.end[x6.n] = (x6.n ? x6.end[x6.n - 1] : 0) + splits;
         x6.it[x6.n++] = g;
     } else {
         ProfScope prof(s, P, IDN_PROF_DW_GEMM);
         if (int e = sh->launch(g, splits, s)) return e;
     }
-    *h = DwProduct{g.part, g.cpart, splits, N, K, cps};
+    *h = DwProduct{g.part, g.cpart, splits, N, Kp, cps};
     part_next += part_floats, part_left -= part_floats;
     cpart_next += cpart_floats, cpart_left -= cpart_floats;
     return IDN_OK;
@@ -592,7 +739,7 @@
 int DwPass::finish() {
     if (x6.n) {
         ProfScope prof(s, P * x6.n, IDN_PROF_DW_GEMM_X6);
-        hipLaunchKernelGGL(gemm_tn_x6_kernel, dim3(1, 1, x6.splits * x6.n), dim3(256), kX6Lds, s, x6);
+        hipLaunchKernelGGL(gemm_tn_x6_kernel, dim3(1, 1, x6.end[x6.n - 1]), dim3(256), kX6Lds, s, x6);
     }
     IDN_HIP_CHECK(hipGetLastError());
     if (red.n) hipLaunchKernelGGL(reduce_batch_kernel, dim3(red_blocks), dim3(256), 0, s, red);
@@ -605,13 +752,13 @@
                    void* ws, size_t ws_bytes, hipStream_t s) {
     if (rows <= 0 || rows % 128) return fail(IDN_EINVAL, "dw_gemm: rows %lld is not a positive multiple of 128", (long long)rows);
     if (ld_delta < 256 || ld_acts < 256) return fail(IDN_EINVAL, "dw_gemm: row pitch < 256");
-    const int x6_items = pipe == IDN_DW_PIPE_BF16X6_PASS ? kX6ItemsPerPass : 1;
+    const int x6_blocks = pipe == IDN_DW_PIPE_BF16X6_PASS ? kX6BlocksPerPass : x6_blocks_of(kX6Full);
     if (pipe == IDN_DW_PIPE_BF16X6_PASS) pipe = IDN_DW_PIPE_BF16X6;
     if (pipe != IDN_DW_PIPE_BF16X6 && pipe != IDN_DW_PIPE_F32) return fail(IDN_EINVAL, "dw_gemm: pipe %d", pipe);
     if (!ws || ws_bytes < dw_gemm_workspace_bytes()) return fail(IDN_EWORKSPACE, "dw_gemm workspace %zu < %zu", ws_bytes, dw_gemm_workspace_bytes());
     float* part = reinterpret_cast<float*>(ws);
     float* cpart = reinterpret_cast<float*>(reinterpret_cast<char*>(ws) + al256((size_t)kMaxSplits * 65536 * 4));
-    DwPass q(part, (size_t)kMaxSplits * 65536, cpart, (size_t)kColsumBlocks * 256, rows, pipe, x6_items, s);
+    DwPass q(part, (size_t)kMaxSplits * 65536, cpart, (size_t)kColsumBlocks * 256, rows, pipe, x6_blocks, s);
     DwProduct h;
     if (int e = q.product(delta, ld_delta, 256, acts, ld_acts, 256, db != nullptr, &h)) return e;
     int e = db ? q.take_colsum(h, 0, 256, db) : IDN_OK;
@@ -624,16 +771,26 @@
     if (!pr) return fail(IDN_EINVAL, "dw_products: NULL pointer");
     if (n < 1 || n > IDN_DW_MAX_PRODUCTS) return fail(IDN_EINVAL, "dw_products: %d products outside [1, %d]", n, IDN_DW_MAX_PRODUCTS);
     if (pipe != kPipeX6 && pipe != kPipeF32) return fail(IDN_EINVAL, "dw_products: pipe %d", pipe);
-    if (rows <= 0 || rows % 128) return fail(IDN_EINVAL, "dw_products: rows %lld is not a positive multiple of 128", (long long)rows);
+    bool folded_only = pipe == kPipeX6;
+    for (int i = 0; i < n; ++i) folded_only = folded_only && (pr[i].acts_x || pr[i].x6_col);
+    if (rows <= 0 || rows % (folded_only ? kTnRows : 128))
+        return fail(IDN_EINVAL, "dw_products: rows %lld is not a positive multiple of 128", (long long)rows);
     if (rows > (int64_t)1 << 24) return fail(IDN_EUNSUPPORTED, "dw_products: rows %lld exceed 2^24", (long long)rows);
-    if (pipe == kPipeX6 && (x6_items < 1 || x6_items > kMaxTnBatch))
+    if (pipe == kPipeX6 && x6_items != IDN_DW_X6_PASS_SHARES && (x6_items < 1 || x6_items > kMaxTnBatch))
         return fail(IDN_EINVAL, "dw_products: x6_items %d outside [1, %d]", x6_items, kMaxTnBatch);
-    int n_x6 = 0, n_red = 0;
+    const int x6_blocks = x6_items == IDN_DW_X6_PASS_SHARES ? kX6BlocksPerPass : x6_items * x6_blocks_of(kX6Full);
+    int n_x6 = 0, n_blocks = 0, n_red = 0;
     size_t part_per_split = 0, cpart_per_split = 0;
     for (int i = 0; i < n; ++i) {
         const idn_dw_product& t = pr[i];
         if (!t.delta || !t.acts) return fail(IDN_EINVAL, "dw_products: product %d: NULL pointer", i);
-        const bool x6 = t.N == 256 && t.K == 256 && pipe == kPipeX6;
+        const bool x6_col = t.x6_col && t.N == 256 && t.K == 64 && pipe == kPipeX6;
+        const bool x6 = (t.N == 256 && t.K == 256 && pipe == kPipeX6) || x6_col;
+        if (t.x6_col && !x6_col) return fail(IDN_EINVAL, "dw_products: product %d: x6_col names a 256 x 64 product of the bf16-piece pipe", i);
+        if (t.acts_x && (!x6 || x6_col)) return fail(IDN_EINVAL, "dw_products: product %d: an extra column block needs the 256 x 256 bf16-piece kernel", i);
+        if (t.acts_x && (t.ld_acts_x < 64 || t.ld_acts_x % 4 || (uintptr_t)t.acts_x % 16))
+            return fail(IDN_EINVAL, "dw_products: product %d: the extra column block's pitch %d (or its alignment)", i, t.ld_acts_x);
+        const int Kp = t.K + (t.acts_x ? 64 : 0);
         bool known = x6;
         for (const DwShape& sh : kF32Shapes) known = known || (sh.N == t.N && sh.K == t.K);
         if (!known) return fail(IDN_EUNSUPPORTED, "dw_products: product %d: no instantiation for %d x %d", i, t.N, t.K);
@@ -646,7 +803,9 @@
             const uintptr_t lo = (uintptr_t)(t.acts < t.acts2 ? t.acts : t.acts2), hi = (uintptr_t)(t.acts < t.acts2 ? t.acts2 : t.acts);
             if (hi - lo >= (uintptr_t)1 << 31) return fail(IDN_EUNSUPPORTED, "dw_products: product %d: split B matrices more than 2 GiB apart", i);
         }
-        if (x6 && ++n_x6 > x6_items) return fail(IDN_EINVAL, "dw_products: more 256 x 256 products than x6_items (%d)", x6_items);
+        if (x6) n_blocks += x6_blocks_of(x6_col ? kX6Col : t.acts_x ? kX6Wide : kX6Full);
+        if (x6 && (++n_x6 > kMaxTnBatch || n_blocks > x6_blocks))
+            return fail(IDN_EINVAL, "dw_products: more 256 x 256 products than x6_items (%d)", x6_items);
         if (t.n_takes < 0 || t.n_takes > IDN_DW_MAX_TAKES || t.n_colsum_takes < 0 || t.n_colsum_takes > IDN_DW_MAX_COLSUM_TAKES)
             return fail(IDN_EINVAL, "dw_products: product %d: %d takes / %d column-sum takes", i, t.n_takes, t.n_colsum_takes);
         if (t.n_colsum_takes && !t.want_colsum) return fail(IDN_EINVAL, "dw_products: product %d kept no column sums", i);
@@ -655,8 +814,8 @@
         for (int j = 0; j < t.n_takes; ++j) {
             const idn_dw_take& k = t.takes[j];
             if (!k.out) return fail(IDN_EINVAL, "dw_products: product %d take %d: NULL pointer", i, j);
-            if (k.row0 < 0 || k.col0 < 0 || k.rows < 1 || k.cols < 1 || k.row0 + k.rows > t.N || k.col0 + k.cols > t.K || k.ldo < k.cols)
-                return fail(IDN_EINVAL, "dw_products: product %d take %d leaves the %d x %d block (or its pitch is short)", i, j, t.N, t.K);
+            if (k.row0 < 0 || k.col0 < 0 || k.rows < 1 || k.cols < 1 || k.row0 + k.rows > t.N || k.col0 + k.cols > Kp || k.ldo < k.cols)
+                return fail(IDN_EINVAL, "dw_products: product %d take %d leaves the %d x %d block (or its pitch is short)", i, j, t.N, Kp);
         }
         for (int j = 0; j < t.n_colsum_takes; ++j) {
             const idn_dw_colsum_take& k = t.colsum_takes[j];
@@ -664,7 +823,7 @@
             if (k.col0 < 0 || k.cols < 1 || k.col0 + k.cols > t.N)
                 return fail(IDN_EINVAL, "dw_products: product %d column-sum take %d leaves the %d columns", i, j, t.N);
         }
-        part_per_split += (size_t)t.N * t.K;
+        part_per_split += (size_t)t.N * Kp;
         cpart_per_split += t.want_colsum ? t.N : 0;
     }
     if (part_per_split > kPartFloatsPerSplit || cpart_per_split * kMaxSplits > kCpartPoolFloats)
@@ -673,11 +832,12 @@
         return fail(IDN_EWORKSPACE, "dw_products workspace %zu < %zu", ws_bytes, dw_products_workspace_bytes());
     float* part = reinterpret_cast<float*>(ws);
     float* cpart = reinterpret_cast<float*>(reinterpret_cast<char*>(ws) + al256(kPartPoolFloats * 4));
-    DwPass q(part, kPartPoolFloats, cpart, kCpartPoolFloats, rows, pipe, x6_items, s);
+    DwPass q(part, kPartPoolFloats, cpart, kCpartPoolFloats, rows, pipe, x6_blocks, s);
     for (int i = 0; i < n; ++i) {
         idn_dw_product& t = pr[i];
         DwProduct h;
-        if (int e = q.product(t.delta, t.ld_delta, t.N, t.acts, t.ld_acts, t.K, t.want_colsum != 0, &h, t.acts2)) return e;
+        if (int e = q.product(t.delta, t.ld_delta, t.N, t.acts, t.ld_acts, t.K, t.want_colsum != 0, &h, t.acts2, t.acts_x, t.ld_acts_x, t.x6_col != 0))
+            return e;
         for (int j = 0; j < t.n_colsum_takes; ++j)
             if (int e = q.take_colsum(h, t.colsum_takes[j].col0, t.colsum_takes[j].cols, t.colsum_takes[j].out)) return e;
         for (int j = 0; j < t.n_takes; ++j) {
diff --git a/ideal-nerf_amd/csrc/train.hip b/ideal-nerf_amd/csrc/train.hip
--- a/ideal-nerf_amd/csrc/train.hip
+++ b/ideal-nerf_amd/csrc/train.hip
@@ -316,7 +316,8 @@
         return launch_fold_bwd(f, true, s);
     }
     const idn_facenerf_grads& gr = *grads;
-    DwPass q(w.part, kPartPoolFloats, w.cpart, kCpartPoolFloats, Pp, pipe, kX6ItemsPerPass, s);
+    DwPass q(w.part, kPartPoolFloats, w.cpart, kCpartPoolFloats, Pp, pipe, kX6BlocksPerPass, s);
+    const bool x6 = pipe == kPipeX6;
     DwProduct h;
     TRY(q.product(w.dRGB, 64, 64, v_l(3), 128, 128, true, &h));
     TRY(q.take_colsum(h, 0, 3, gr.rgb_b));
@@ -334,23 +335,23 @@
             TRY(q.take(h, 0, 0, 128, 128, gr.views_w[l], 128));
         }
     }
-    TRY(q.product(w.dV0, 256, 256, a_l(8), 256, 256, true, &h));
+    TRY(q.product(w.dV0, 256, 256, a_l(8), 256, 256, true, &h, nullptr, x6 ? act(kActDir) : nullptr, 64));
     TRY(q.take_colsum(h, 0, 128, gr.views_b[0]));
     TRY(q.take_colsum(h, kSigmaChannel, 1, gr.alpha_b));
     TRY(q.take(h, 0, 0, 128, 256, gr.views_w[0], ldv));
     TRY(q.take(h, kSigmaChannel, 0, 1, 256, gr.alpha_w, 256));
-    TRY(q.product(w.dV0, 256, 128, act(kActDir), 64, 64, false, &h));
-    TRY(q.take(h, 0, 0, 128, VC, gr.views_w[0] + IDN_W, ldv));
+    if (!x6) TRY(q.product(w.dV0, 256, 128, act(kActDir), 64, 64, false, &h));
+    TRY(q.take(h, 0, x6 ? 256 : 0, 128, VC, gr.views_w[0] + IDN_W, ldv));
     for (int l = 7; l >= 1; --l) {
-        TRY(q.product(w.dA[l], 256, 256, a_l(l), 256, 256, true, &h));
+        TRY(q.product(w.dA[l], 256, 256, a_l(l), 256, 256, true, &h, nullptr, x6 && l == 5 ? act(kActX0) : nullptr, 64));
         TRY(q.take_colsum(h, 0, 256, gr.pts_b[l]));
         TRY(q.take(h, 0, 0, 256, 256, l == 5 ? gr.pts_w[5] + PC + C : gr.pts_w[l], l == 5 ? ld5 : 256));
         if (l == 5) {
-            TRY(q.product(w.dA[5], 256, 256, act(kActX0), 64, 64, false, &h));
-            TRY(q.take(h, 0, 0, 256, PC, gr.pts_w[5], ld5));
-        }
-    }
-    TRY(q.product(w.dA[0], 256, 256, act(kActX0), 64, 64, true, &h));
+            if (!x6) TRY(q.product(w.dA[5], 256, 256, act(kActX0), 64, 64, false, &h));
+            TRY(q.take(h, 0, x6 ? 256 : 0, 256, PC, gr.pts_w[5], ld5));
+        }
+    }
+    TRY(q.product(w.dA[0], 256, 256, act(kActX0), 64, 64, true, &h, nullptr, nullptr, 0, x6));
     TRY(q.take_colsum(h, 0, 256, gr.pts_b[0]));
     TRY(q.take(h, 0, 0, 256, PC, gr.pts_w[0], ld0));
     TRY(q.finish());
diff --git a/ideal-nerf_amd/ops.py b/ideal-nerf_amd/ops.py
--- a/ideal-nerf_amd/ops.py
+++ b/ideal-nerf_amd/ops.py
@@ -490,6 +490,7 @@
 
 DW_SHAPES = ((256, 256), (256, 64), (128, 256), (128, 64), (128, 128), (64, 128))
 DW_MAX_X6_ITEMS, DW_MAX_REDUCE_ITEMS = 12, 32
+DW_X6_PASS_SHARES = -1
 
 
 _dw_products_ws = {}
@@ -502,9 +503,10 @@
         raise E(f"dw_products: {len(products)} products outside [1, {_lib.DW_MAX_PRODUCTS}]")
     if pipe not in (0, 1):
         raise E(f"dw_products: pipe {pipe}")
-    if rows <= 0 or rows % 128:
+    folded_only = pipe == 0 and all(t.get("acts_x") is not None or t.get("x6_col") for t in products)
+    if rows <= 0 or rows % (16 if folded_only else 128):
         raise E(f"dw_products: rows {rows} is not a positive multiple of 128")
-    if pipe == 0 and not 1 <= x6_items <= DW_MAX_X6_ITEMS:
+    if pipe == 0 and x6_items != DW_X6_PASS_SHARES and not 1 <= x6_items <= DW_MAX_X6_ITEMS:
         raise E(f"dw_products: x6_items {x6_items} outside [1, {DW_MAX_X6_ITEMS}]")
     n_x6 = n_red = 0
     tensors = []
@@ -520,13 +522,23 @@
         d0 = int(t.get("delta_col0", 0))
         if d0 < 0 or d0 % 4 or d0 + N > t["delta"].shape[1]:
             raise E(f"dw_products: product {i}: delta columns {d0} .. {d0 + N} of {t['delta'].shape[1]}")
-        x6 = pipe == 0 and (N, K) == (256, 256)
+        x6_col = bool(t.get("x6_col"))
+        if x6_col and (pipe != 0 or (N, K) != (256, 64)):
+            raise E(f"dw_products: product {i}: x6_col names a 256 x 64 product of the bf16-piece pipe")
+        x6 = pipe == 0 and ((N, K) == (256, 256) or x6_col)
+        if t.get("acts_x") is not None:
+            if not x6 or x6_col:
+                raise E(f"dw_products: product {i}: an extra column block needs the 256 x 256 bf16-piece kernel")
+            _shape(t["acts_x"], f"product {i}: acts_x", rows, None)
+            if t["acts_x"].shape[1] < 64:
+                raise E(f"dw_products: product {i}: acts_x has {t['acts_x'].shape[1]} columns < 64")
+            K += 64
         if t.get("acts2") is not None:
             if not x6:
                 raise E(f"dw_products: product {i}: a split B needs the 256 x 256 bf16-piece kernel")
             _shape(t["acts2"], f"product {i}: acts2", rows, t["acts"].shape[1])
         n_x6 += x6
-        if n_x6 > x6_items:
+        if x6_items != DW_X6_PASS_SHARES and n_x6 > x6_items:
             raise E(f"dw_products: more 256 x 256 products than x6_items ({x6_items})")
         takes, ctakes = t.get("takes", ()), t.get("colsum_takes", ())
         if len(takes) > _lib.DW_MAX_TAKES or len(ctakes) > _lib.DW_MAX_COLSUM_TAKES:
@@ -550,13 +562,16 @@
             if o0 < 0 or o0 + nc > out.shape[0]:
                 raise E(f"dw_products: product {i} column-sum take {j} does not fit out {list(out.shape)}")
             tensors.append(out)
-        tensors += [t["delta"], t["acts"], t.get("acts2")]
+        tensors += [t["delta"], t["acts"], t.get("acts2"), t.get("acts_x")]
     with _Launch(*tensors) as L:
         recs = (_lib.DwProduct * len(products))()
         for r, t in zip(recs, products):
             r.delta, r.ld_delta, r.N = _ptr(t["delta"], "delta") + 4 * int(t.get("delta_col0", 0)), t["delta"].shape[1], int(t["N"])
             r.acts, r.ld_acts, r.K = _ptr(t["acts"], "acts"), t["acts"].shape[1], int(t["K"])
             r.acts2, r.want_colsum = _ptr(t.get("acts2"), "acts2"), int(bool(t.get("colsum")))
+            if t.get("acts_x") is not None:
+                r.acts_x, r.ld_acts_x = _ptr(t["acts_x"], "acts_x"), t["acts_x"].shape[1]
+            r.x6_col = int(bool(t.get("x6_col")))
             takes, ctakes = t.get("takes", ()), t.get("colsum_takes", ())
             r.n_takes, r.n_colsum_takes = len(takes), len(ctakes)
             for k, (row0, col0, nr, nc, out, o_r, o_c) in zip(r.takes, takes):
diff --git a/include/idealnerf.h b/include/idealnerf.h
--- a/include/idealnerf.h
+++ b/include/idealnerf.h
@@ -270,6 +270,7 @@
                       int pipe, void* workspace, size_t workspace_bytes, void* stream);
 
 #define IDN_DW_MAX_PRODUCTS 16
+#define IDN_DW_X6_PASS_SHARES (-1)
 #define IDN_DW_MAX_TAKES 4
 #define IDN_DW_MAX_COLSUM_TAKES 2
 typedef struct idn_dw_take {
@@ -293,6 +294,8 @@
     int n_colsum_takes;
     idn_dw_colsum_take colsum_takes[IDN_DW_MAX_COLSUM_TAKES];
     int splits, chunks_per_split;
+    const float* acts_x;
+    int ld_acts_x, x6_col;
 } idn_dw_product;
 size_t idealnerf_dw_products_workspace_bytes(void);
 int idealnerf_dw_products(int64_t rows, int pipe, int x6_items, idn_dw_product* products, int n, void* workspace,
```

Result: no change. 132.7 million (-0.3%).
